# chenhuims/DistributedDeepLearningSpark

Hardware: AMD Instinct MI355X
Metric: images/sec (whole node) ResNet-50 ImageNet-shape at 1/2/4/8 MI355X (higher is better)
Workload: dtype bf16; 1 GPU; model=resnet50, global_batch=256, image=224, per_gpu_batch=256, parallelism=dp1, optimizer=sgd-momentum, buckets=4

## Files before the change

### distributeddeeplearningspark_amd/csrc/bindings.cpp

```cpp
#include <torch/extension.h>
#include <ATen/hip/impl/HIPStreamMasqueradingAsCUDA.h>
#include <ATen/DeviceGuard.h>

#include "ddl_gemm.h"
#include "ddl_ops.h"

namespace py = pybind11;
using namespace ddl;

namespace {

inline hipStream_t cur_stream() { return at::hip::getCurrentHIPStreamMasqueradingAsCUDA().stream(); }

#define CHECK_CUDA(x) TORCH_CHECK((x).is_cuda(), #x " must be a GPU tensor")
#define CHECK_BF16(x) TORCH_CHECK((x).scalar_type() == at::kBFloat16, #x " must be bf16")
#define CHECK_F32(x) TORCH_CHECK((x).scalar_type() == at::kFloat, #x " must be fp32")
#define CHECK_CONTIG(x) TORCH_CHECK((x).is_contiguous(), #x " must be contiguous")
#define HIP_OK(expr)                                                                   \
  do {                                                                                 \
    int _e = (expr);                                                                   \
    TORCH_CHECK(_e == 0, "HIP launch failed: ", hipGetErrorString((hipError_t)_e)); \
  } while (0)

void fill_geom(ConvGeom& g, const py::dict& d) {
  g.n = d["n"].cast<int>();
  g.hi = d["hi"].cast<int>();
  g.wi = d["wi"].cast<int>();
  g.c = d["c"].cast<int>();
  g.ho = d["ho"].cast<int>();
  g.wo = d["wo"].cast<int>();
  g.sh = d["sh"].cast<int>();
  g.sw = d["sw"].cast<int>();
  g.tap_c = d["tap_c"].cast<int>();
  g.tap_shift = (g.tap_c > 0 && (g.tap_c & (g.tap_c - 1)) == 0) ? __builtin_ctz((unsigned)g.tap_c) : -1;
  auto dh = d["dh"].cast<std::vector<int>>();
  auto dw = d["dw"].cast<std::vector<int>>();
  std::vector<int> wt = d.contains("wt") ? d["wt"].cast<std::vector<int>>() : std::vector<int>(dh.size(), 0);
  TORCH_CHECK(dh.size() == dw.size() && dh.size() <= (size_t)kMaxTaps && wt.size() == dh.size(), "bad tap table");
  g.ntaps = (int)dh.size();
  for (size_t i = 0; i < dh.size(); ++i) {
    TORCH_CHECK(dh[i] >= -128 && dh[i] < 128 && dw[i] >= -128 && dw[i] < 128, "tap offset out of int8 range");
    g.dh[i] = (int8_t)dh[i];
    g.dw[i] = (int8_t)dw[i];
    g.wt[i] = (int16_t)wt[i];
  }
}

void gemm(const at::Tensor& a, const at::Tensor& b, const at::Tensor& c, int64_t M, int64_t N, int64_t K,
          int64_t a_mode, int64_t b_mode, int64_t lda, int64_t ldb, int64_t ldc, int64_t epi, int64_t tile,
          int64_t k_split, double alpha, double beta, c10::optional<at::Tensor> bias,
          c10::optional<at::Tensor> resid, int64_t ldr, int64_t relu, c10::optional<py::dict> geom,
          c10::optional<py::dict> outmap, int64_t b_kdiv, int64_t b_tap_stride,
          c10::optional<at::Tensor> stats, c10::optional<at::Tensor> aux, double drop_p, int64_t drop_seed,
          c10::optional<at::Tensor> resid_mask, c10::optional<at::Tensor> bnr_x, c10::optional<at::Tensor> bnr_mask,
          c10::optional<at::Tensor> bnr_mean, int64_t rsub_h, int64_t rsub_w, c10::optional<at::Tensor> bnr_scale, c10::optional<at::Tensor> bnr_shift, int64_t split_stride,
          int64_t zcount, int64_t za, int64_t zb, int64_t zc, int64_t zbias, std::vector<int64_t> cls_tap0,
          std::vector<int64_t> cls_nt, std::vector<int64_t> cls_coff, bool bnr_premask,
          c10::optional<at::Tensor> colscale, c10::optional<at::Tensor> relu_mask_out) {
  CHECK_CUDA(a);
  CHECK_CUDA(b);
  CHECK_CUDA(c);
  CHECK_BF16(a);
  CHECK_BF16(b);
  if (epi == EPI_BF16) { CHECK_BF16(c); } else { CHECK_F32(c); }
  const bool k_vec = a_mode == OP_KC || a_mode == OP_KC_GATHER || a_mode == OP_KC_GATHER8 || b_mode == OP_KC;
  TORCH_CHECK(!k_vec || K % 8 == 0, "gemm: K-contiguous operands need K % 8 == 0 (16-B vectors), got ", K);
  if (a_mode == OP_KC) TORCH_CHECK(lda % 8 == 0, "gemm: lda must be a multiple of 8");
  if (b_mode == OP_KC) TORCH_CHECK(ldb % 8 == 0, "gemm: ldb must be a multiple of 8");
  if (a_mode == OP_RC) TORCH_CHECK(lda % 8 == 0, "gemm: lda must be a multiple of 8");
  if (b_mode == OP_RC || b_mode == OP_RC_TAPS) TORCH_CHECK(ldb % 8 == 0, "gemm: ldb must be a multiple of 8");
  TORCH_CHECK(((uintptr_t)a.data_ptr() % 16) == 0 && ((uintptr_t)b.data_ptr() % 16) == 0, "gemm: operands must be 16-B aligned");
  TORCH_CHECK(k_split > 0 && k_split % 64 == 0, "gemm: k_split must be a positive multiple of 64");
  TORCH_CHECK(tile >= 0 && tile <= kTileConv3, "gemm: bad tile id");
  if (tile == kTileStream) {
    TORCH_CHECK(a_mode == OP_KC && (b_mode == OP_KC || b_mode == OP_RC) && epi == EPI_BF16 && !outmap.has_value() &&
                    relu <= ACT_RELU && drop_p == 0.0 && beta == 0.0 && k_split >= K,
                "gemm stream: KC x (KC|RC) operands, bf16 epilogue without GELU/dropout/outmap/beta/split-K");
    TORCH_CHECK(gemm_stream_panel((int)N, (int)K) > 0, "gemm stream: unsupported (N, K) = (", N, ", ", K, ")");
    TORCH_CHECK(ldc % 8 == 0 && ((uintptr_t)c.data_ptr() % 16) == 0, "gemm stream: 16-B aligned output rows");
    TORCH_CHECK(!resid || (ldr % 4 == 0 && ((uintptr_t)resid->data_ptr() % 8) == 0), "gemm stream: resid alignment");
  }
  if (tile == kTile256) {
    TORCH_CHECK(a_mode <= OP_RC && b_mode <= OP_RC && !outmap.has_value(), "gemm256: plain KC/RC operands only");
    TORCH_CHECK(K % 64 == 0 && k_split % 64 == 0, "gemm256: K and k_split must be multiples of 64");
    TORCH_CHECK(M >= 8 && N >= 8, "gemm256: M, N >= 8");
  }
  const int bm = (tile == 0 || tile == 1) ? 128 : 64;
  const int bn = (tile == 0 || tile == 2) ? 128 : 64;
  if (a_mode == OP_RC || a_mode == OP_RC_GATHER) TORCH_CHECK(M % 8 == 0, "gemm: row-contiguous A needs M % 8 == 0");
  if (b_mode == OP_RC || b_mode == OP_RC_GATHER || b_mode == OP_RC_GATHER8 || b_mode == OP_RC_TAPS)
    TORCH_CHECK(N % 8 == 0, "gemm: row-contiguous B needs N % 8 == 0");
  GemmParams p{};
  p.a = a.data_ptr();
  p.b = b.data_ptr();
  p.c = c.data_ptr();
  p.lda = lda;
  p.ldb = ldb;
  p.ldc = ldc;
  p.M = (int)M;
  p.N = (int)N;
  p.K = (int)K;
  p.k_split = (int)k_split;
  p.a_mode = (int)a_mode;
  p.b_mode = (int)b_mode;
  p.b_kdiv = (int)b_kdiv;
  p.b_tap_stride = b_tap_stride;
  p.alpha = (float)alpha;
  p.beta = (float)beta;
  TORCH_CHECK(relu >= ACT_NONE && relu <= ACT_GELU_BWD, "gemm: bad activation code");
  TORCH_CHECK(epi == EPI_BF16 || (relu == 0 && drop_p == 0.0), "gemm: activation/dropout need the bf16 epilogue");
  p.relu = (int)relu;
  if (relu >= ACT_GELU) {
    TORCH_CHECK(aux.has_value(), "gemm: GELU epilogues need the aux (pre-activation) tensor");
    CHECK_CUDA(*aux);
    CHECK_BF16(*aux);
    TORCH_CHECK(aux->numel() >= (M - 1) * ldc + N && ((uintptr_t)aux->data_ptr() % 16) == 0, "gemm: aux size/alignment");
    p.aux = aux->data_ptr();
  }
  TORCH_CHECK(drop_p >= 0.0 && drop_p < 1.0, "gemm: dropout p in [0, 1)");
  if (drop_p > 0.0) {
    p.drop_thresh = drop_t8(drop_p);
    p.drop_scale = drop_scale8(p.drop_thresh);
    p.drop_seed = (unsigned long long)drop_seed;
  }
  p.ldr = ldr;
  if (bias) {
    CHECK_CUDA(*bias);
    CHECK_F32(*bias);
    TORCH_CHECK(bias->numel() >= N, "bias too short");
    TORCH_CHECK((uintptr_t)bias->data_ptr() % 16 == 0, "gemm: bias must be 16-B aligned (vector loads)");
    p.bias = bias->data_ptr<float>();
  }
  if (resid) {
    CHECK_CUDA(*resid);
    CHECK_BF16(*resid);
    p.resid = resid->data_ptr();
  }
  if (rsub_h > 0) {
    TORCH_CHECK(resid.has_value() && epi == EPI_BF16 && !outmap.has_value() && !resid_mask.has_value() && rsub_w > 0 &&
                    M % (rsub_h * rsub_w) == 0,
                "gemm: a stride-2 residual needs resid (bf16, no outmap / mask) and M = N * rsub_h * rsub_w");
    const int64_t hs = (rsub_h + 1) / 2, ws_ = (rsub_w + 1) / 2;
    TORCH_CHECK(resid->numel() >= ((M / (rsub_h * rsub_w)) * hs * ws_ - 1) * ldr + N, "gemm: stride-2 residual too small");
    p.rsub_h = (int)rsub_h;
    p.rsub_w = (int)rsub_w;
  }
  if (resid_mask) {
    TORCH_CHECK(resid.has_value() && epi == EPI_BF16 && !outmap.has_value(), "gemm: resid_mask needs a residual (bf16, no outmap)");
    TORCH_CHECK(resid_mask->scalar_type() == at::kByte && resid_mask->is_contiguous() && ldr % 8 == 0 &&
                    resid_mask->numel() >= ((M - 1) * ldr + N + 7) / 8,
                "gemm: resid_mask must be uint8 [M * ldr / 8] with ldr % 8 == 0");
    p.resid_mask = resid_mask->data_ptr<uint8_t>();
  }
  if (geom) {
    fill_geom(p.g, *geom);
    TORCH_CHECK((int64_t)p.g.n * p.g.hi * p.g.wi * p.g.c < (int64_t(1) << 31),
                "gemm: a gathered tensor must have fewer than 2^31 elements");
    if (a_mode == OP_KC_GATHER)
      TORCH_CHECK(p.g.tap_c % 64 == 0 && (cls_nt.empty() ? K == (int64_t)p.g.ntaps * p.g.tap_c : K <= (int64_t)p.g.ntaps * p.g.tap_c),
                  "conv A gather: tap_c % 64 and K = taps*C");
    if (b_mode == OP_RC_GATHER) TORCH_CHECK(p.g.tap_c % bn == 0 && N == (int64_t)p.g.ntaps * p.g.tap_c, "conv B gather: tap_c % BN and N = taps*C");
    if (b_mode == OP_RC_TAPS) TORCH_CHECK(b_kdiv % 64 == 0 && K == (int64_t)p.g.ntaps * b_kdiv, "conv B taps: kdiv % 64 and K = taps*kdiv");
    if (a_mode == OP_KC_GATHER8) TORCH_CHECK(p.g.tap_c % 8 == 0 && K == (int64_t)p.g.ntaps * p.g.tap_c, "conv A gather8: tap_c % 8 and K = taps*C");
    if (b_mode == OP_RC_GATHER8) TORCH_CHECK(p.g.tap_c % 8 == 0 && N == (int64_t)p.g.ntaps * p.g.tap_c, "conv B gather8: tap_c % 8 and N = taps*C");
    if (a_mode == OP_KC_GATHER || a_mode == OP_KC_GATHER8) TORCH_CHECK(p.g.c == p.g.tap_c, "gather: c == tap_c");
  } else {
    TORCH_CHECK(a_mode <= OP_RC && b_mode <= OP_RC, "gather modes need a geometry");
  }
  if (outmap) {
    const auto& d = *outmap;
    p.om.enabled = 1;
    p.om.gh = d["gh"].cast<int>();
    p.om.gw = d["gw"].cast<int>();
    p.om.hy = d["hy"].cast<int>();
    p.om.wy = d["wy"].cast<int>();
    p.om.so = d["so"].cast<int>();
    p.om.oh = d["oh"].cast<int>();
    p.om.ow = d["ow"].cast<int>();
    p.om.zero_siblings = d.contains("zero") ? d["zero"].cast<int>() : 0;
  }
  if (stats) {
    CHECK_CUDA(*stats);
    CHECK_F32(*stats);
    TORCH_CHECK(epi == EPI_BF16, "fused stats need the bf16 epilogue");
    TORCH_CHECK(stats->numel() >= (int64_t)kStatShards * 2 * N, "stats workspace too small");
    p.stats = stats->data_ptr<float>();
  }
  if (bnr_x) {
    TORCH_CHECK(stats.has_value() && bnr_mean.has_value() && epi == EPI_BF16 && tile != kTile256,
                "gemm: the fused BN-backward reduction needs a stats workspace, the mean and a bf16 epilogue");
    TORCH_CHECK(tile == kTileStream || (N % 4 == 0 && ldc % 8 == 0 && !bias && relu == 0 && !aux &&
                                        drop_p == 0.0 && (a_mode == OP_KC || (a_mode == OP_KC_GATHER && b_mode == OP_KC))),
                "gemm: BN-backward reduce outside the streaming kernel: plain or gathered-A data-gradient, N % 4 == 0, "
                "ldc % 8 == 0, no bias / activation (a residual and a parity-class output map are allowed)");
    CHECK_CUDA(*bnr_x);
    CHECK_BF16(*bnr_x);
    TORCH_CHECK(bnr_x->is_contiguous() && bnr_x->numel() >= (M - 1) * ldc + N && ((uintptr_t)bnr_x->data_ptr() % 16) == 0,
                "gemm: bnr_x must be a 16-B aligned bf16 [M][ldc]");
    CHECK_F32(*bnr_mean);
    TORCH_CHECK(bnr_mean->numel() >= N && ((uintptr_t)bnr_mean->data_ptr() % 16) == 0, "gemm: bnr_mean [N], 16-B aligned");
    p.bnr_x = bnr_x->data_ptr();
    p.bnr_mean = bnr_mean->data_ptr<float>();
    if (bnr_mask) {
      TORCH_CHECK(bnr_mask->scalar_type() == at::kByte && bnr_mask->is_contiguous() && ldc % 8 == 0 &&
                      bnr_mask->numel() >= ((M - 1) * ldc + N + 7) / 8,
                  "gemm: bnr_mask must be uint8 [M * ldc / 8]");
      p.bnr_mask = bnr_mask->data_ptr<uint8_t>();
    }
    if (bnr_scale || bnr_shift) {
      TORCH_CHECK(bnr_scale && bnr_shift && !bnr_mask, "gemm: bnr scale/shift (no mask bits)");
      CHECK_F32(*bnr_scale);
      CHECK_F32(*bnr_shift);
      TORCH_CHECK(bnr_scale->numel() >= N && bnr_shift->numel() >= N && ((uintptr_t)bnr_scale->data_ptr() % 16) == 0 &&
                      ((uintptr_t)bnr_shift->data_ptr() % 16) == 0,
                  "gemm: bnr scale / shift [N], 16-B aligned");
      p.bnr_scale = bnr_scale->data_ptr<float>();
      p.bnr_shift = bnr_shift->data_ptr<float>();
    }
    if (bnr_premask) {
      TORCH_CHECK(bnr_mask.has_value() && !outmap.has_value(), "gemm: bnr_premask needs the mask bits and no output map");
      p.bnr_premask = 1;
    }
  } else if (bnr_premask) {
    TORCH_CHECK(stats.has_value() && bnr_mask.has_value() && !bnr_scale && !bnr_shift && !outmap.has_value() &&
                    epi == EPI_BF16 && tile != kTile256,
                "gemm: bnr_premask needs a stats workspace, the mask bits, a bf16 epilogue and no output map");
    TORCH_CHECK(tile == kTileStream || (tile != kTileConv3 && N % 4 == 0 && ldc % 8 == 0 && !bias && relu == 0 && !aux &&
                                        drop_p == 0.0 && a_mode == OP_KC),
                "gemm: bnr_premask outside the streaming kernel: plain data-gradient (a pointwise conv), N % 4 == 0, "
                "ldc % 8 == 0, no bias / activation");
    TORCH_CHECK(bnr_mask->is_cuda() && bnr_mask->scalar_type() == at::kByte && bnr_mask->is_contiguous() && ldc % 8 == 0 &&
                    bnr_mask->numel() >= ((M - 1) * ldc + N + 7) / 8,
                "gemm: bnr_mask must be uint8 [M * ldc / 8]");
    p.bnr_mask = bnr_mask->data_ptr<uint8_t>();
    p.bnr_premask = 1;
  }
  if (colscale || relu_mask_out) {
    TORCH_CHECK(tile == kTileStream && colscale.has_value() && resid.has_value() && b_mode == OP_KC && !stats && !bnr_x &&
                    !bnr_premask && rsub_h == 0 && alpha == 1.0,
                "gemm: colscale / relu_mask_out run on the streaming kernel's forward form with a residual, without "
                "statistics or a BN-backward reduction; the column scale takes alpha's place (alpha == 1)");
    CHECK_CUDA(*colscale);
    CHECK_F32(*colscale);
    TORCH_CHECK(colscale->is_contiguous() && colscale->numel() >= N && ((uintptr_t)colscale->data_ptr() % 16) == 0,
                "gemm: colscale [N] fp32, 16-B aligned");
    p.colscale = colscale->data_ptr<float>();
    if (relu_mask_out) {
      TORCH_CHECK(relu_mask_out->is_cuda() && relu_mask_out->scalar_type() == at::kByte && relu_mask_out->is_contiguous() &&
                      relu_mask_out->numel() >= ((M - 1) * ldc + N + 7) / 8,
                  "gemm: relu_mask_out must be uint8 [M * ldc / 8]");
      p.relu_mask_out = relu_mask_out->data_ptr<uint8_t>();
    }
  }
  (void)bm;
  if (tile == kTileConv3)
    TORCH_CHECK(conv3x3_halo_ok(p) && epi == EPI_BF16, "gemm conv3x3: needs a 3x3 / stride-1 / pad-1 KC_GATHER x KC "
                "conv with C % 64 == 0, N % 64 == 0, no split-K and at most bias/ReLU/statistics in the epilogue");
  if (split_stride > 0) {
    const int64_t splits = (K + k_split - 1) / k_split;
    TORCH_CHECK(epi == EPI_F32 && beta == 0.0 && split_stride >= M * ldc && c.numel() >= splits * split_stride,
                "gemm: split-K slabs need EPI_F32, beta = 0 and a workspace of splits x split_stride floats");
    p.split_stride = split_stride;
  }
  if (zcount > 1 && cls_nt.empty()) {
    TORCH_CHECK(tile >= 0 && tile <= 3 && !stats && !bnr_x && !outmap && !resid && !aux && drop_p == 0.0 &&
                    split_stride == 0 && relu <= ACT_RELU && za >= 0 && zb >= 0 && zc >= 0 && zbias >= 0,
                "gemm: replica batching (zcount > 1) runs the 64/128 tiles with at most bias / ReLU / split-K atomics");
    TORCH_CHECK(za % 8 == 0 && zb % 8 == 0 && (epi == EPI_BF16 ? zc % 8 : zc % 4) == 0 && zbias % 4 == 0,
                "gemm: replica strides must keep 16-B alignment");
    TORCH_CHECK(c.numel() >= (zcount - 1) * zc + (M - 1) * ldc + N, "gemm: output too small for zcount replicas");
    TORCH_CHECK(!bias || bias->numel() >= (zcount - 1) * zbias + N, "gemm: bias too short for zcount replicas");
    p.zcount = (int)zcount;
    p.za = za;
    p.zb = zb;
    p.zc = zc;
    p.zbias = zbias;
  }
  if (!cls_nt.empty()) {
    const int64_t nc = (int64_t)cls_nt.size();
    TORCH_CHECK(nc <= kMaxZCls && (int64_t)cls_tap0.size() == nc && (int64_t)cls_coff.size() == nc && zcount == nc,
                "gemm: parity classes need cls_tap0 / cls_nt / cls_coff of zcount <= ", kMaxZCls, " entries");
    TORCH_CHECK(tile >= 0 && tile <= 3 && a_mode == OP_KC_GATHER && b_mode == OP_KC && epi == EPI_BF16 && outmap &&
                    p.om.oh == 0 && p.om.ow == 0 && !p.om.zero_siblings && !stats && !bnr_x && !resid && !aux && !bias &&
                    drop_p == 0.0 && relu == 0 && split_stride == 0 && za == 0 && zb == 0 && zc == 0 && zbias == 0,
                "gemm: parity classes run KC_GATHER x KC on the 64/128 tiles with a plain bf16 output map");
    TORCH_CHECK(p.om.gh > 0 && p.om.gw > 0 && M % ((int64_t)p.om.gh * p.om.gw) == 0, "gemm: classes need M = n * gh * gw");
    const int64_t nimg = M / ((int64_t)p.om.gh * p.om.gw);
    const int64_t last_row = ((nimg - 1) * p.om.hy + (int64_t)(p.om.gh - 1) * p.om.so) * p.om.wy + (int64_t)(p.om.gw - 1) * p.om.so;
    int64_t kmax = 0;
    for (int64_t z = 0; z < nc; ++z) {
      TORCH_CHECK(cls_nt[z] > 0 && cls_tap0[z] >= 0 && cls_tap0[z] + cls_nt[z] <= p.g.ntaps, "gemm: class taps out of range");
      TORCH_CHECK(cls_coff[z] >= 0 && cls_coff[z] % 8 == 0 && cls_coff[z] + last_row * ldc + N <= c.numel(),
                  "gemm: class output offset out of range");
      TORCH_CHECK((cls_tap0[z] + cls_nt[z]) * (int64_t)p.g.tap_c <= ldb, "gemm: class filter columns past ldb");
      kmax = std::max(kmax, cls_nt[z] * (int64_t)p.g.tap_c);
      p.cls_tap0[z] = (int)cls_tap0[z];
      p.cls_nt[z] = (int)cls_nt[z];
      p.cls_coff[z] = cls_coff[z];
    }
    TORCH_CHECK(K == kmax && k_split >= K, "gemm: classes need K = the largest class's K and no split-K");
    p.zcls = 1;
    p.zcount = (int)nc;
  }
  at::DeviceGuard guard(a.device());
  HIP_OK(launch_gemm_bf16(p, (int)epi, (int)tile, cur_stream()));
}

void conv3x3_wgrad(const at::Tensor& dy, const at::Tensor& x, const at::Tensor& gw, const c10::optional<at::Tensor>& ws,
                   int64_t splits, int64_t tpb, bool pp) {
  CHECK_CUDA(dy);
  CHECK_CUDA(x);
  CHECK_CUDA(gw);
  CHECK_BF16(dy);
  CHECK_BF16(x);
  CHECK_F32(gw);
  CHECK_CONTIG(dy);
  CHECK_CONTIG(x);
  CHECK_CONTIG(gw);
  TORCH_CHECK(x.dim() == 4 && gw.dim() == 4 && gw.size(1) == 3 && gw.size(2) == 3 && gw.size(3) == x.size(3),
              "conv3x3_wgrad: x [N, H, W, Ci], gw [Co, 3, 3, Ci]");
  const int n = (int)x.size(0), h = (int)x.size(1), w = (int)x.size(2), ci = (int)x.size(3), co = (int)gw.size(0);
  TORCH_CHECK(dy.numel() == (int64_t)n * h * w * co, "conv3x3_wgrad: dy must be [N, H, W, Co] (stride 1, pad 1)");
  TORCH_CHECK(conv3x3_wgrad_ok(n, h, w, ci, co), "conv3x3_wgrad: needs Ci, Co % 64 == 0 and a <= 256-pixel row tiling");
  int s_plan = 0, t_plan = 0, ntiles = 0;
  conv3x3_wgrad_plan(n, h, w, ci, co, 1, 1, s_plan, t_plan, ntiles);
  TORCH_CHECK(splits >= 1 && tpb >= 1 && (splits - 1) * tpb < ntiles && splits * tpb >= ntiles,
              "conv3x3_wgrad: splits x tiles-per-split must cover the pixel tiles exactly once");
  float* wsp = nullptr;
  if (ws) {
    CHECK_CUDA(*ws);
    CHECK_F32(*ws);
    TORCH_CHECK(ws->is_contiguous() && ws->numel() >= splits * co * 9 * (int64_t)ci, "conv3x3_wgrad: workspace too small");
    wsp = ws->data_ptr<float>();
  }
  at::DeviceGuard guard(x.device());
  HIP_OK(launch_conv3x3_wgrad(reinterpret_cast<const uint16_t*>(dy.data_ptr()), reinterpret_cast<const uint16_t*>(x.data_ptr()),
                              gw.data_ptr<float>(), wsp, n, h, w, ci, co, (int)splits, (int)tpb, pp, cur_stream()));
}

py::object conv3x3_wgrad_plan_py(int64_t n, int64_t h, int64_t w, int64_t ci, int64_t co, int64_t blocks_per_cu,
                                 int64_t cus) {
  if (!conv3x3_wgrad_ok((int)n, (int)h, (int)w, (int)ci, (int)co)) return py::none();
  int splits = 0, tpb = 0, ntiles = 0;
  conv3x3_wgrad_plan((int)n, (int)h, (int)w, (int)ci, (int)co, (int)blocks_per_cu, (int)cus, splits, tpb, ntiles);
  return py::make_tuple(splits, tpb);
}

}

void register_ops(py::module& m);
void register_runtime(py::module& m);
void register_transformer(py::module& m);
void register_rnn(py::module& m);
void register_layer_ops(py::module& m);

PYBIND11_MODULE(_C, m) {
  m.doc() = "MI355X-native kernels and runtime of distributeddeeplearningspark_amd";
  m.def("gemm", &gemm, "MFMA implicit-GEMM (bf16 in, fp32 accumulate)", py::arg("a"), py::arg("b"), py::arg("c"),
        py::arg("M"), py::arg("N"), py::arg("K"), py::arg("a_mode"), py::arg("b_mode"), py::arg("lda"),
        py::arg("ldb"), py::arg("ldc"), py::arg("epi"), py::arg("tile"), py::arg("k_split"), py::arg("alpha") = 1.0,
        py::arg("beta") = 0.0, py::arg("bias") = py::none(), py::arg("resid") = py::none(), py::arg("ldr") = 0,
        py::arg("relu") = false, py::arg("geom") = py::none(), py::arg("outmap") = py::none(),
        py::arg("b_kdiv") = 0, py::arg("b_tap_stride") = 0, py::arg("stats") = py::none(),
        py::arg("aux") = py::none(), py::arg("drop_p") = 0.0, py::arg("drop_seed") = 0,
        py::arg("resid_mask") = py::none(), py::arg("bnr_x") = py::none(), py::arg("bnr_mask") = py::none(),
        py::arg("bnr_mean") = py::none(), py::arg("rsub_h") = 0, py::arg("rsub_w") = 0,
        py::arg("bnr_scale") = py::none(), py::arg("bnr_shift") = py::none(),
        py::arg("split_stride") = 0, py::arg("zcount") = 1, py::arg("za") = 0, py::arg("zb") = 0, py::arg("zc") = 0,
        py::arg("zbias") = 0, py::arg("cls_tap0") = std::vector<int64_t>{}, py::arg("cls_nt") = std::vector<int64_t>{},
        py::arg("cls_coff") = std::vector<int64_t>{}, py::arg("bnr_premask") = false,
        py::arg("colscale") = py::none(), py::arg("relu_mask_out") = py::none());
  m.def("conv3x3_wgrad", &conv3x3_wgrad, "3x3 stride-1 weight gradient (halo kernel): gw += dW", py::arg("dy"),
        py::arg("x"), py::arg("gw"), py::arg("ws"), py::arg("splits"), py::arg("tpb"), py::arg("pp") = false);
  m.def("conv3x3_wgrad_plan", &conv3x3_wgrad_plan_py,
        "(splits, tiles per split) of the 3x3 weight-gradient halo kernel, or None when it does not apply",
        py::arg("n"), py::arg("h"), py::arg("w"), py::arg("ci"), py::arg("co"), py::arg("blocks_per_cu"),
        py::arg("cus"));
  m.attr("ACT_NONE") = (int)ACT_NONE;
  m.attr("ACT_RELU") = (int)ACT_RELU;
  m.attr("ACT_GELU") = (int)ACT_GELU;
  m.attr("ACT_GELU_BWD") = (int)ACT_GELU_BWD;
  m.attr("OP_KC") = (int)OP_KC;
  m.attr("OP_RC") = (int)OP_RC;
  m.attr("OP_KC_GATHER") = (int)OP_KC_GATHER;
  m.attr("OP_RC_GATHER") = (int)OP_RC_GATHER;
  m.attr("OP_RC_TAPS") = (int)OP_RC_TAPS;
  m.attr("OP_KC_GATHER8") = (int)OP_KC_GATHER8;
  m.attr("OP_RC_GATHER8") = (int)OP_RC_GATHER8;
  m.attr("EPI_BF16") = (int)EPI_BF16;
  m.attr("EPI_F32") = (int)EPI_F32;
  m.attr("EPI_F32_ATOMIC") = (int)EPI_F32_ATOMIC;
  register_ops(m);
  register_transformer(m);
  register_rnn(m);
  register_layer_ops(m);
  register_runtime(m);
}
```

### distributeddeeplearningspark_amd/csrc/include/ddl_gemm.h

```cpp
#pragma once
#include <stdint.h>

namespace ddl {

enum OperandMode : int {
  OP_KC = 0,
  OP_RC = 1,
  OP_KC_GATHER = 2,
  OP_RC_GATHER = 3,
  OP_RC_TAPS = 4,
  OP_KC_GATHER8 = 5,
  OP_RC_GATHER8 = 6,
};

enum EpilogueMode : int {
  EPI_BF16 = 0,
  EPI_F32 = 1,
  EPI_F32_ATOMIC = 2,
  EPI_BF16_LITE = 3,
  EPI_BF16_BNR = 4,
};

constexpr int kMaxTaps = 64;
constexpr int kMaxZCls = 4;

struct ConvGeom {
  int n, hi, wi, c;
  int ho, wo;
  int sh, sw;
  int ntaps;
  int tap_c;
  int tap_shift;
  int8_t dh[kMaxTaps];
  int8_t dw[kMaxTaps];
  int16_t wt[kMaxTaps];
};

struct OutMap {
  int enabled;
  int gh, gw;
  int hy, wy;
  int so;
  int oh, ow;
  int zero_siblings;
};

struct GemmParams {
  const void* a; long lda;
  const void* b; long ldb;
  void* c; long ldc;
  int M, N, K;
  int k_split;
  int a_mode, b_mode;
  int b_kdiv; long b_tap_stride;
  ConvGeom g;
  OutMap om;
  const float* bias;
  const void* resid; long ldr;
  const uint8_t* resid_mask;
  float alpha, beta;
  int relu;
  float* stats;
  void* aux;
  uint32_t drop_thresh;
  float drop_scale;
  unsigned long long drop_seed;
  const void* bnr_x;
  const uint8_t* bnr_mask;
  const float* bnr_mean;
  const float* bnr_scale;
  const float* bnr_shift;
  int bnr_premask;
  int rsub_h, rsub_w;
  int group_m;
  long split_stride;
  int zcount;
  long za, zb, zc, zbias;
  int zcls;
  int cls_tap0[kMaxZCls], cls_nt[kMaxZCls];
  long cls_coff[kMaxZCls];
  const float* colscale;
  uint8_t* relu_mask_out;
};

enum Activation : int { ACT_NONE = 0, ACT_RELU = 1, ACT_GELU = 2, ACT_GELU_BWD = 3 };

constexpr int kStatShards = 32;
constexpr int kTile256 = 4;
constexpr int kTileStream = 5;
constexpr int kTileConv3 = 6;

bool conv3x3_halo_ok(const GemmParams& p);

bool conv3x3_wgrad_ok(int n, int h, int w, int ci, int co);
void conv3x3_wgrad_plan(int n, int h, int w, int ci, int co, int blocks_per_cu, int cus, int& splits, int& tpb,
                        int& ntiles);
int launch_conv3x3_wgrad(const uint16_t* dy, const uint16_t* x, float* gw, float* ws, int n, int h, int w, int ci,
                         int co, int splits, int tpb, bool pp, void* stream);

int gemm_stream_panel(int N, int K);

int launch_gemm_bf16(const GemmParams& p, int epi, int tile, void* stream);

}
```

### distributeddeeplearningspark_amd/csrc/include/ddl_ops.h

```cpp
#pragma once
#include <hip/hip_runtime.h>
#include <stdint.h>

namespace ddl {

inline uint32_t drop_t8(double p) {
  if (!(p > 0.0)) return 0u;
  const double t = p * 256.0 + 0.5;
  return t < 1.0 ? 1u : (t >= 255.0 ? 255u : (uint32_t)t);
}
inline float drop_scale8(uint32_t t8) { return t8 ? (float)(256.0 / (256.0 - (double)t8)) : 1.f; }

constexpr int kBnShards = 32;
constexpr int kMaxPartials = 512;

int bn_partial_rows(long M, int C);
int splitk_finalize(float* ws, void* y, const float* bias, float* stats, long M, int C, int relu, int splits,
                    long slab_stride, hipStream_t s, long brows = 0,
                    long zbias = 0);
int bn_stats(const void* x, float* ws, long M, int C, hipStream_t s);
int bn_finalize(const float* ws, int S, long M, int C, const float* gamma, const float* beta, float eps,
                float momentum, float* running_mean, float* running_var, float* save_mean, float* save_invstd,
                float* scale, float* shift, hipStream_t s);
int bn_apply(const void* x, const float* scale, const float* shift, const void* resid, void* y, void* mask, long M,
             int C, int relu, hipStream_t s, const float* res_scale = nullptr, const float* res_shift = nullptr);
int bn_bwd_reduce(const void* dy, const void* x, const void* y, const float* scale, const float* shift,
                  const float* mean, float* ws, long M, int C, int mode, hipStream_t s);
int bn_bwd_finalize(const float* ws, int S, long M, int C, const float* gamma, const float* mean, const float* invstd,
                    float* dgamma, float* dbeta, float* coef, hipStream_t s);
int bn_bwd_dx(const void* dy, const void* x, const void* y, const float* scale, const float* shift,
              const float* coef, void* dx, void* dres, long M, int C, int mode, hipStream_t s,
              const void* x2 = nullptr, const float* mean2 = nullptr, float* ws2 = nullptr);

int bn_fold_sums(const void* w, long ldw, const float* P, const float* wsg, const float* mean, const float* wsy,
                 int rows, float* sums, float* s, int Co, int Ci, hipStream_t st);
int bn_fold_coef(const void* w, long ldw, const float* P, const float* S, const float* s, const float* coef, void* WA,
                 void* WAt, void* Gm, float* kv, float* dW, long lddw, int Co, int Ci, hipStream_t st);
int gram_colsum(const void* y2, long ld, long M, int Ci, float* S, float* s, int cus, hipStream_t st);
int bn_fold_fwd_stats(const void* w, long ldw, const float* S, const float* s, long M, float* ws, int Co, int Ci,
                      hipStream_t st);

bool pool3s2_bn_bwd_ok(int N, int H, int W, int C, int Ho, int Wo, int k = 3);
int pool3s2_bn_bwd(const void* dy, const uint8_t* am, const void* x, const float* scale, const float* shift,
                   const float* mean, const float* coef, float* ws, int S, void* dx, int N, int H, int W, int C, int Ho,
                   int Wo, hipStream_t s, int k = 3);

int maxpool_fwd(const void* x, void* y, uint8_t* argmax, int N, int H, int W, int C, int Ho, int Wo, int kh, int kw,
                int sh, int sw, int ph, int pw, hipStream_t s, const float* scale = nullptr, const float* shift = nullptr);
int maxpool_bwd(const void* dy, const uint8_t* argmax, void* dx, int N, int H, int W, int C, int Ho, int Wo, int kh,
                int kw, int sh, int sw, int ph, int pw, hipStream_t s);
int avgpool_global_fwd(const void* x, void* y, int N, int HW, int C, hipStream_t s);
int avgpool_global_bwd(const void* dy, void* dx, int N, int HW, int C, hipStream_t s);

int softmax_xent(const void* logits, int logits_bf16, const int64_t* labels, const float* target_probs,
                 float* loss_rows, void* dlogits, int B, int K, long ld, float grad_scale, float label_smoothing,
                 int ignore_index, hipStream_t s, const float* grad_scale_dev = nullptr, float* loss_out = nullptr,
                 float out_scale = 1.f, int zrows = 0);
int label_count_inv(const int64_t* labels, long n, int ignore_index, float* inv, hipStream_t s);
int rows_sum_scaled(const float* rows, long n, float scale, const float* dev, float* out, hipStream_t s);
int scale_bf16_dev(void* x, long n, const float* s_dev, hipStream_t s);
int mse_fwd_bwd(const float* pred, const float* target, long n, float* loss, float* grad, hipStream_t s);
int prob_xent(const float* p, const int64_t* labels, const float* target, float* loss_rows, float* dp, int B, int K,
              float eps, float scale, int ignore_index, hipStream_t s);

int cast_f32_bf16(const float* x, void* y, long n, hipStream_t s);
int cast_bf16_f32(const void* x, float* y, long n, hipStream_t s);
int sum_rows_bf16(const void* x, void* y, int R, long n, hipStream_t s);
int relu_bwd(const void* dy, const void* y, void* dx, long n, hipStream_t s);
int add_bf16(const void* a, const void* b, void* y, long n, hipStream_t s);
int bias_grad(const void* dy, float* db, long M, int N, int accumulate, hipStream_t s, float* det_ws = nullptr,
              const void* relu_y = nullptr, void* relu_dx = nullptr, int zcount = 1, long zdb = 0);
int pad_cols_bf16(const void* x, long ldx, void* out, long R, int K, int Kp, hipStream_t s);
constexpr int kMaxZeroRanges = 8;
struct ZeroRanges {
  void* p[kMaxZeroRanges];
  long pre[kMaxZeroRanges + 1];
  int tail_words[kMaxZeroRanges];
  int count;
};
int zero_ranges(const ZeroRanges& r, hipStream_t s);
int gather_bf16(const void* src, const int* idx, void* out, long n, hipStream_t s);
int scatter_add_f32(const float* src, const int* idx, float* dst, long n, hipStream_t s);
int bias_grad_rows(long M);
int slab_reduce(const float* ws, int splits, float* c, long M, int N, long ldc, float beta, hipStream_t s);
int transpose_bf16(const void* x, void* y, int R, int C, long ldx, hipStream_t s);
int im2col(const void* x, void* col, int n, int hi, int wi, int c, int ho, int wo, int sh, int sw, int ntaps,
           const int* dh, const int* dw, int kpad, hipStream_t s);
int s2d_pad(const void* x, void* y, int N, int H, int W, int C, int Ho, int Wo, int pad, hipStream_t s);
int normalize_u8(const uint8_t* x, void* y, long npix, int c, int cpad, const float* mean, const float* invstd,
                 hipStream_t s);

int sgd_step(float* w, const float* g, float* mom, void* w16, long n, float lr, float momentum, float dampening,
             float wd, int nesterov, float gscale, hipStream_t s);
int adam_step(float* w, const float* g, float* m, float* v, void* w16, long n, float lr, float b1, float b2,
              float eps, float wd, int adamw, float bc1, float bc2, float gscale, float* tstep,
              hipStream_t s, unsigned* tick_ctr = nullptr);
int step_tick(float* t, hipStream_t s);
int adagrad_step(float* w, const float* g, float* acc, void* w16, long n, float lr, float eps, float wd, float gscale,
                 hipStream_t s);
int rmsprop_step(float* w, const float* g, float* acc, void* w16, long n, float lr, float rho, float eps, float wd,
                 float gscale, hipStream_t s);
int sumsq_f32(const float* x, long n, float* out, hipStream_t s);

struct AttnParams {
  const uint16_t* qkv; long ld;
  int q_off, k_off, v_off;
  uint16_t* o; long ldo;
  float* lse;
  const int* lens;
  int B, H, S;
  float scale, scale_log2;
  uint32_t drop_t8;
  float drop_scale;
  unsigned long long drop_seed;
  const uint16_t* dout; long lddo;
  float* dvec;
  uint16_t* dqkv; long lddqkv;
  int xcd_remap;
};
int attn_fwd(const AttnParams& p, hipStream_t s);
int attn_bwd(const AttnParams& p, hipStream_t s);

int layernorm_fwd(const void* x, const float* gamma, const float* beta, void* y, float* mean, float* rstd, long M,
                  int H, float eps, float drop_p, unsigned long long seed, hipStream_t s);
int ln_partial_rows(long M);
int ln_bwd_rows(long M, int H);
int layernorm_bwd(const void* dy, const void* x, const float* mean, const float* rstd, const float* gamma, void* dx,
                  void* dx_drop, float drop_p, unsigned long long seed, float* ws, int P, long M, int H,
                  float in_drop_p, unsigned long long in_seed, int parts, hipStream_t s);
int embed_word_grad(const int64_t* sorted_ids, const int64_t* perm, const void* ds, float* gword, long T, int H,
                    hipStream_t s);
int embed_word_grad_atomic(const int64_t* ids, const void* ds, float* gword, long T, int H, long V, hipStream_t s);
int embed_pos_grad(const void* ds, float* gpos, int B, int S, int H, hipStream_t s);
int colsum_partials(const float* ws, int P, int N, float* out, int accumulate, hipStream_t s, long ld = 0);
int mlm_gather(const void* h, const int64_t* pos, void* out, int B, int S, int P, int H, hipStream_t s);
int mlm_scatter(const void* dout, const int64_t* pos, void* dh, int B, int S, int P, int H, hipStream_t s);
int embed_fwd(const int64_t* ids, const int64_t* types, const void* word, const void* pos, const void* type,
              void* out, long T, int S, int H, hipStream_t s);
int embed_bwd(const int64_t* ids, const int64_t* types, const void* ds, float* gword, float* gpos, float* wsT, int P,
              int ntypes, long T, int S, int H, hipStream_t s);

constexpr int kMaxRnnRep = 16;
struct RnnRep {
  const float* x[kMaxRnnRep];
  const float* y[kMaxRnnRep];
  const float* W[kMaxRnnRep];
  const float* U[kMaxRnnRep];
  const float* b[kMaxRnnRep];
  const float* Wd[kMaxRnnRep];
  const float* bd[kMaxRnnRep];
  float* gW[kMaxRnnRep];
  float* gU[kMaxRnnRep];
  float* gb[kMaxRnnRep];
  float* gWd[kMaxRnnRep];
  float* gbd[kMaxRnnRep];
  float* hist[kMaxRnnRep];
  int nbr[kMaxRnnRep];
  int steps[kMaxRnnRep];
  int* ctr;
  int* live;
  int B, K;
};
struct OptRep {
  float* w[kMaxRnnRep];
  const float* g[kMaxRnnRep];
  float* s1[kMaxRnnRep];
  float* s2[kMaxRnnRep];
  float* t[kMaxRnnRep];
};
int rnn_replica_step(int cell, const RnnRep& rp, int R, int T, int H, int I, float* hs, float* cs, float* gates,
                     float* hlast, float* dh, float* dgates, const OptRep& op, long n, int opt, float lr, float p1,
                     float p2, float eps, float wd, int amode, hipStream_t s);
bool rnn_replica_ok(int cell, int H, int I, int K, int B);

bool rnn_fast_path(int H);
bool rnn_fuses_input(int H, int I);
bool rnn_reg_path(int cell, int H, int act, int ract);
int rnn_fwd(int cell, const float* xw, const float* x, const float* W, const float* b, int I, const float* U,
            float* hs, float* cs, float* gates, float* y, int B, int T, int H, int rs, int act, int ract,
            hipStream_t s);
int rnn_param_grad(int cell, const float* dg, const float* hs, const float* gates, const float* x, float* gU,
                   float* gW, float* gb, int B, int T, int H, int I, hipStream_t s, int rev = 0);
bool rnn_bwd_uses_ut(int H);
int rnn_bwd(int cell, const float* dy, const float* U, const float* UT, const float* hs, const float* cs,
            const float* gates, float* dgates, int B, int T, int H, int rs, int act, int ract, hipStream_t s);

struct RnnDir {
  const float* xw[2];
  const float* W[2];
  const float* b[2];
// ... 91 lines not shown
```

### distributeddeeplearningspark_amd/csrc/kernels/bn_fold.hip

```cpp
#include "ddl_common.h"
#include "ddl_ops.h"

namespace ddl {
namespace {

constexpr int FT = 32;
constexpr int BKG = 128;
constexpr int BKW = 64;

__device__ __forceinline__ double wave_sum(double v) {
#pragma unroll
  for (int o = 32; o > 0; o >>= 1) v += __shfl_xor(v, o, 64);
  return v;
}

constexpr int kSumSplit = 8;
__global__ __launch_bounds__(256) void bn_fold_sums_kernel(const bf16_t* __restrict__ w, long ldw,
                                                            const float* __restrict__ P,
                                                            const float* __restrict__ wsg,
                                                            const float* __restrict__ mean,
                                                            const float* __restrict__ wsy, int rows,
                                                            float* __restrict__ sums, float* __restrict__ s, int Co,
                                                            int Ci, int cb) {
  const int lane = threadIdx.x & 63, wv = threadIdx.x >> 6;
// ... 148 lines not shown
#pragma unroll
    for (int v = 0; v < G::V; ++v) {
      const int row = t0 + pr + v * G::PPP;
      reg[v] = row < r1 ? *reinterpret_cast<const uint4*>(y2 + (long)row * ld + ch * 8) : make_uint4(0u, 0u, 0u, 0u);
    }
  };
  load(r0);
  for (int t0 = r0; t0 < r1; t0 += G::TP) {
    __syncthreads();
#pragma unroll
    for (int v = 0; v < G::V; ++v)
      *reinterpret_cast<uint4*>(tile + (pr + v * G::PPP) * G::ROWB + ch * 16) = reg[v];
    if (panel == 0) {
#pragma unroll
      for (int v = 0; v < G::V; ++v) {
        const uint32_t wv[4] = {reg[v].x, reg[v].y, reg[v].z, reg[v].w};
#pragma unroll
        for (int q = 0; q < 4; ++q) {
          cs[2 * q] += __uint_as_float(wv[q] << 16);
          cs[2 * q + 1] += __uint_as_float(wv[q] & 0xffff0000u);
        }
      }
    }
    __syncthreads();
    if (t0 + G::TP < r1) load(t0 + G::TP);
    f32x4 acc[G::RB];
#pragma unroll
    for (int i = 0; i < G::RB; ++i) acc[i] = f32x4{0.f, 0.f, 0.f, 0.f};
#pragma unroll 2
    for (int kk = 0; kk < G::TP / 32; ++kk) {
      const bf16x8 b = gram_frag<G::ROWB>(tile, kk, cb, lane);
#pragma unroll
      for (int i = 0; i < G::RB; ++i) acc[i] = mfma16x16x32(gram_frag<G::ROWB>(tile, kk, 16 * i, lane), b, acc[i]);
    }
#pragma unroll
    for (int i = 0; i < G::RB; ++i) tot[i] += acc[i];
  }
#pragma unroll
  for (int i = 0; i < G::RB; ++i)
#pragma unroll
    for (int e = 0; e < 4; ++e)
      atomicAdd(S + (long)(16 * i + 4 * (lane >> 4) + e) * CI + cb + (lane & 15), tot[i][e]);
  if (panel == 0) {
    __syncthreads();
    float* red = reinterpret_cast<float*>(tile);
#pragma unroll
    for (int e = 0; e < 8; ++e) red[pr * CI + ch * 8 + e] = cs[e];
    __syncthreads();
    if ((int)threadIdx.x < CI) {
      double a = 0.0;
      for (int j = 0; j < G::PPP; ++j) a += (double)red[j * CI + threadIdx.x];
      atomicAdd(s + threadIdx.x, (float)a);
    }
  }
}

constexpr int FST = 32;
__global__ __launch_bounds__(256) void bn_fold_fwd_stats_kernel(const bf16_t* __restrict__ w, long ldw,
                                                                 const float* __restrict__ S,
                                                                 const float* __restrict__ s, long M,
                                                                 float* __restrict__ ws, int Co, int Ci) {
  __shared__ float Ssh[FST][256];
  __shared__ double wsh[4][256];
  __shared__ double sb[256];
  const int lane = threadIdx.x & 63, wv = threadIdx.x >> 6;
  const int co = (int)blockIdx.x * 4 + wv;
  const int cor = min(co, Co - 1);
  const double invM = 1.0 / (double)M;
  for (int ci = lane; ci < Ci; ci += 64) wsh[wv][ci] = (double)bf2f(w[(long)cor * ldw + ci]);
  for (int ci = threadIdx.x; ci < Ci; ci += 256) sb[ci] = (double)s[ci] * invM;
  double q[4] = {0.0, 0.0, 0.0, 0.0};
  for (int ci0 = 0; ci0 < Ci; ci0 += FST) {
    __syncthreads();
    for (int idx = threadIdx.x * 4; idx < FST * Ci; idx += 1024) {
      const float4 v = *reinterpret_cast<const float4*>(S + (long)ci0 * Ci + idx);
      *reinterpret_cast<float4*>(&Ssh[idx / Ci][idx % Ci]) = v;
    }
    __syncthreads();
#pragma unroll
    for (int t = 0; t < 4; ++t) {
      const int cj = lane + 64 * t;
      if (cj < Ci) {
        const double sj = sb[cj];
        double inner = 0.0;
#pragma unroll 8
        for (int r = 0; r < FST; ++r) inner += wsh[wv][ci0 + r] * ((double)Ssh[r][cj] * invM - sb[ci0 + r] * sj);
        q[t] += inner;
      }
    }
  }
  double mean = 0.0, var = 0.0;
#pragma unroll
  for (int t = 0; t < 4; ++t) {
    const int cj = lane + 64 * t;
    if (cj < Ci) {
      mean += wsh[wv][cj] * sb[cj];
      var += wsh[wv][cj] * q[t];
    }
  }
  mean = wave_sum(mean);
  var = wave_sum(var);
  if (var < 0.0) var = 0.0;
  if (lane == 0 && co < Co) {
    ws[co] = (float)((double)M * mean);
    ws[Co + co] = (float)((double)M * (var + mean * mean));
  }
}

}

int gram_colsum(const void* y2, long ld, long M, int Ci, float* S, float* s, int cus, hipStream_t st) {
  if ((Ci != 64 && Ci != 128 && Ci != 256) || M <= 0 || M >= (1L << 30) || ld % 8) return (int)hipErrorInvalidValue;
  const int P = Ci / 64, tp = Ci == 64 ? 256 : (Ci == 128 ? 128 : 64);
  long rows = std::max<long>(std::max(1024, 8 * Ci), (M + 2 * cus / P - 1) / std::max(1, 2 * cus / P));
  rows = (rows + tp - 1) / tp * tp;
  const int chunks = (int)((M + rows - 1) / rows);
  const dim3 grid((unsigned)(chunks * P));
  const bf16_t* y = (const bf16_t*)y2;
  switch (Ci) {
    case 64: hipLaunchKernelGGL(gram_colsum_kernel<64>, grid, dim3(256), 0, st, y, ld, (int)M, (int)rows, S, s); break;
    case 128: hipLaunchKernelGGL(gram_colsum_kernel<128>, grid, dim3(256), 0, st, y, ld, (int)M, (int)rows, S, s); break;
    default: hipLaunchKernelGGL(gram_colsum_kernel<256>, grid, dim3(256), 0, st, y, ld, (int)M, (int)rows, S, s); break;
  }
  return (int)hipGetLastError();
}

int bn_fold_fwd_stats(const void* w, long ldw, const float* S, const float* s, long M, float* ws, int Co, int Ci,
                      hipStream_t st) {
  if (Ci % FST || Ci > 256 || Ci % 4 || Co <= 0 || M <= 0) return (int)hipErrorInvalidValue;
  hipLaunchKernelGGL(bn_fold_fwd_stats_kernel, dim3((Co + 3) / 4), dim3(256), 0, st, (const bf16_t*)w, ldw, S, s, M, ws,
                     Co, Ci);
  return (int)hipGetLastError();
}

int bn_fold_sums(const void* w, long ldw, const float* P, const float* wsg, const float* mean, const float* wsy,
                 int rows, float* sums, float* s, int Co, int Ci, hipStream_t st) {
  const int cb = (Co + 3) / 4;
  const int sblocks = rows > 0 ? kSumSplit * ((Ci + 63) / 64) : 0;
  hipLaunchKernelGGL(bn_fold_sums_kernel, dim3(cb + sblocks), dim3(256), 0, st, (const bf16_t*)w, ldw, P, wsg,
                     mean, wsy, rows, sums, s, Co, Ci, cb);
  return (int)hipGetLastError();
}

int bn_fold_coef(const void* w, long ldw, const float* P, const float* S, const float* s, const float* coef, void* WA,
                 void* WAt, void* Gm, float* kv, float* dW, long lddw, int Co, int Ci, hipStream_t st) {
  if (Co % BKG || Ci % BKW) return (int)hipErrorInvalidValue;
  const int tc = Ci / FT;
  const int blocks = tc * tc + (Co / FT) * tc;
  hipLaunchKernelGGL(bn_fold_coef_kernel, dim3(blocks), dim3(256), 0, st, (const bf16_t*)w, ldw, P, S, s, coef,
                     (bf16_t*)WA, (bf16_t*)WAt, (bf16_t*)Gm, kv, dW, lddw, Co, Ci);
  return (int)hipGetLastError();
}

}
```

### distributeddeeplearningspark_amd/csrc/kernels/gemm_dispatch.hip

```cpp
#include "ddl_gemm.h"
#include <hip/hip_runtime.h>
#include <stdlib.h>
namespace ddl {
int launch_gemm_plain_akc(const GemmParams& p, int epi, int tile, hipStream_t s);
int launch_gemm_plain_arc(const GemmParams& p, int epi, int tile, hipStream_t s);
int launch_gemm_conv(const GemmParams& p, int epi, int tile, hipStream_t s);
int launch_gemm256(const GemmParams& p, int epi, hipStream_t s);
int launch_gemm_stream(const GemmParams& p, int epi, hipStream_t s);
int launch_conv3x3(const GemmParams& p, int epi, hipStream_t s);

int launch_gemm_bf16(const GemmParams& p_in, int epi, int tile, void* stream) {
  hipStream_t s = reinterpret_cast<hipStream_t>(stream);
  if (p_in.M <= 0 || p_in.N <= 0) return 0;
  GemmParams p = p_in;
  p.group_m = 8;
  if ((p.colscale || p.relu_mask_out) && tile != kTileStream) return (int)hipErrorInvalidValue;
  if (p.bnr_premask && (!p.bnr_mask || !p.stats || p.bnr_scale)) return (int)hipErrorInvalidValue;
  if (p.bnr_premask && !p.bnr_x && tile != kTileStream && p.a_mode != OP_KC) return (int)hipErrorInvalidValue;
  if ((p.bnr_x || p.bnr_premask) && tile != kTileStream &&
      (tile == kTile256 || epi != EPI_BF16 || p.om.zero_siblings ||
       (p.resid && (p.ldr % 4 || (uintptr_t)p.resid % 8)) || p.aux || p.drop_thresh || p.bias || p.relu || p.N % 4 || p.ldc % 8 ||
       !(p.a_mode == OP_KC || p.a_mode == OP_KC_GATHER) || (p.a_mode == OP_KC_GATHER && p.b_mode != OP_KC)))
    return (int)hipErrorInvalidValue;
  const bool plain = (p.a_mode == OP_KC || p.a_mode == OP_RC) && (p.b_mode == OP_KC || p.b_mode == OP_RC);
  if (tile == kTile256) {
    if (!plain || p.K % 64 || p.k_split % 64 || p.om.enabled) return (int)hipErrorInvalidValue;
    return launch_gemm256(p, epi, s);
  }
  if (tile == kTileStream) return launch_gemm_stream(p, epi, s);
  if (tile == kTileConv3) return launch_conv3x3(p, epi, s);
  if (plain) return p.a_mode == OP_KC ? launch_gemm_plain_akc(p, epi, tile, s) : launch_gemm_plain_arc(p, epi, tile, s);
  return launch_gemm_conv(p, epi, tile, s);
}
}
```

### distributeddeeplearningspark_amd/csrc/kernels/gemm_stream.hip

```cpp
#include "ddl_gemm_kernel.h"

namespace ddl {
namespace gst {

constexpr int THREADS = 256;
constexpr int BM = 64;
constexpr int LDS_BUDGET = 80 * 1024;
typedef __attribute__((address_space(3))) void lds_t;

template <int WN, int K, bool CSM = false>
struct Cfg {
  static constexpr int NB = 4 * WN;
  static constexpr int RN = WN / 16;
  static constexpr int KS = K / 32;
  static constexpr int CPR = K / 8;
  static constexpr int TILE = BM * K * 2;
  static constexpr int D = TILE / 1024 / 4;
  static constexpr int OCPR = NB / 8;
  static constexpr int STAGE = BM * NB * 2;
  static constexpr int RPP = THREADS / OCPR;
  static constexpr int S = BM / RPP;
  static constexpr int SV = CSM ? 2 * S : S;
  static constexpr int NBUF_FIT = (LDS_BUDGET - STAGE) / TILE;
  static constexpr int NBUF = NBUF_FIT > 4 ? 4 : NBUF_FIT;
  static constexpr int LDS = NBUF * TILE + STAGE;
  static_assert(NBUF >= 2, "A ring needs two buffers");
  static_assert(D >= 1 && OCPR >= 8 && RPP >= 1 && BM % RPP == 0, "shape");
  static_assert((NBUF - 1) * (D + SV) <= 63, "vmcnt range");
  static_assert(4 * 2 * OCPR * 8 * 4 <= STAGE, "stats reduction fits in the staging buffer");
};

template <int CPR>
__device__ __forceinline__ int sw(int r) {
  if constexpr (CPR == 8) return (r >> 1) & 7;
  else return r & 15;
}

template <int N>
__device__ __forceinline__ void wait_vm() {
  __builtin_amdgcn_s_waitcnt((N & 15) | ((N >> 4) << 14) | 0x0F70);
}

template <class CF, int SV = CF::S>
__device__ __forceinline__ void wait_tile(int younger_store_tiles) {
  constexpr int base = (CF::NBUF - 1) * CF::D;
  switch (younger_store_tiles) {
    case 0: wait_vm<base>(); break;
    case 1: wait_vm<base + SV>(); break;
    case 2: wait_vm<base + 2 * SV>(); break;
    default: wait_vm<base + 3 * SV>(); break;
  }
}

template <class CF>
__device__ __forceinline__ void stage_a(const bf16_t* __restrict__ A, long lda, int M, int m0, char* slot, int w,
                                        int lane) {
#pragma unroll
  for (int i = 0; i < CF::D; ++i) {
    const int blk = i * 4 + w;
    const int u = blk * 64 + lane;
    const int r = u / CF::CPR, cp = u % CF::CPR;
    const int c = cp ^ sw<CF::CPR>(r);
    const int gr = min(m0 + r, M - 1);
    const bf16_t* src = A + (long)gr * lda + c * 8;
    const uint32_t dst = __builtin_amdgcn_readfirstlane((uint32_t) reinterpret_cast<uintptr_t>((lds_t*)(slot + blk * 1024)));
    asm volatile("s_mov_b32 m0, %1\n\tglobal_load_lds_dwordx4 %0, off" ::"v"(src), "s"(dst) : "memory", "m0");
  }
}

}

typedef __attribute__((ext_vector_type(2))) unsigned u32x2_t;
typedef __attribute__((ext_vector_type(4))) unsigned u32x4_t;
__device__ __forceinline__ u32x4_t ald128(const void* p) {
  u32x4_t v;
  asm volatile("global_load_dwordx4 %0, %1, off" : "=v"(v) : "v"(p) : "memory");
  return v;
}
__device__ __forceinline__ u32x2_t ald64(const void* p) {
  u32x2_t v;
  asm volatile("global_load_dwordx2 %0, %1, off" : "=v"(v) : "v"(p) : "memory");
  return v;
}
__device__ __forceinline__ unsigned ald32(const void* p) {
  unsigned v;
  asm volatile("global_load_dword %0, %1, off" : "=v"(v) : "v"(p) : "memory");
  return v;
}
__device__ __forceinline__ unsigned ald16(const void* p) {
  unsigned v;
  asm volatile("global_load_ushort %0, %1, off" : "=v"(v) : "v"(p) : "memory");
  return v;
}
__device__ __forceinline__ unsigned ald8(const void* p) {
  unsigned v;
  asm volatile("global_load_ubyte %0, %1, off" : "=v"(v) : "v"(p) : "memory");
  return v;
}
template <bool ASM> __device__ __forceinline__ u32x4_t sld128(const void* p) {
  if constexpr (ASM) return ald128(p);
  return *reinterpret_cast<const u32x4_t*>(p);
}
template <bool ASM> __device__ __forceinline__ u32x2_t sld64(const void* p) {
  if constexpr (ASM) return ald64(p);
  return *reinterpret_cast<const u32x2_t*>(p);
}
template <bool ASM> __device__ __forceinline__ unsigned sld32(const void* p) {
  if constexpr (ASM) return ald32(p);
  return *reinterpret_cast<const uint32_t*>(p);
}
template <bool ASM> __device__ __forceinline__ unsigned sld16(const void* p) {
  if constexpr (ASM) return ald16(p);
  return *reinterpret_cast<const uint16_t*>(p);
}
template <bool ASM> __device__ __forceinline__ unsigned sld8(const void* p) {
  if constexpr (ASM) return ald8(p);
  return *reinterpret_cast<const uint8_t*>(p);
}


template <int WN, int K, int BMODE, bool RES, int BNR = 0, bool CSM = false>
__global__ __launch_bounds__(gst::THREADS, 2) void gemm_stream_kernel(const GemmParams p) {
  using namespace gst;
  using CF = Cfg<WN, K, CSM>;
  constexpr bool kAsmSide = true;
  __shared__ __attribute__((aligned(16))) char smem[CF::LDS];
  char* const stg = smem + CF::NBUF * CF::TILE;
  const int lane = threadIdx.x & 63, w = threadIdx.x >> 6;
  const int n0 = blockIdx.y * CF::NB;
  const int mt = (p.M + BM - 1) / BM;
  const int nloc = ((int)blockIdx.x < mt) ? (mt - 1 - (int)blockIdx.x) / (int)gridDim.x + 1 : 0;
  const bf16_t* __restrict__ A = reinterpret_cast<const bf16_t*>(p.a);

  bf16x8 bfr[CF::RN][CF::KS];
  {
    const bf16_t* __restrict__ B = reinterpret_cast<const bf16_t*>(p.b);
#pragma unroll
    for (int rn = 0; rn < CF::RN; ++rn)
#pragma unroll
      for (int ks = 0; ks < CF::KS; ++ks) {
        const int n = n0 + WN * w + 16 * rn + (lane & 15);
        const int k = 32 * ks + 8 * (lane >> 4);
        if constexpr (BMODE == OP_KC) {
          bfr[rn][ks] = *reinterpret_cast<const bf16x8*>(B + (long)n * p.ldb + k);
        } else {
          s16x8 v;
#pragma unroll
          for (int j = 0; j < 8; ++j) v[j] = (short)B[(long)(k + j) * p.ldb + n];
          bfr[rn][ks] = __builtin_bit_cast(bf16x8, v);
        }
      }
  }
  float bias_r[CF::RN][4];
#pragma unroll
  for (int rn = 0; rn < CF::RN; ++rn) {
    const float4 bv = p.bias ? *reinterpret_cast<const float4*>(p.bias + n0 + WN * w + 16 * rn + 4 * (lane >> 4))
                             : make_float4(0.f, 0.f, 0.f, 0.f);
    bias_r[rn][0] = bv.x;
    bias_r[rn][1] = bv.y;
    bias_r[rn][2] = bv.z;
    bias_r[rn][3] = bv.w;
  }
  float csc_r[CSM ? CF::RN : 1][4];
  if constexpr (CSM) {
#pragma unroll
    for (int rn = 0; rn < CF::RN; ++rn) {
      const float4 cv = *reinterpret_cast<const float4*>(p.colscale + n0 + WN * w + 16 * rn + 4 * (lane >> 4));
      csc_r[rn][0] = cv.x;
      csc_r[rn][1] = cv.y;
      csc_r[rn][2] = cv.z;
      csc_r[rn][3] = cv.w;
    }
  }
  wait_vm<0>();
  auto tile_m0 = [&](int i) { return min((int)blockIdx.x + i * (int)gridDim.x, mt - 1) * BM; };

#pragma unroll
  for (int s = 0; s < CF::NBUF - 1; ++s) stage_a<CF>(A, p.lda, p.M, tile_m0(s), smem + s * CF::TILE, w, lane);

  float s1[8], s2[8];
#pragma unroll
  for (int e = 0; e < 8; ++e) s1[e] = s2[e] = 0.f;
  const int oc = threadIdx.x % CF::OCPR, orow = threadIdx.x / CF::OCPR;
  float bmu[8];
  float bsc[BNR == 2 ? 8 : 1], bsh[BNR == 2 ? 8 : 1];
  if constexpr (BNR == 1 || BNR == 2) {
    const float4 a = *reinterpret_cast<const float4*>(p.bnr_mean + n0 + oc * 8);
    const float4 b = *reinterpret_cast<const float4*>(p.bnr_mean + n0 + oc * 8 + 4);
    bmu[0] = a.x; bmu[1] = a.y; bmu[2] = a.z; bmu[3] = a.w;
    bmu[4] = b.x; bmu[5] = b.y; bmu[6] = b.z; bmu[7] = b.w;
  }
  if constexpr (BNR == 2) {
    const float4 a0 = *reinterpret_cast<const float4*>(p.bnr_scale + n0 + oc * 8);
    const float4 a1 = *reinterpret_cast<const float4*>(p.bnr_scale + n0 + oc * 8 + 4);
    const float4 b0 = *reinterpret_cast<const float4*>(p.bnr_shift + n0 + oc * 8);
    const float4 b1 = *reinterpret_cast<const float4*>(p.bnr_shift + n0 + oc * 8 + 4);
    bsc[0] = a0.x; bsc[1] = a0.y; bsc[2] = a0.z; bsc[3] = a0.w; bsc[4] = a1.x; bsc[5] = a1.y; bsc[6] = a1.z; bsc[7] = a1.w;
    bsh[0] = b0.x; bsh[1] = b0.y; bsh[2] = b0.z; bsh[3] = b0.w; bsh[4] = b1.x; bsh[5] = b1.y; bsh[6] = b1.z; bsh[7] = b1.w;
  }
  bf16_t* __restrict__ Cout = reinterpret_cast<bf16_t*>(p.c);

  for (int i = 0; i < nloc; ++i) {
    const int m0 = tile_m0(i);
    u32x2_t rres[BM / 16][CF::RN];
    unsigned rmk32[BM / 16];
    u32x2_t rmk64[CF::RN == 4 ? BM / 16 : 1];
    unsigned rodd_bits = 0u;
    const bool has_mask = p.resid_mask != nullptr;
    if constexpr (RES) {
#pragma unroll
      for (int mb = 0; mb < BM / 16; ++mb) {
        const int m = min(m0 + 16 * mb + (lane & 15), p.M - 1);
        long rrow = m;
        if (p.rsub_h) {
          int rn_, ri_, rj_;
          pix_decompose((uint32_t)m, p.rsub_h, p.rsub_w, rn_, ri_, rj_);
          const bool rodd = (ri_ | rj_) & 1;
          rodd_bits |= (rodd ? 1u : 0u) << mb;
          rrow = rodd ? 0L : ((long)rn_ * ((p.rsub_h + 1) >> 1) + (ri_ >> 1)) * ((p.rsub_w + 1) >> 1) + (rj_ >> 1);
        }
        const long row = rrow * p.ldr + n0 + WN * w;
#pragma unroll
        for (int rn = 0; rn < CF::RN; ++rn)
          rres[mb][rn] = sld64<kAsmSide>(reinterpret_cast<const bf16_t*>(p.resid) + row + 16 * rn + 4 * (lane >> 4));
        const void* mp = has_mask ? (const void*)(p.resid_mask + (row >> 3)) : p.resid;
        if constexpr (CF::RN == 1) rmk32[mb] = sld16<kAsmSide>(mp);
        else if constexpr (CF::RN == 2) rmk32[mb] = sld32<kAsmSide>(mp);
        else rmk64[mb] = sld64<kAsmSide>(mp);
      }
    }
    u32x4_t bx[(BNR == 1 || BNR == 2) ? CF::S : 1];
    unsigned bm8[(BNR == 1 || BNR == 3) ? CF::S : 1];
    if constexpr (BNR) {
#pragma unroll
      for (int ps = 0; ps < CF::S; ++ps) {
        const int m = min(m0 + orow + ps * CF::RPP, p.M - 1);
        const long idx = (long)m * p.ldc + n0 + oc * 8;
        if constexpr (BNR != 3) bx[ps] = sld128<kAsmSide>(reinterpret_cast<const bf16_t*>(p.bnr_x) + idx);
        if constexpr (BNR == 1)
          bm8[ps] = sld8<kAsmSide>(p.bnr_mask ? (const void*)(p.bnr_mask + (idx >> 3)) : (const void*)p.bnr_x);
        if constexpr (BNR == 3) bm8[ps] = sld8<kAsmSide>(p.bnr_mask + (idx >> 3));
      }
    }
    const int ahead = i + CF::NBUF - 1;
    stage_a<CF>(A, p.lda, p.M, tile_m0(ahead), smem + (ahead % CF::NBUF) * CF::TILE, w, lane);
    if constexpr (CSM) {
      if (p.relu_mask_out) wait_tile<CF, CF::SV>(min(i, CF::NBUF - 1));
      else wait_tile<CF>(min(i, CF::NBUF - 1));
    } else {
      wait_tile<CF>(min(i, CF::NBUF - 1));
    }
    __builtin_amdgcn_s_barrier();

    const char* abuf = smem + (i % CF::NBUF) * CF::TILE;
    f32x4 acc[BM / 16][CF::RN];
#pragma unroll
    for (int mb = 0; mb < BM / 16; ++mb)
#pragma unroll
      for (int rn = 0; rn < CF::RN; ++rn) acc[mb][rn] = f32x4{0.f, 0.f, 0.f, 0.f};
#pragma unroll
    for (int ks = 0; ks < CF::KS; ++ks)
#pragma unroll
      for (int mb = 0; mb < BM / 16; ++mb) {
        const int r = 16 * mb + (lane & 15);
        const int c = 4 * ks + (lane >> 4);
        const bf16x8 a = *reinterpret_cast<const bf16x8*>(abuf + r * (K * 2) + ((c ^ sw<CF::CPR>(r)) << 4));
#pragma unroll
        for (int rn = 0; rn < CF::RN; ++rn) acc[mb][rn] = mfma16x16x32(bfr[rn][ks], a, acc[mb][rn]);
      }

    constexpr int kBnrLoads = BNR == 1 ? 2 * CF::S : (BNR != 0 ? CF::S : 0);
    if constexpr (kAsmSide && RES) {
      wait_vm<CF::D + kBnrLoads>();
      __builtin_amdgcn_sched_barrier(0);
#pragma unroll
      for (int mb = 0; mb < BM / 16; ++mb) {
#pragma unroll
        for (int rn = 0; rn < CF::RN; ++rn) asm volatile("" : "+v"(rres[mb][rn]));
        if constexpr (CF::RN == 4) asm volatile("" : "+v"(rmk64[mb]));
        else asm volatile("" : "+v"(rmk32[mb]));
      }
    }
#pragma unroll
    for (int mb = 0; mb < BM / 16; ++mb) {
      const int r = 16 * mb + (lane & 15);
#pragma unroll
      for (int rn = 0; rn < CF::RN; ++rn) {
        const int nl = WN * w + 16 * rn + 4 * (lane >> 4);
        float v[4];
#pragma unroll
        for (int e = 0; e < 4; ++e) {
          if constexpr (CSM) v[e] = fmaf(acc[mb][rn][e], csc_r[rn][e], bias_r[rn][e]);
          else v[e] = fmaf(acc[mb][rn][e], p.alpha, bias_r[rn][e]);
        }
        if constexpr (RES) {
          const u32x2_t rv = rres[mb][rn];
          uint64_t mraw;
          if constexpr (CF::RN == 4) mraw = ((uint64_t)rmk64[mb].y << 32) | rmk64[mb].x;
          else mraw = rmk32[mb];
          const uint64_t rm = ((rodd_bits >> mb) & 1u) ? 0ull : (has_mask ? mraw : ~0ull);
          const uint32_t mk = (uint32_t)(rm >> (16 * rn + 4 * (lane >> 4)));
          v[0] += (mk & 1u) ? __uint_as_float(rv.x << 16) : 0.f;
          v[1] += (mk & 2u) ? __uint_as_float(rv.x & 0xffff0000u) : 0.f;
          v[2] += (mk & 4u) ? __uint_as_float(rv.y << 16) : 0.f;
          v[3] += (mk & 8u) ? __uint_as_float(rv.y & 0xffff0000u) : 0.f;
        }
        if (p.relu == ACT_RELU) {
#pragma unroll
          for (int e = 0; e < 4; ++e) v[e] = fmaxf(v[e], 0.f);
        }
        *reinterpret_cast<uint2*>(stg + r * (CF::NB * 2) + (((nl >> 3) ^ sw<CF::OCPR>(r)) << 4) + (nl & 7) * 2) =
            make_uint2(pack_bf16x2(v[0], v[1]), pack_bf16x2(v[2], v[3]));
      }
    }
    __builtin_amdgcn_s_waitcnt(0xC07F);
    __builtin_amdgcn_s_barrier();

    if constexpr (kAsmSide && BNR) {
      wait_vm<CF::D>();
      __builtin_amdgcn_sched_barrier(0);
#pragma unroll
      for (int ps = 0; ps < CF::S; ++ps) {
        if constexpr (BNR != 3) asm volatile("" : "+v"(bx[ps]));
        if constexpr (BNR == 1 || BNR == 3) asm volatile("" : "+v"(bm8[ps]));
      }
    }
#pragma unroll
    for (int ps = 0; ps < CF::S; ++ps) {
      const int r = orow + ps * CF::RPP;
      const int m = m0 + r;
      uint4 v = *reinterpret_cast<const uint4*>(stg + r * (CF::NB * 2) + ((oc ^ sw<CF::OCPR>(r)) << 4));
      if constexpr (BNR == 3) {
        const uint32_t b = bm8[ps];
        v.x &= ((b & 1u) ? 0xffffu : 0u) | ((b & 2u) ? 0xffff0000u : 0u);
        v.y &= ((b & 4u) ? 0xffffu : 0u) | ((b & 8u) ? 0xffff0000u : 0u);
        v.z &= ((b & 16u) ? 0xffffu : 0u) | ((b & 32u) ? 0xffff0000u : 0u);
        v.w &= ((b & 64u) ? 0xffffu : 0u) | ((b & 128u) ? 0xffff0000u : 0u);
      }
      if (m < p.M) {
        *reinterpret_cast<uint4*>(Cout + (long)m * p.ldc + n0 + oc * 8) = v;
        if constexpr (CSM) {
          if (p.relu_mask_out) {
            const uint32_t wv[4] = {v.x, v.y, v.z, v.w};
            uint32_t bits = 0u;
#pragma unroll
            for (int q = 0; q < 4; ++q) {
              bits |= (((wv[q] & 0xffffu) - 1u) < 0x7f80u ? 1u : 0u) << (2 * q);
              bits |= (((wv[q] >> 16) - 1u) < 0x7f80u ? 1u : 0u) << (2 * q + 1);
            }
            p.relu_mask_out[((long)m * p.ldc + n0 + oc * 8) >> 3] = (uint8_t)bits;
          }
        }
        if constexpr (BNR == 3) {
          const uint32_t wv[4] = {v.x, v.y, v.z, v.w};
#pragma unroll
          for (int q = 0; q < 4; ++q) {
            s1[2 * q] += __uint_as_float(wv[q] << 16);
            s1[2 * q + 1] += __uint_as_float(wv[q] & 0xffff0000u);
          }
        } else if constexpr (BNR) {
          const uint32_t wv[4] = {v.x, v.y, v.z, v.w};
          const uint32_t xv[4] = {bx[ps].x, bx[ps].y, bx[ps].z, bx[ps].w};
          uint32_t bmk = 0xffu;
          if constexpr (BNR == 1) bmk = p.bnr_mask ? bm8[ps] : 0xffu;
#pragma unroll
          for (int q = 0; q < 4; ++q) {
#pragma unroll
            for (int h = 0; h < 2; ++h) {
              const int e = 2 * q + h;
              const float xe = __uint_as_float(h ? (xv[q] & 0xffff0000u) : (xv[q] << 16));
              bool keep;
              if constexpr (BNR == 2) keep = xe * bsc[e] + bsh[e] > 0.f;
              else keep = (bmk >> e) & 1u;
              const float d = keep ? __uint_as_float(h ? (wv[q] & 0xffff0000u) : (wv[q] << 16)) : 0.f;
              s1[e] += d;
              s2[e] += d * (xe - bmu[e]);
            }
          }
        } else if (!CSM && p.stats) {
          const uint32_t wv[4] = {v.x, v.y, v.z, v.w};
#pragma unroll
          for (int q = 0; q < 4; ++q) {
            const float lo = __uint_as_float(wv[q] << 16), hi = __uint_as_float(wv[q] & 0xffff0000u);
            s1[2 * q] += lo;
            s2[2 * q] += lo * lo;
            s1[2 * q + 1] += hi;
            s2[2 * q + 1] += hi * hi;
          }
        }
      }
    }
  }
  wait_vm<0>();

  if (!CSM && p.stats) {
#pragma unroll
    for (int o = CF::OCPR; o < 64; o <<= 1)
#pragma unroll
      for (int e = 0; e < 8; ++e) {
        s1[e] += __shfl_xor(s1[e], o, 64);
        s2[e] += __shfl_xor(s2[e], o, 64);
      }
    __syncthreads();
    float* red = reinterpret_cast<float*>(stg);
    if (lane < CF::OCPR) {
#pragma unroll
      for (int e = 0; e < 8; ++e) {
        red[(w * CF::OCPR + lane) * 16 + e] = s1[e];
        red[(w * CF::OCPR + lane) * 16 + 8 + e] = s2[e];
      }
    }
    __syncthreads();
    float* st = p.stats + (long)(blockIdx.x % kStatShards) * 2 * p.N;
    for (int t = threadIdx.x; t < CF::NB; t += THREADS) {
      const int ch = t >> 3, e = t & 7;
      float a = 0.f, b = 0.f;
#pragma unroll
      for (int ww = 0; ww < 4; ++ww) {
        a += red[(ww * CF::OCPR + ch) * 16 + e];
        b += red[(ww * CF::OCPR + ch) * 16 + 8 + e];
      }
      atomicAdd(st + n0 + t, a);
      atomicAdd(st + p.N + n0 + t, b);
    }
  }
}

namespace {

int num_cus() {
  static int cus = 0;
  if (!cus) {
    int dev = 0;
    (void)hipGetDevice(&dev);
    if (hipDeviceGetAttribute(&cus, hipDeviceAttributeMultiprocessorCount, dev) != hipSuccess || cus <= 0) cus = 256;
  }
  return cus;
}

template <int WN, int K, int BMODE>
int launch_ws(const GemmParams& p, hipStream_t s) {
  using CF = gst::Cfg<WN, K>;
  constexpr bool kRes = !(WN == 64 && K == 128);
  constexpr bool kBnr = CF::NB <= (K >= 256 ? 64 : 128);
  const int panels = p.N / CF::NB;
  const int mt = (p.M + gst::BM - 1) / gst::BM;
  const int gx = std::max(1, std::min(mt, 2 * num_cus() / std::max(1, panels)));
  if (p.colscale || p.relu_mask_out) {
    constexpr bool kCsm = BMODE == OP_KC && ((WN == 64 && K == 64) || (WN == 32 && K == 128) || (WN == 32 && K == 256));
    if constexpr (kCsm) {
      if (!p.colscale || !p.resid || p.bnr_x || p.bnr_premask || p.stats || p.rsub_h) return (int)hipErrorInvalidValue;
      hipLaunchKernelGGL((gemm_stream_kernel<WN, K, BMODE, true, 0, true>), dim3(gx, panels), dim3(gst::THREADS), 0, s, p);
    } else {
      return (int)hipErrorInvalidValue;
    }
  } else if (p.bnr_premask) {
    if constexpr (kBnr && kRes && BMODE == OP_RC) {
      if (!p.bnr_mask || p.bnr_scale) return (int)hipErrorInvalidValue;
      if (p.resid)
        hipLaunchKernelGGL((gemm_stream_kernel<WN, K, BMODE, true, 3>), dim3(gx, panels), dim3(gst::THREADS), 0, s, p);
      else
        hipLaunchKernelGGL((gemm_stream_kernel<WN, K, BMODE, false, 3>), dim3(gx, panels), dim3(gst::THREADS), 0, s, p);
    } else {
      return (int)hipErrorInvalidValue;
    }
  } else if (p.bnr_x && p.bnr_scale) {
    constexpr bool kRes2 = WN == 16 && K == 256 && BMODE == OP_RC;
    if constexpr (kBnr) {
      if (p.resid) {
        if constexpr (kRes2)
          hipLaunchKernelGGL((gemm_stream_kernel<WN, K, BMODE, true, 2>), dim3(gx, panels), dim3(gst::THREADS), 0, s, p);
        else
          return (int)hipErrorInvalidValue;
      } else {
        hipLaunchKernelGGL((gemm_stream_kernel<WN, K, BMODE, false, 2>), dim3(gx, panels), dim3(gst::THREADS), 0, s, p);
      }
    } else {
      return (int)hipErrorInvalidValue;
    }
  } else if (p.bnr_x) {
    if constexpr (kBnr && kRes) {
      if (p.resid)
        hipLaunchKernelGGL((gemm_stream_kernel<WN, K, BMODE, true, 1>), dim3(gx, panels), dim3(gst::THREADS), 0, s, p);
      else
        hipLaunchKernelGGL((gemm_stream_kernel<WN, K, BMODE, false, 1>), dim3(gx, panels), dim3(gst::THREADS), 0, s, p);
    } else if constexpr (kBnr) {
      if (p.resid) return (int)hipErrorInvalidValue;
      hipLaunchKernelGGL((gemm_stream_kernel<WN, K, BMODE, false, 1>), dim3(gx, panels), dim3(gst::THREADS), 0, s, p);
    } else {
      return (int)hipErrorInvalidValue;
    }
  } else if (p.resid) {
    if constexpr (kRes)
      hipLaunchKernelGGL((gemm_stream_kernel<WN, K, BMODE, true>), dim3(gx, panels), dim3(gst::THREADS), 0, s, p);
    else
      return (int)hipErrorInvalidValue;
  } else {
    hipLaunchKernelGGL((gemm_stream_kernel<WN, K, BMODE, false>), dim3(gx, panels), dim3(gst::THREADS), 0, s, p);
  }
  return (int)hipGetLastError();
}

template <int WN, int BMODE>
int launch_k(const GemmParams& p, hipStream_t s) {
  switch (p.K) {
    case 64: return launch_ws<WN, 64, BMODE>(p, s);
    case 128: return launch_ws<WN, 128, BMODE>(p, s);
    default:
      if constexpr (WN <= 32) return launch_ws<WN, 256, BMODE>(p, s);
      return (int)hipErrorInvalidValue;
  }
}

template <int BMODE>
int launch_panel(const GemmParams& p, int nb, hipStream_t s) {
  switch (nb) {
    case 64: return launch_k<16, BMODE>(p, s);
    case 128: return launch_k<32, BMODE>(p, s);
    default: return launch_k<64, BMODE>(p, s);
  }
}

}

int gemm_stream_panel(int N, int K) {
  if (K != 64 && K != 128 && K != 256) return 0;
  const int max_nb = K == 256 ? 128 : 256;
  for (int nb = max_nb; nb >= 64; nb >>= 1)
    if (N % nb == 0 && (N == nb || nb == max_nb)) return nb;
  return 0;
}

int launch_gemm_stream(const GemmParams& p, int epi, hipStream_t s) {
  int nb = gemm_stream_panel(p.N, p.K);
  if (p.resid && p.K == 128 && nb == 256) nb = 128;
  if ((p.bnr_x || p.bnr_premask) && nb > (p.K >= 256 ? 64 : 128)) nb = p.K >= 256 ? 64 : 128;
  const bool ok = nb && epi == EPI_BF16 && p.a_mode == OP_KC && (p.b_mode == OP_KC || p.b_mode == OP_RC) &&
                  !p.om.enabled && !p.aux && !p.drop_thresh && (p.relu == ACT_NONE || p.relu == ACT_RELU) &&
                  p.beta == 0.f && p.k_split >= p.K && p.lda % 8 == 0 && p.ldc % 8 == 0 &&
                  (p.b_mode == OP_RC || p.ldb % 8 == 0) && (!p.resid || p.ldr % 4 == 0) &&
                  ((uintptr_t)p.a % 16 == 0) && ((uintptr_t)p.c % 16 == 0) &&
                  (p.b_mode == OP_RC || (uintptr_t)p.b % 16 == 0) && (!p.resid || (uintptr_t)p.resid % 8 == 0) &&
                  (!p.bnr_x || (p.stats && (uintptr_t)p.bnr_x % 16 == 0 && (uintptr_t)p.bnr_mean % 16 == 0)) &&
                  (!p.bnr_scale || (p.bnr_shift && (uintptr_t)p.bnr_scale % 16 == 0 &&
                                    (uintptr_t)p.bnr_shift % 16 == 0)) &&
                  (!p.bnr_premask || (p.stats && p.bnr_mask)) &&
                  (!p.colscale || (uintptr_t)p.colscale % 16 == 0);
  if (!ok) return (int)hipErrorInvalidValue;
  return p.b_mode == OP_KC ? launch_panel<OP_KC>(p, nb, s) : launch_panel<OP_RC>(p, nb, s);
}

}
```

### distributeddeeplearningspark_amd/csrc/ops_bindings.cpp

```cpp
#include <torch/extension.h>
#include <ATen/hip/impl/HIPStreamMasqueradingAsCUDA.h>
#include <ATen/DeviceGuard.h>

#include "ddl_ops.h"

namespace py = pybind11;
using namespace ddl;

namespace {

inline hipStream_t cur_stream() { return at::hip::getCurrentHIPStreamMasqueradingAsCUDA().stream(); }

#define CK(cond, ...) TORCH_CHECK(cond, __VA_ARGS__)
#define GPU(x) CK((x).is_cuda(), #x " must be a GPU tensor")
#define BF16(x) CK((x).scalar_type() == at::kBFloat16 && (x).is_contiguous(), #x " must be contiguous bf16")
#define F32(x) CK((x).scalar_type() == at::kFloat && (x).is_contiguous(), #x " must be contiguous fp32")
#define HIP_OK(expr)                                                                  \
  do {                                                                                \
    int _e = (expr);                                                                  \
    CK(_e == 0, "HIP launch failed: ", hipGetErrorString((hipError_t)_e)); \
  } while (0)

template <class T>
T* optr(const c10::optional<at::Tensor>& t) {
// ... 8 lines not shown
  HIP_OK(bn_stats(x.data_ptr(), ws.data_ptr<float>(), x.numel() / C, (int)C, cur_stream()));
}

void splitk_finalize_(const at::Tensor& ws, const at::Tensor& y, int64_t C, c10::optional<at::Tensor> bias, bool relu,
                      c10::optional<at::Tensor> stats, int64_t splits, int64_t brows, int64_t zbias) {
  GPU(ws); F32(ws); BF16(y);
  CK(C % 8 == 0 && y.numel() % C == 0 && y.is_contiguous() && ws.is_contiguous(), "splitk_finalize: shapes");
  CK(splits >= 0 && ws.numel() >= std::max<int64_t>(splits, 1) * y.numel() && (splits > 0 || ws.numel() == y.numel()),
     "splitk_finalize: workspace size");
  if (bias) {
    F32(*bias);
    CK(brows > 0 ? (zbias % 4 == 0 && bias->numel() >= ((y.numel() / C - 1) / brows) * zbias + C) : bias->numel() == C,
       "splitk_finalize: bias [C] (or per-replica biases every zbias elements)");
  }
  if (stats) { F32(*stats); CK(stats->numel() == (int64_t)kBnShards * 2 * C, "splitk_finalize: stats [32, 2, C]"); }
  at::DeviceGuard g(ws.device());
  HIP_OK(splitk_finalize(ws.data_ptr<float>(), y.data_ptr(), optr<const float>(bias), optr<float>(stats), y.numel() / C,
                         (int)C, relu ? 1 : 0, (int)splits, (long)y.numel(), cur_stream(), (long)brows, (long)zbias));
}

int64_t bn_partial_rows_(int64_t M, int64_t C) { return bn_partial_rows(M, (int)C); }

void bn_finalize_(const at::Tensor& ws, int64_t M, int64_t C, c10::optional<at::Tensor> gamma,
                  c10::optional<at::Tensor> beta, double eps, double momentum, c10::optional<at::Tensor> rmean,
                  c10::optional<at::Tensor> rvar, const at::Tensor& smean, const at::Tensor& sinv,
                  const at::Tensor& scale, const at::Tensor& shift) {
  GPU(ws); F32(ws); F32(smean); F32(sinv); F32(scale); F32(shift);
  CK(smean.numel() >= C && sinv.numel() >= C && scale.numel() >= C && shift.numel() >= C, "bn_finalize: sizes");
  CK(ws.numel() % (2 * C) == 0, "bn_finalize: ws must be [S][2][C]");
  at::DeviceGuard g(ws.device());
  HIP_OK(bn_finalize(ws.data_ptr<float>(), (int)(ws.numel() / (2 * C)), M, (int)C, optr<const float>(gamma),
                     optr<const float>(beta), (float)eps, (float)momentum, optr<float>(rmean), optr<float>(rvar),
                     smean.data_ptr<float>(), sinv.data_ptr<float>(), scale.data_ptr<float>(),
                     shift.data_ptr<float>(), cur_stream()));
}

void bn_apply_(const at::Tensor& x, const at::Tensor& scale, const at::Tensor& shift, c10::optional<at::Tensor> resid,
               const at::Tensor& y, int64_t C, bool relu, c10::optional<at::Tensor> mask,
               c10::optional<at::Tensor> res_scale, c10::optional<at::Tensor> res_shift) {
  GPU(x); BF16(x); BF16(y); F32(scale); F32(shift);
  CK(C % 8 == 0 && x.numel() % C == 0 && y.numel() == x.numel(), "bn_apply: shapes");
  if (resid) { BF16(*resid); CK(resid->numel() == x.numel(), "bn_apply: resid shape"); }
  CK(res_scale.has_value() == res_shift.has_value() && (!res_scale || resid), "bn_apply: res_scale/res_shift pair needs resid");
  if (res_scale) {
    F32(*res_scale); F32(*res_shift);
    CK(res_scale->numel() == C && res_shift->numel() == C && res_scale->is_contiguous() && res_shift->is_contiguous(),
       "bn_apply: res_scale/res_shift [C]");
  }
  if (mask) {
    CK(mask->scalar_type() == at::kByte && mask->is_contiguous() && mask->numel() >= (x.numel() / 8 + 3) / 4 * 4,
       "bn_apply: mask must be uint8 [numel / 8 rounded up to 4] (one byte per 8 channels)");
  }
  at::DeviceGuard g(x.device());
  HIP_OK(bn_apply(x.data_ptr(), scale.data_ptr<float>(), shift.data_ptr<float>(), optr<const void>(resid), y.data_ptr(),
                  optr<void>(mask), x.numel() / C, (int)C, relu ? 1 : 0, cur_stream(), optr<const float>(res_scale),
                  optr<const float>(res_shift)));
}

void bn_bwd_reduce_(const at::Tensor& dy, const at::Tensor& x, c10::optional<at::Tensor> y,
                    c10::optional<at::Tensor> scale, c10::optional<at::Tensor> shift, const at::Tensor& mean,
                    const at::Tensor& ws, int64_t C, int64_t mode) {
  GPU(dy); BF16(dy); BF16(x); F32(mean); F32(ws);
  CK(dy.numel() == x.numel() && x.numel() % C == 0 && C % 8 == 0, "bn_bwd_reduce: shapes");
  if (mode == 1) { CK(y.has_value(), "mode 1 needs y"); BF16(*y); CK(y->numel() == x.numel(), "bn_bwd_reduce: y shape"); }
  if (mode == 3) CK(y.has_value() && y->scalar_type() == at::kByte && y->numel() >= x.numel() / 8,
                    "mode 3 needs the uint8 bit mask of bn_apply");
  CK(mode >= 0 && mode <= 3, "bn_bwd_reduce: mode");
  if (mode == 2) { CK(scale.has_value() && shift.has_value(), "mode 2 needs scale/shift"); F32(*scale); F32(*shift); }
  CK(ws.numel() >= (int64_t)bn_partial_rows(x.numel() / C, (int)C) * 2 * C, "bn_bwd_reduce: workspace too small");
  at::DeviceGuard g(x.device());
  HIP_OK(bn_bwd_reduce(dy.data_ptr(), x.data_ptr(), optr<const void>(y), optr<const float>(scale),
                       optr<const float>(shift), mean.data_ptr<float>(), ws.data_ptr<float>(), x.numel() / C, (int)C,
                       (int)mode, cur_stream()));
}

void bn_bwd_finalize_(const at::Tensor& ws, int64_t M, int64_t C, c10::optional<at::Tensor> gamma,
                      const at::Tensor& mean, const at::Tensor& invstd, c10::optional<at::Tensor> dgamma,
                      c10::optional<at::Tensor> dbeta, const at::Tensor& coef) {
  GPU(ws); F32(ws); F32(mean); F32(invstd); F32(coef);
  CK(coef.numel() >= 3 * C, "bn_bwd_finalize: coef size");
  CK(ws.numel() % (2 * C) == 0, "bn_bwd_finalize: ws must be [S][2][C]");
  at::DeviceGuard g(ws.device());
  HIP_OK(bn_bwd_finalize(ws.data_ptr<float>(), (int)(ws.numel() / (2 * C)), M, (int)C, optr<const float>(gamma), mean.data_ptr<float>(),
                         invstd.data_ptr<float>(), optr<float>(dgamma), optr<float>(dbeta), coef.data_ptr<float>(),
                         cur_stream()));
}

void bn_fold_sums_(const at::Tensor& w, const at::Tensor& P, const at::Tensor& wsg, const at::Tensor& mean,
                   c10::optional<at::Tensor> wsy, const at::Tensor& sums, const at::Tensor& s) {
  GPU(w); F32(P); F32(wsg); F32(mean); F32(sums); F32(s);
  CK(w.scalar_type() == at::kBFloat16 && w.dim() == 2 && w.stride(1) == 1, "bn_fold_sums: w [Co, Ci] bf16");
  const int64_t Co = w.size(0), Ci = w.size(1);
  CK(P.numel() == Co * Ci && wsg.numel() == (int64_t)kBnShards * 2 * Co && mean.numel() >= Co && sums.numel() == 2 * Co &&
         s.numel() == Ci,
     "bn_fold_sums: shapes");
  if (wsy) { F32(*wsy); CK(wsy->numel() % (2 * Ci) == 0 && wsy->numel() > 0, "bn_fold_sums: wsy [rows, 2, Ci]"); }
  at::DeviceGuard g(w.device());
  HIP_OK(bn_fold_sums(w.data_ptr(), w.stride(0), P.data_ptr<float>(), wsg.data_ptr<float>(), mean.data_ptr<float>(),
                      optr<const float>(wsy), wsy ? (int)(wsy->numel() / (2 * Ci)) : 0, sums.data_ptr<float>(),
                      s.data_ptr<float>(), (int)Co, (int)Ci, cur_stream()));
}

void gram_colsum_(const at::Tensor& y2, const at::Tensor& S, const at::Tensor& s) {
  GPU(y2); GPU(S); GPU(s); F32(S); F32(s);
  CK(y2.scalar_type() == at::kBFloat16 && y2.dim() == 2 && y2.stride(1) == 1 && y2.stride(0) % 8 == 0 &&
         ((uintptr_t)y2.data_ptr() % 16) == 0,
     "gram_colsum: y2 [M, Ci] bf16, 16-B aligned rows");
  const int64_t M = y2.size(0), Ci = y2.size(1);
  CK((Ci == 64 || Ci == 128 || Ci == 256) && M > 0 && y2.stride(0) >= Ci, "gram_colsum: Ci in {64, 128, 256}");
  CK(S.numel() == Ci * Ci && s.numel() == Ci && ((uintptr_t)S.data_ptr() % 16) == 0, "gram_colsum: S [Ci, Ci], s [Ci]");
  CK(S.device() == y2.device() && s.device() == y2.device(), "gram_colsum: y2, S and s on one device");
  at::DeviceGuard g(y2.device());
  static int cus_of[64] = {};
  const int dev = y2.device().index();
  int cus = dev >= 0 && dev < 64 ? cus_of[dev] : 0;
  if (!cus) {
    if (hipDeviceGetAttribute(&cus, hipDeviceAttributeMultiprocessorCount, dev) != hipSuccess || cus <= 0) cus = 256;
    if (dev >= 0 && dev < 64) cus_of[dev] = cus;
  }
  HIP_OK(gram_colsum(y2.data_ptr(), y2.stride(0), M, (int)Ci, S.data_ptr<float>(), s.data_ptr<float>(), cus, cur_stream()));
}

void bn_fold_fwd_stats_(const at::Tensor& w, const at::Tensor& S, const at::Tensor& s, int64_t M, const at::Tensor& ws) {
  GPU(w); GPU(S); GPU(s); GPU(ws); F32(S); F32(s); F32(ws);
  CK(S.device() == w.device() && s.device() == w.device() && ws.device() == w.device(),
     "bn_fold_fwd_stats: w, S, s and ws on one device");
  CK(w.scalar_type() == at::kBFloat16 && w.dim() == 2 && w.stride(1) == 1, "bn_fold_fwd_stats: w [Co, Ci] bf16");
  const int64_t Co = w.size(0), Ci = w.size(1);
  CK(Ci % 32 == 0 && Ci <= 256 && M > 0 && S.numel() == Ci * Ci && s.numel() == Ci && ws.numel() >= 2 * Co &&
         ((uintptr_t)S.data_ptr() % 16) == 0,
     "bn_fold_fwd_stats: Ci % 32 == 0, Ci <= 256, S [Ci, Ci], s [Ci], ws [>= 1, 2, Co]");
  at::DeviceGuard g(w.device());
  HIP_OK(bn_fold_fwd_stats(w.data_ptr(), w.stride(0), S.data_ptr<float>(), s.data_ptr<float>(), M, ws.data_ptr<float>(),
                           (int)Co, (int)Ci, cur_stream()));
}

void bn_fold_coef_(const at::Tensor& w, const at::Tensor& P, const at::Tensor& S, const at::Tensor& s,
                   const at::Tensor& coef, const at::Tensor& WA, const at::Tensor& WAt, const at::Tensor& Gm,
                   const at::Tensor& kv, const at::Tensor& dW) {
  GPU(w); F32(P); F32(S); F32(s); F32(coef); BF16(WA); BF16(WAt); BF16(Gm); F32(kv);
  CK(w.scalar_type() == at::kBFloat16 && w.dim() == 2 && w.stride(1) == 1, "bn_fold_coef: w [Co, Ci] bf16");
  const int64_t Co = w.size(0), Ci = w.size(1);
  CK(Co % 128 == 0 && Ci % 64 == 0, "bn_fold_coef: Co % 128, Ci % 64");
  CK(P.numel() == Co * Ci && S.numel() == Ci * Ci && s.numel() == Ci && coef.numel() >= 3 * Co && WA.numel() == Co * Ci &&
         WAt.numel() == Co * Ci && Gm.numel() == Ci * Ci && kv.numel() == Ci,
     "bn_fold_coef: shapes");
  CK(dW.is_cuda() && dW.scalar_type() == at::kFloat && dW.dim() == 2 && dW.size(0) == Co && dW.size(1) == Ci &&
         dW.stride(1) == 1 && dW.stride(0) >= Ci,
     "bn_fold_coef: dW [Co, Ci] fp32");
  at::DeviceGuard g(w.device());
  HIP_OK(bn_fold_coef(w.data_ptr(), w.stride(0), P.data_ptr<float>(), S.data_ptr<float>(), s.data_ptr<float>(),
                      coef.data_ptr<float>(), WA.data_ptr(), WAt.data_ptr(), Gm.data_ptr(), kv.data_ptr<float>(),
                      dW.data_ptr<float>(), dW.stride(0), (int)Co, (int)Ci, cur_stream()));
}

void bn_bwd_dx_(const at::Tensor& dy, const at::Tensor& x, c10::optional<at::Tensor> y,
                c10::optional<at::Tensor> scale, c10::optional<at::Tensor> shift, const at::Tensor& coef,
                const at::Tensor& dx, c10::optional<at::Tensor> dres, int64_t C, int64_t mode) {
  GPU(dy); BF16(dy); BF16(x); BF16(dx); F32(coef);
  CK(dy.numel() == x.numel() && dx.numel() == x.numel() && x.numel() % C == 0 && C % 8 == 0, "bn_bwd_dx: shapes");
  CK(coef.numel() >= 3 * C, "bn_bwd_dx: coef size");
  if (mode == 1) { CK(y.has_value(), "mode 1 needs y"); BF16(*y); CK(y->numel() == x.numel(), "bn_bwd_dx: y shape"); }
  if (mode == 3) CK(y.has_value() && y->scalar_type() == at::kByte && y->numel() >= x.numel() / 8,
                    "mode 3 needs the uint8 bit mask of bn_apply");
  CK(mode >= 0 && mode <= 3, "bn_bwd_dx: mode");
  if (mode == 2) { CK(scale.has_value() && shift.has_value(), "mode 2 needs scale/shift"); F32(*scale); F32(*shift); }
  if (dres) { BF16(*dres); CK(dres->numel() == x.numel(), "bn_bwd_dx: dres shape"); }
  at::DeviceGuard g(x.device());
  HIP_OK(bn_bwd_dx(dy.data_ptr(), x.data_ptr(), optr<const void>(y), optr<const float>(scale),
                   optr<const float>(shift), coef.data_ptr<float>(), dx.data_ptr(), optr<void>(dres), x.numel() / C,
                   (int)C, (int)mode, cur_stream()));
}

void bn_bwd_dx_red_(const at::Tensor& dy, const at::Tensor& x, c10::optional<at::Tensor> y,
                    c10::optional<at::Tensor> scale, c10::optional<at::Tensor> shift, const at::Tensor& coef,
                    const at::Tensor& dx, int64_t C, int64_t mode, const at::Tensor& x2, const at::Tensor& mean2,
                    const at::Tensor& ws2) {
  GPU(dy); BF16(dy); BF16(x); BF16(dx); F32(coef); BF16(x2); F32(mean2); F32(ws2);
  CK(dy.numel() == x.numel() && dx.numel() == x.numel() && x2.numel() == x.numel() && x.numel() % C == 0 && C % 8 == 0,
     "bn_bwd_dx_red: shapes");
  CK(coef.numel() >= 3 * C && mean2.numel() >= C, "bn_bwd_dx_red: coef / mean2 size");
  CK(ws2.numel() >= (int64_t)bn_partial_rows(x.numel() / C, (int)C) * 2 * C, "bn_bwd_dx_red: workspace too small");
  if (mode == 1) { CK(y.has_value(), "mode 1 needs y"); BF16(*y); CK(y->numel() == x.numel(), "bn_bwd_dx_red: y shape"); }
  if (mode == 3) CK(y.has_value() && y->scalar_type() == at::kByte && y->numel() >= x.numel() / 8,
                    "mode 3 needs the uint8 bit mask of bn_apply");
  CK(mode >= 0 && mode <= 3, "bn_bwd_dx_red: mode");
  if (mode == 2) { CK(scale.has_value() && shift.has_value(), "mode 2 needs scale/shift"); F32(*scale); F32(*shift); }
  at::DeviceGuard g(x.device());
  HIP_OK(bn_bwd_dx(dy.data_ptr(), x.data_ptr(), optr<const void>(y), optr<const float>(scale),
                   optr<const float>(shift), coef.data_ptr<float>(), dx.data_ptr(), nullptr, x.numel() / C, (int)C,
                   (int)mode, cur_stream(), x2.data_ptr(), mean2.data_ptr<float>(), ws2.data_ptr<float>()));
}

void pool3s2_bn_bwd_(const at::Tensor& dy, const at::Tensor& am, const at::Tensor& x, const at::Tensor& scale,
                     const at::Tensor& shift, const at::Tensor& mean, const at::Tensor& coef_or_ws,
                     c10::optional<at::Tensor> dx, int64_t k) {
  GPU(dy); BF16(dy); BF16(x); F32(scale); F32(shift); F32(mean); F32(coef_or_ws);
  CK(dy.dim() == 4 && x.dim() == 4 && dy.size(0) == x.size(0) && dy.size(3) == x.size(3) && dy.is_contiguous() &&
     x.is_contiguous(), "pool3s2_bn_bwd: NHWC dy / x");
  CK(am.scalar_type() == at::kByte && am.numel() == dy.numel() && am.is_contiguous(), "pool3s2_bn_bwd: argmax bytes");
  const int N = (int)x.size(0), H = (int)x.size(1), W = (int)x.size(2), C = (int)x.size(3);
  const int Ho = (int)dy.size(1), Wo = (int)dy.size(2);
  CK(pool3s2_bn_bwd_ok(N, H, W, C, Ho, Wo, (int)k), "pool3s2_bn_bwd: 3x3 / 2 / pad-1 (k = 3) or 2x2 / 2 (k = 2) pool, ",
     "C % 8 == 0, C <= 2048");
  CK(scale.numel() >= C && shift.numel() >= C && mean.numel() >= C, "pool3s2_bn_bwd: per-channel vectors");
  if (dx) {
    BF16(*dx);
    CK(dx->numel() == x.numel() && dx->is_contiguous() && coef_or_ws.numel() >= 3 * C, "pool3s2_bn_bwd: dx / coef");
  } else {
    CK(coef_or_ws.numel() % (2 * C) == 0 && coef_or_ws.numel() / (2 * C) <= 16384, "pool3s2_bn_bwd: ws [S][2][C]");
  }
  at::DeviceGuard g(x.device());
  HIP_OK(pool3s2_bn_bwd(dy.data_ptr(), am.data_ptr<uint8_t>(), x.data_ptr(), scale.data_ptr<float>(),
                        shift.data_ptr<float>(), mean.data_ptr<float>(), dx ? coef_or_ws.data_ptr<float>() : nullptr,
                        dx ? nullptr : coef_or_ws.data_ptr<float>(), (int)(coef_or_ws.numel() / (2 * C)),
                        dx ? dx->data_ptr() : nullptr, N, H, W, C, Ho, Wo,
                        cur_stream(), (int)k));
}

void maxpool_fwd_(const at::Tensor& x, const at::Tensor& y, const at::Tensor& am, int64_t kh, int64_t kw, int64_t sh,
                  int64_t sw, int64_t ph, int64_t pw, c10::optional<at::Tensor> scale, c10::optional<at::Tensor> shift) {
  GPU(x); BF16(x); BF16(y);
  CK(am.scalar_type() == at::kByte && am.is_contiguous(), "argmax must be uint8");
  CK(x.dim() == 4 && y.dim() == 4, "maxpool: NHWC tensors");
  const int N = x.size(0), H = x.size(1), W = x.size(2), C = x.size(3), Ho = y.size(1), Wo = y.size(2);
  CK(C % 8 == 0 && y.size(0) == N && y.size(3) == C && am.numel() == y.numel(), "maxpool: shapes");
  CK(kh * kw <= 256, "maxpool: window too large for byte argmax");
  at::DeviceGuard g(x.device());
  CK(scale.has_value() == shift.has_value(), "maxpool: scale and shift together");
  if (scale) {
    F32(*scale); F32(*shift);
    CK(scale->numel() == C && shift->numel() == C && scale->is_contiguous() && shift->is_contiguous() &&
           ((uintptr_t)scale->data_ptr() % 16) == 0 && ((uintptr_t)shift->data_ptr() % 16) == 0,
       "maxpool: per-channel scale / shift [C], 16-B aligned");
  }
  HIP_OK(maxpool_fwd(x.data_ptr(), y.data_ptr(), am.data_ptr<uint8_t>(), N, H, W, C, Ho, Wo, kh, kw, sh, sw, ph, pw,
                     cur_stream(), optr<const float>(scale), optr<const float>(shift)));
}

void maxpool_bwd_(const at::Tensor& dy, const at::Tensor& am, const at::Tensor& dx, int64_t kh, int64_t kw, int64_t sh,
                  int64_t sw, int64_t ph, int64_t pw) {
  GPU(dy); BF16(dy); BF16(dx);
  const int N = dx.size(0), H = dx.size(1), W = dx.size(2), C = dx.size(3), Ho = dy.size(1), Wo = dy.size(2);
  CK(C % 8 == 0 && dy.size(3) == C && am.numel() == dy.numel(), "maxpool_bwd: shapes");
  at::DeviceGuard g(dy.device());
  HIP_OK(maxpool_bwd(dy.data_ptr(), am.data_ptr<uint8_t>(), dx.data_ptr(), N, H, W, C, Ho, Wo, kh, kw, sh, sw, ph, pw,
                     cur_stream()));
}

void avgpool_fwd_(const at::Tensor& x, const at::Tensor& y) {
  GPU(x); BF16(x); BF16(y);
  CK(x.dim() == 4, "avgpool: NHWC");
  const int N = x.size(0), HW = x.size(1) * x.size(2), C = x.size(3);
  CK(C % 8 == 0 && y.numel() == (int64_t)N * C, "avgpool: shapes");
  at::DeviceGuard g(x.device());
  HIP_OK(avgpool_global_fwd(x.data_ptr(), y.data_ptr(), N, HW, C, cur_stream()));
}

void avgpool_bwd_(const at::Tensor& dy, const at::Tensor& dx) {
  GPU(dy); BF16(dy); BF16(dx);
  const int N = dx.size(0), HW = dx.size(1) * dx.size(2), C = dx.size(3);
  CK(C % 8 == 0 && dy.numel() == (int64_t)N * C, "avgpool_bwd: shapes");
  at::DeviceGuard g(dy.device());
  HIP_OK(avgpool_global_bwd(dy.data_ptr(), dx.data_ptr(), N, HW, C, cur_stream()));
}

void softmax_xent_(const at::Tensor& logits, c10::optional<at::Tensor> labels, c10::optional<at::Tensor> probs,
                   c10::optional<at::Tensor> loss_rows, c10::optional<at::Tensor> dlogits, double grad_scale, double smoothing,
                   int64_t ignore_index, c10::optional<at::Tensor> grad_scale_dev, c10::optional<at::Tensor> loss_out,
                   double out_scale, int64_t zrows) {
  GPU(logits);
  CK(logits.dim() == 2 && logits.stride(1) == 1 && logits.stride(0) >= logits.size(1),
     "softmax_xent: logits [B,K] with unit column stride");
  const bool bf = logits.scalar_type() == at::kBFloat16;
  CK(bf || logits.scalar_type() == at::kFloat, "softmax_xent: logits bf16/fp32");
  const int B = logits.size(0), K = logits.size(1);
  CK(loss_rows.has_value() || loss_out.has_value(), "softmax_xent: loss_rows and/or loss_out");
  if (loss_rows) { F32(*loss_rows); CK(loss_rows->numel() == B, "loss_rows size"); }
  const int64_t nz = zrows > 0 ? (B + zrows - 1) / zrows : 1;
  if (loss_out) { F32(*loss_out); CK(loss_out->numel() == nz && nz <= 64 && B <= 4096, "softmax_xent: loss_out [B / zrows <= 64], B <= 4096 (one workgroup)"); }
  CK(zrows == 0 || loss_out.has_value(), "softmax_xent: zrows needs loss_out");
  CK((labels.has_value()) != (probs.has_value()), "exactly one of labels/probs");
  if (labels) CK(labels->scalar_type() == at::kLong && labels->numel() == B, "labels int64 [B]");
  if (probs) { F32(*probs); CK(probs->numel() == (int64_t)B * K, "probs [B,K]"); }
  const long ld = logits.stride(0);
  if (dlogits)
    CK(dlogits->scalar_type() == logits.scalar_type() && dlogits->dim() == 2 && dlogits->size(0) == B &&
           dlogits->stride(0) == ld && dlogits->stride(1) == 1,
       "dlogits: same layout as logits");
  if (grad_scale_dev) { F32(*grad_scale_dev); CK(grad_scale_dev->numel() == 1 && grad_scale_dev->is_cuda(), "grad_scale_dev: one fp32 on the GPU"); }
  at::DeviceGuard g(logits.device());
  HIP_OK(softmax_xent(logits.data_ptr(), bf ? 1 : 0, optr<const int64_t>(labels), optr<const float>(probs),
                      optr<float>(loss_rows), optr<void>(dlogits), B, K, ld, (float)grad_scale, (float)smoothing,
                      (int)ignore_index, cur_stream(), optr<const float>(grad_scale_dev), optr<float>(loss_out),
                      (float)out_scale, (int)zrows));
}

void label_count_inv_(const at::Tensor& labels, int64_t ignore_index, const at::Tensor& inv) {
  GPU(labels); F32(inv);
  CK(labels.scalar_type() == at::kLong && labels.is_contiguous() && inv.numel() == 1, "label_count_inv: int64 labels, inv [1]");
  at::DeviceGuard g(labels.device());
  HIP_OK(label_count_inv(labels.data_ptr<int64_t>(), labels.numel(), (int)ignore_index, inv.data_ptr<float>(), cur_stream()));
}

void rows_sum_scaled_(const at::Tensor& rows, double scale, c10::optional<at::Tensor> dev, const at::Tensor& out) {
  GPU(rows); F32(rows); F32(out);
// ... 260 lines not shown
    const long bytes = (long)d.numel() * (long)d.element_size();
    CK((long)s.numel() * (long)s.element_size() >= bytes * nbs[q], "batch_fetch: shard smaller than nbatch batches");
    bc.src[q] = s.data_ptr();
    bc.dst[q] = d.data_ptr();
    bc.bytes[q] = bytes;
    bc.nbatch[q] = nbs[q];
  }
  at::DeviceGuard g(ctr.device());
  HIP_OK(batch_fetch(bc, (int)srcs.size(), ctr.data_ptr<int>(), cur_stream()));
}
void step_record_(const at::Tensor& loss, c10::optional<at::Tensor> hist, const at::Tensor& ctr,
                  c10::optional<at::Tensor> steps, c10::optional<at::Tensor> ts) {
  F32(loss);
  const int64_t R = loss.numel();
  CK(loss.is_cuda() && loss.is_contiguous() && R >= 1 && R <= 64, "step_record: 1..64 fp32 losses on the GPU");
  CK(ctr.is_cuda() && ctr.scalar_type() == at::kInt && ctr.numel() == 1 && ctr.device() == loss.device(),
     "step_record: int32 step counter on the loss device");
  if (hist) {
    F32(*hist);
    CK(hist->device() == loss.device() && hist->is_contiguous() && (R == 1 || (hist->dim() == 2 && hist->size(0) == R)),
       "step_record: history [cap] (or [R, cap] for R losses) on the loss device");
  }
  if (steps) CK(steps->is_cuda() && steps->scalar_type() == at::kInt && steps->numel() == R &&
                    steps->device() == loss.device(), "step_record: int32 steps [R] on the loss device");
  if (ts) { F32(*ts); CK(ts->is_cuda() && ts->numel() == R && ts->device() == loss.device(), "step_record: ts [R]"); }
  at::DeviceGuard g(loss.device());
  HIP_OK(step_record(loss.data_ptr<float>(), optr<float>(hist), hist ? (int)(hist->numel() / R) : 0, ctr.data_ptr<int>(),
                     cur_stream(), (int)R, steps ? steps->data_ptr<int>() : nullptr, optr<float>(ts)));
}
void opt_stack_step_(int64_t opt, const at::Tensor& w, const at::Tensor& g, c10::optional<at::Tensor> s1,
                     c10::optional<at::Tensor> s2, c10::optional<at::Tensor> w16, const at::Tensor& ctr,
                     const at::Tensor& steps, c10::optional<at::Tensor> ts, double lr, double mu, double b1, double b2,
                     double eps, double wd, int64_t amode) {
  F32(w); F32(g);
  CK(w.is_cuda() && w.dim() == 2 && w.is_contiguous() && g.sizes() == w.sizes() && g.is_contiguous() &&
         g.device() == w.device(), "opt_stack_step: w, g [R, n] contiguous on one GPU");
  const int64_t R = w.size(0), n = w.size(1);
  for (auto* t : {&s1, &s2}) if (*t) { F32(**t); CK((*t)->sizes() == w.sizes() && (*t)->is_contiguous() &&
                                                       (*t)->device() == w.device(), "opt_stack_step: state [R, n]"); }
  if (w16) CK(w16->scalar_type() == at::kBFloat16 && w16->sizes() == w.sizes() && w16->is_contiguous() &&
                  w16->device() == w.device(), "opt_stack_step: bf16 copy [R, n]");
  CK(ctr.is_cuda() && ctr.scalar_type() == at::kInt && ctr.numel() == 1 && ctr.device() == w.device(),
     "opt_stack_step: int32 step counter");
  CK(steps.is_cuda() && steps.scalar_type() == at::kInt && steps.numel() == R && steps.device() == w.device(),
     "opt_stack_step: int32 steps [R]");
  if (ts) { F32(*ts); CK(ts->numel() == R && ts->device() == w.device(), "opt_stack_step: ts [R]"); }
  at::DeviceGuard dg(w.device());
  HIP_OK(opt_stack_step((int)opt, w.data_ptr<float>(), g.data_ptr<float>(), optr<float>(s1), optr<float>(s2),
                        w16 ? w16->data_ptr() : nullptr, n, (int)R, ctr.data_ptr<int>(), steps.data_ptr<int>(),
                        optr<float>(ts), (float)lr, (float)mu, (float)b1, (float)b2, (float)eps, (float)wd, (int)amode,
                        cur_stream()));
}
void prob_xent_(const at::Tensor& p, c10::optional<at::Tensor> labels, c10::optional<at::Tensor> target,
                const at::Tensor& loss_rows, const at::Tensor& dp, double eps, double scale, int64_t ignore_index) {
  GPU(p); F32(p); F32(loss_rows); F32(dp);
  CK(p.dim() == 2 && dp.sizes() == p.sizes() && loss_rows.numel() == p.size(0), "prob_xent: p [B, K], dp, loss_rows [B]");
  CK((labels.has_value()) != (target.has_value()), "prob_xent: labels OR target");
  if (labels) CK(labels->scalar_type() == at::kLong && labels->is_contiguous() && labels->numel() == p.size(0),
                 "prob_xent: int64 labels [B]");
  if (target) { F32(*target); CK(target->sizes() == p.sizes(), "prob_xent: target [B, K]"); }
  at::DeviceGuard g(p.device());
  HIP_OK(prob_xent(p.data_ptr<float>(), labels ? labels->data_ptr<int64_t>() : nullptr, optr<const float>(target),
                   loss_rows.data_ptr<float>(), dp.data_ptr<float>(), (int)p.size(0), (int)p.size(1), (float)eps,
                   (float)scale, (int)ignore_index, cur_stream()));
}
void slab_reduce_(const at::Tensor& ws, int64_t splits, const at::Tensor& c, int64_t M, int64_t N, int64_t ldc,
                  double beta) {
  GPU(ws); F32(ws); GPU(c);
  CK(c.scalar_type() == at::kFloat, "slab_reduce: fp32 c");
  CK(splits >= 1 && ws.numel() >= splits * M * N && ldc >= N && c.numel() >= (M - 1) * ldc + N,
     "slab_reduce: ws [splits, M, N], c [M, ldc]");
  at::DeviceGuard g(ws.device());
  HIP_OK(slab_reduce(ws.data_ptr<float>(), (int)splits, c.data_ptr<float>(), M, (int)N, ldc, (float)beta, cur_stream()));
}
void mse_fwd_bwd_(const at::Tensor& pred, const at::Tensor& target, const at::Tensor& loss, const at::Tensor& grad) {
  F32(pred); F32(target); F32(loss); F32(grad);
  CK(pred.is_cuda() && pred.numel() == target.numel() && grad.numel() == pred.numel() && loss.numel() == 1,
     "mse: pred / target / grad sizes");
  at::DeviceGuard gd(pred.device());
  HIP_OK(mse_fwd_bwd(pred.data_ptr<float>(), target.data_ptr<float>(), pred.numel(), loss.data_ptr<float>(),
                     grad.data_ptr<float>(), cur_stream()));
}
void etl_minmax_(const at::Tensor& x, const at::Tensor& y, double o_min, double scale, double n_min) {
  CK(x.is_cuda() && x.scalar_type() == at::kDouble && y.scalar_type() == at::kDouble && x.is_contiguous() &&
         y.is_contiguous() && x.numel() == y.numel(), "etl_minmax: contiguous fp64 x / y of equal size");
  at::DeviceGuard gd(x.device());
  HIP_OK(etl_minmax(x.data_ptr<double>(), y.data_ptr<double>(), x.numel(), o_min, scale, n_min, cur_stream()));
}
void etl_one_hot_(const at::Tensor& labels, const at::Tensor& y, const at::Tensor& bad) {
  CK(labels.is_cuda() && labels.scalar_type() == at::kLong && labels.is_contiguous(), "etl_one_hot: int64 labels");
  CK(y.scalar_type() == at::kDouble && y.dim() == 2 && y.size(0) == labels.numel() && y.is_contiguous(),
     "etl_one_hot: y [n, K] fp64");
  CK(bad.scalar_type() == at::kInt && bad.numel() == 1, "etl_one_hot: int32 flag");
  at::DeviceGuard gd(y.device());
  HIP_OK(etl_one_hot(labels.data_ptr<int64_t>(), y.data_ptr<double>(), labels.numel(), (int)y.size(1),
                     bad.data_ptr<int>(), cur_stream()));
}
void etl_argmax_(const at::Tensor& x, const at::Tensor& out) {
  CK(x.is_cuda() && x.scalar_type() == at::kDouble && x.dim() == 2 && x.stride(1) == 1, "etl_argmax: x [rows, K] fp64");
  CK(out.scalar_type() == at::kLong && out.numel() == x.size(0), "etl_argmax: out int64 [rows]");
  at::DeviceGuard gd(x.device());
  HIP_OK(etl_argmax(x.data_ptr<double>(), x.size(0), (int)x.size(1), x.stride(0), out.data_ptr<int64_t>(),
                    cur_stream()));
}
void step_tick_(const at::Tensor& t) {
  F32(t);
  CK(t.is_cuda() && t.numel() == 1, "step counter: one fp32 element on the GPU");
  at::DeviceGuard gd(t.device());
  HIP_OK(step_tick(t.data_ptr<float>(), cur_stream()));
}
void adagrad_step_(const at::Tensor& w, const at::Tensor& g, const at::Tensor& acc, c10::optional<at::Tensor> w16,
                   double lr, double eps, double wd, double gscale) {
  OPT_CHECK(w, g);
  F32(acc);
  CK(acc.numel() == w.numel(), "adagrad: state size");
  if (w16) BF16(*w16);
  at::DeviceGuard gd(w.device());
  HIP_OK(adagrad_step(w.data_ptr<float>(), g.data_ptr<float>(), acc.data_ptr<float>(), optr<void>(w16), w.numel(),
                      (float)lr, (float)eps, (float)wd, (float)gscale, cur_stream()));
}
void rmsprop_step_(const at::Tensor& w, const at::Tensor& g, const at::Tensor& acc, c10::optional<at::Tensor> w16,
                   double lr, double rho, double eps, double wd, double gscale) {
  OPT_CHECK(w, g);
  F32(acc);
  CK(acc.numel() == w.numel(), "rmsprop: state size");
  if (w16) BF16(*w16);
  at::DeviceGuard gd(w.device());
  HIP_OK(rmsprop_step(w.data_ptr<float>(), g.data_ptr<float>(), acc.data_ptr<float>(), optr<void>(w16), w.numel(),
                      (float)lr, (float)rho, (float)eps, (float)wd, (float)gscale, cur_stream()));
}
void sumsq_(const at::Tensor& x, const at::Tensor& out) {
  GPU(x); F32(x); F32(out);
  CK(x.numel() % 4 == 0, "sumsq: multiple of 4");
  at::DeviceGuard gd(x.device());
  HIP_OK(sumsq_f32(x.data_ptr<float>(), x.numel(), out.data_ptr<float>(), cur_stream()));
}

}

void register_ops(py::module& m) {
  m.attr("BN_SHARDS") = (int)kBnShards;
  m.def("bn_stats", &bn_stats_);
  m.def("splitk_finalize", &splitk_finalize_, py::arg("ws"), py::arg("y"), py::arg("C"), py::arg("bias"), py::arg("relu"),
        py::arg("stats"), py::arg("splits") = 0, py::arg("brows") = 0, py::arg("zbias") = 0);
  m.def("bn_partial_rows", &bn_partial_rows_);
  m.def("bn_finalize", &bn_finalize_);
  m.def("bn_apply", &bn_apply_, py::arg("x"), py::arg("scale"), py::arg("shift"), py::arg("resid"), py::arg("y"),
        py::arg("C"), py::arg("relu"), py::arg("mask") = py::none(), py::arg("res_scale") = py::none(),
        py::arg("res_shift") = py::none());
  m.def("bn_bwd_reduce", &bn_bwd_reduce_);
  m.def("bn_bwd_finalize", &bn_bwd_finalize_);
  m.def("bn_fold_sums", &bn_fold_sums_);
  m.def("bn_fold_coef", &bn_fold_coef_);
  m.def("gram_colsum", &gram_colsum_);
  m.def("bn_fold_fwd_stats", &bn_fold_fwd_stats_);
  m.def("bn_bwd_dx", &bn_bwd_dx_);
  m.def("bn_bwd_dx_red", &bn_bwd_dx_red_);
  m.def("pool3s2_bn_bwd", &pool3s2_bn_bwd_, py::arg("dy"), py::arg("am"), py::arg("x"), py::arg("scale"),
        py::arg("shift"), py::arg("mean"), py::arg("coef_or_ws"), py::arg("dx"), py::arg("k") = 3);
  m.def("pool3s2_bn_bwd_ok", [](int64_t N, int64_t H, int64_t W, int64_t C, int64_t Ho, int64_t Wo, int64_t k) {
    return pool3s2_bn_bwd_ok((int)N, (int)H, (int)W, (int)C, (int)Ho, (int)Wo, (int)k);
  });
  m.def("maxpool_fwd", &maxpool_fwd_, "NHWC max pool (byte argmax); optional fused BN affine + ReLU on load",
        py::arg("x"), py::arg("y"), py::arg("am"), py::arg("kh"), py::arg("kw"), py::arg("sh"), py::arg("sw"),
        py::arg("ph"), py::arg("pw"), py::arg("scale") = py::none(), py::arg("shift") = py::none());
  m.def("maxpool_bwd", &maxpool_bwd_);
  m.def("avgpool_fwd", &avgpool_fwd_);
  m.def("avgpool_bwd", &avgpool_bwd_);
  m.def("softmax_xent", &softmax_xent_, "fused softmax cross-entropy", py::arg("logits"), py::arg("labels"),
        py::arg("probs"), py::arg("loss_rows"), py::arg("dlogits"), py::arg("grad_scale"), py::arg("smoothing"),
        py::arg("ignore_index"), py::arg("grad_scale_dev") = py::none(), py::arg("loss_out") = py::none(),
        py::arg("out_scale") = 1.0, py::arg("zrows") = 0);
  m.def("label_count_inv", &label_count_inv_);
  m.def("rows_sum_scaled", &rows_sum_scaled_);
  m.def("pad_cols_bf16", &pad_cols_bf16_, "zero-padded copy of a row-strided bf16 view");
  m.def("zero_ranges", &zero_ranges_, "zero up to 8 contiguous device buffers in one launch", py::arg("buffers"));
  m.def("gather_bf16", &gather_bf16_, "out[i] = src[idx[i]] (0 where idx < 0)", py::arg("src"), py::arg("idx"),
        py::arg("out"), py::arg("src_extent"));
  m.def("scatter_add_f32", &scatter_add_f32_, "dst[idx[i]] += src[i] (idx injective, < 0 skipped)", py::arg("src"),
        py::arg("idx"), py::arg("dst"), py::arg("dst_extent"));
  m.def("scale_bf16_dev", &scale_bf16_dev_);
  m.def("cast_f32_bf16", &cast_f32_bf16_);
  m.def("sum_rows_bf16", &sum_rows_bf16_);
  m.def("cast_bf16_f32", &cast_bf16_f32_);
  m.def("relu_bwd", &relu_bwd_);
  m.def("add_bf16", &add_bf16_);
  m.def("bias_grad", &bias_grad_, py::arg("dy"), py::arg("db"), py::arg("N"), py::arg("accumulate"),
        py::arg("relu_y") = py::none(), py::arg("relu_dx") = py::none(), py::arg("zcount") = 1, py::arg("zdb") = 0);
  m.def("transpose_bf16", &transpose_bf16_);
  m.def("im2col", &im2col_);
  m.def("normalize_u8", &normalize_u8_);
  m.def("s2d_pad", &s2d_pad_);
  m.def("sgd_step", &sgd_step_);
  m.def("adam_step", &adam_step_, "fused Adam/AdamW", py::arg("w"), py::arg("g"), py::arg("m"), py::arg("v"),
        py::arg("w16"), py::arg("lr"), py::arg("b1"), py::arg("b2"), py::arg("eps"), py::arg("wd"), py::arg("mode"),
        py::arg("bc1"), py::arg("bc2"), py::arg("gscale"), py::arg("tstep") = py::none(),
        py::arg("tick_ctr") = py::none());
  m.def("step_tick", &step_tick_);
  m.def("mse_fwd_bwd", &mse_fwd_bwd_);
  m.def("prob_xent", &prob_xent_);
  m.def("slab_reduce", &slab_reduce_);
  m.def("commit_delta", &commit_delta_);
  m.def("commit_apply", &commit_apply_);
  m.def("commit_replicas", &commit_replicas_, "one commit round over R co-located replicas", py::arg("ws"),
        py::arg("w16s"), py::arg("scales"), py::arg("center"), py::arg("sum") = py::none(), py::arg("elastic") = false,
        py::arg("mode") = 0);
  m.def("batch_fetch", &batch_fetch_);
  m.def("step_record", &step_record_, py::arg("loss"), py::arg("hist"), py::arg("ctr"), py::arg("steps") = py::none(),
        py::arg("ts") = py::none());
  m.def("opt_stack_step", &opt_stack_step_);
  m.def("etl_minmax", &etl_minmax_);
  m.def("etl_one_hot", &etl_one_hot_);
  m.def("etl_argmax", &etl_argmax_);
  m.def("adagrad_step", &adagrad_step_);
  m.def("rmsprop_step", &rmsprop_step_);
  m.def("sumsq", &sumsq_);
}
```

### distributeddeeplearningspark_amd/ops/fused_blocks.py

```python
from __future__ import annotations

import weakref

import torch

from . import conv as CV
from . import determinism as _det
from . import gemm as G
from . import zpad as ZP
from ._native import C
from .norm import new_stats_workspace, partials_workspace, pool_epoch
from .streams import on_grad_stream


class _ConvBNState:

    __slots__ = ("g", "yc", "y", "mean", "invstd", "scale", "shift", "mode", "mask", "pre_reduced", "fold", "gram",
                 "__weakref__")

    def __init__(self):
        self.pre_reduced = None
        self.fold = False
        self.gram = None


_PRODUCERS: dict = {}


def _register_output(y, unit, st):
    _PRODUCERS[y.data_ptr()] = (weakref.ref(y), unit, weakref.ref(st))
    if len(_PRODUCERS) > 4096:
        for k in [k for k, v in _PRODUCERS.items() if v[0]() is None]:
            del _PRODUCERS[k]


def _producer_of(x):
    e = _PRODUCERS.get(x.data_ptr())
    if e is None or e[0]() is not x:
        return None
    st = e[2]()
    return None if st is None else (e[1], st)


def _bn_forward(layer_bn, yc, stats, resid, relu, training, mask=None, apply=True, res_affine=None):
    Cc = yc.shape[-1]
    M = yc.numel() // Cc
    dev = yc.device
    bn = layer_bn
    gamma = None if bn.gamma is None else bn.gamma.master
    beta = None if bn.beta is None else bn.beta.master
    rm, rv = bn._states["moving_mean"], bn._states["moving_variance"]
    scale, shift, mean, invstd = torch.empty(4, Cc, dtype=torch.float32, device=dev).unbind(0)
    if stats is None:
        stats = partials_workspace(M, Cc, dev)
        C().bn_stats(yc, stats, Cc)
    C().bn_finalize(stats, M, Cc, gamma, beta, bn.epsilon, 1.0 - bn.momentum, rm, rv, mean, invstd, scale, shift)
    if not apply:
        return None, mean, invstd, scale, shift
    y = torch.empty_like(yc)
    rs, rt = res_affine if res_affine is not None else (None, None)
    C().bn_apply(yc, scale, shift, resid, y, Cc, relu, mask, rs, rt)
    return y, mean, invstd, scale, shift


def convbn_forward(unit, x, resid=None, relu=True, apply=True, res_affine=None):
    conv, bn = unit.conv, unit.bn
    N, H, W, Ci = x.shape
    kh, kw = conv.kernel_size
    p = conv.padding if isinstance(conv.padding, tuple) else (kh // 2, kw // 2)
    g = CV.geometry(N, H, W, Ci, conv.filters, kh, kw, conv.strides, p, conv.dilation_rate)
    stats = new_stats_workspace(conv.filters, x.device)
    yc = CV.conv_fwd_native(x, conv.kernel.data, g, stats=stats)
    st = _ConvBNState()
    st.g, st.yc = g, yc
    bits = relu and resid is not None
    st.mask = torch.empty(-(-yc.numel() // 32) * 4, dtype=torch.uint8, device=yc.device) if bits else None
    st.y, st.mean, st.invstd, st.scale, st.shift = _bn_forward(bn, yc, stats, resid, relu, True, st.mask, apply,
                                                               res_affine)
    st.mode = 0 if not relu else (2 if resid is None else (3 if bits else 1))
    return st


def bn_backward(unit, st, dy, want_dres, red2=None, dy_mask=None, reduced=None):
    bn = unit.bn
    Cc = st.yc.shape[-1]
    M = st.yc.numel() // Cc
    mode = st.mode
    y = st.y if st.mode == 1 else (st.mask if st.mode == 3 else None)
    if dy_mask is not None:
        if st.mode != 0:
            raise ValueError("bn_backward: dy_mask applies to a BN without its own ReLU")
        mode, y = 3, dy_mask
    pre, st.pre_reduced = st.pre_reduced, None
    if reduced is not None:
        ws = reduced
    elif pre is not None and not pre[2] and _same_tensor(pre[1], dy):
        ws = pre[0]
    else:
        ws = partials_workspace(M, Cc, dy.device)
        C().bn_bwd_reduce(dy, st.yc, y, st.scale, st.shift, st.mean, ws, Cc, mode)
    coef = torch.empty(3 * Cc, dtype=torch.float32, device=dy.device)
    C().bn_bwd_finalize(ws, M, Cc, None if bn.gamma is None else bn.gamma.master, st.mean, st.invstd,
                        None if bn.gamma is None else bn.gamma.grad, None if bn.beta is None else bn.beta.grad, coef)
    dyc = torch.empty_like(dy)
    dres = torch.empty_like(dy) if want_dres else None
    if red2 is not None:
        if dres is not None:
            raise ValueError("bn_backward: red2 replaces dres")
        C().bn_bwd_dx_red(dy, st.yc, y, st.scale, st.shift, coef, dyc, Cc, mode, red2[0], red2[1], red2[2])
    else:
        C().bn_bwd_dx(dy, st.yc, y, st.scale, st.shift, coef, dyc, dres, Cc, mode)
    if bn.grad_hook is not None:
        bn.grad_hook()
    return dyc, dres


def conv_backward(unit, st, dyc, x, need_dx, resid=None, resid_mask=None, bnr=None, rsub=None):
    conv = unit.conv
    with on_grad_stream(dyc.device, dyc, x, default=False):
        CV.conv_wgrad_native(dyc, x, st.g, conv.kernel.grad)
    dx = None
    if need_dx:
        dx = CV.conv_dgrad_native(dyc, conv.kernel.data, st.g, resid=resid, resid_mask=resid_mask, bnr=bnr, rsub=rsub)
    if conv.grad_hook is not None:
        conv.grad_hook()
    return dx


class _BottleneckFn(torch.autograd.Function):
    @staticmethod
    def forward(ctx, x, anchor, block):
        ctx.prev = _producer_of(x) if _FUSE_BNR else None
        x = x.contiguous()
        s_down = convbn_forward(block.down, x, relu=False, apply=False) if block.down is not None else None
        sc = s_down.yc if s_down is not None else x
        s1 = convbn_forward(block.c1, x, relu=True)
        s2 = convbn_forward(block.c2, s1.y, relu=True)
        g3 = _fold_fwd_geometry(block.c3, s2.y) if s_down is None else None
        if g3 is not None:
            s3 = _convbn3_fold_forward(block.c3, s2.y, sc, g3)
        else:
            s3 = convbn_forward(block.c3, s2.y, resid=sc, relu=True,
                                res_affine=None if s_down is None else (s_down.scale, s_down.shift))
        s3.fold = s_down is None and s3.mode == 3 and _fold_gate(s3.g)
        ctx.block, ctx.states = block, (s_down, s1, s2, s3)
        ctx.save_for_backward(x)
        ctx.needs_dx = ctx.needs_input_grad[0]
        _register_output(s3.y, block.c3, s3)
        return s3.y

    @staticmethod
    def backward(ctx, dout):
        (x,) = ctx.saved_tensors
        b = ctx.block
        s_down, s1, s2, s3 = ctx.states
        dout = dout.contiguous()
        masked_sc = s_down is None and s3.mode == 3 and s1.g.is_pointwise
        fuse_down = _FUSE_DOWN and s_down is not None and s3.mode == 3 and s_down.mode == 0
        ws_d = None
        pre3 = s3.pre_reduced
        fold = (_FOLD_BN3 and s3.fold and not _det.enabled() and pre3 is not None and pre3[2]
                and _same_tensor(pre3[1], dout) and b.c3.bn.gamma is not None)
        if fold:
            s3.pre_reduced = None
            bnr2 = _bnr_mode2(s2, dout.device)
            d2 = _fold_bn3_backward(b.c3, s3, s2, dout, pre3[0], bnr2)
            dsc = dout
        elif s3.yc is None:
            _recompute_yc(b.c3, s3, s2)
            d3c, dsc = bn_backward(b.c3, s3, dout, want_dres=not masked_sc)
        elif fuse_down:
            Cd = s_down.yc.shape[-1]
            ws_d = partials_workspace(s_down.yc.numel() // Cd, Cd, dout.device)
            d3c, dsc = bn_backward(b.c3, s3, dout, False, red2=(s_down.yc, s_down.mean, ws_d))
        else:
            d3c, dsc = bn_backward(b.c3, s3, dout, want_dres=not masked_sc)
        if not fold:
            bnr2 = _bnr_mode2(s2, dout.device)
            d2 = conv_backward(b.c3, s3, d3c, s2.y, True, bnr=bnr2)
        _take_reduced(s2, bnr2, d2)
        d2c, _ = bn_backward(b.c2, s2, d2, False)
        bnr1 = _bnr_mode2(s1, dout.device)
        d1 = conv_backward(b.c2, s2, d2c, s1.y, True, bnr=bnr1)
        _take_reduced(s1, bnr1, d1)
        d1c, _ = bn_backward(b.c1, s1, d1, False)
        rsub = None
        if s_down is not None:
            if fuse_down:
                ddc, _ = bn_backward(b.down, s_down, dout, False, dy_mask=s3.mask, reduced=ws_d)
            else:
                ddc, _ = bn_backward(b.down, s_down, dsc, False)
            gd = s_down.g
            if (_HALF_RES_SC and ctx.needs_dx and s1.g.is_pointwise and gd.KH == 1 and gd.KW == 1
                    and (gd.sh, gd.sw) == (2, 2) and (gd.ph, gd.pw) == (0, 0)):
                wd = b.down.conv.kernel.data
                dsc = G.linear_dgrad(ddc.view(gd.M, gd.Co), wd.view(gd.Co, gd.Ci))
                rsub = (gd.H, gd.W)
                conv_backward(b.down, s_down, ddc, x, False)
            else:
                dsc = conv_backward(b.down, s_down, ddc, x, ctx.needs_dx)
        bnr = None
        if ctx.needs_dx and ctx.prev is not None and ctx.prev[1].mode == 3 and not _det.enabled():
            pst = ctx.prev[1]
            premask = bool(_FOLD_BN3 and pst.fold and s1.g.is_pointwise)
            if premask or pst.yc is not None:
                bnr = {"x": pst.yc, "mask": pst.mask, "mean": pst.mean,
                       "ws": new_stats_workspace(pst.g.Co, dout.device), "premask": premask}
        if _TEST_MUTATION is not None and _TEST_MUTATION[0] == "drop_shortcut" and _TEST_MUTATION[1] in (None, b.name):
            masked_sc, dsc, rsub = False, None, None
        if masked_sc:
            dx = conv_backward(b.c1, s1, d1c, x, ctx.needs_dx, resid=dout, resid_mask=s3.mask, bnr=bnr)
        else:
            dx = conv_backward(b.c1, s1, d1c, x, ctx.needs_dx, resid=dsc, bnr=bnr, rsub=rsub)
        if bnr is not None and bnr.get("done"):
            ctx.prev[1].pre_reduced = (bnr["ws"], dx, bool(bnr["premask"]))
        ctx.states = ctx.prev = None
        return dx, None, None



_FUSE_BNR = True
_TEST_MUTATION = None
_FUSE_BNR_INNER = True
_HALF_RES_SC = True
_FUSE_DOWN = True
_FUSE_STEM_BWD = True
_STEM_PARTIALS = 2048


def _bnr_mode2(st, device):
    if not _FUSE_BNR_INNER or st.mode != 2 or _det.enabled():
        return None
    return {"x": st.yc, "scale": st.scale, "shift": st.shift, "mean": st.mean,
            "ws": new_stats_workspace(st.yc.shape[-1], device)}


def _take_reduced(st, bnr, d):
    if bnr is not None and bnr.get("done"):
        st.pre_reduced = (bnr["ws"], d, False)


_FOLD_BN3 = True
_FOLD_MIN_ELEMS = 1 << 26


def _fold_gate(g) -> bool:
    return g.is_pointwise and g.Ci % 64 == 0 and g.Co % 128 == 0 and g.M * g.Co >= _FOLD_MIN_ELEMS


_FOLD_BN3_FWD = True


def _fold_fwd_geometry(unit, x2):
    if not (_FOLD_BN3 and _FOLD_BN3_FWD) or _det.enabled() or x2.device.type != "cuda":
        return None
    if unit.bn.gamma is None:
        return None
    conv = unit.conv
    N, H, W, Ci = x2.shape
    kh, kw = conv.kernel_size
    if (kh, kw) != (1, 1):
        return None
    p = conv.padding if isinstance(conv.padding, tuple) else (0, 0)
    g = CV.geometry(N, H, W, Ci, conv.filters, kh, kw, conv.strides, p, conv.dilation_rate)
    if not (_fold_gate(g) and G.stream_colscale_ok(g.Co, g.Ci) and x2.is_contiguous()):
        return None
    return g


def _convbn3_fold_forward(unit, x2, resid, g):
    conv, bn = unit.conv, unit.bn
    M, Co, Ci = g.M, g.Co, g.Ci
    dev = x2.device
    x2m = x2.view(M, Ci)
    ps = new_stats_workspace(-(-(Ci * Ci + Ci) // 64), dev).view(-1)
    S, s = ps[: Ci * Ci].view(Ci, Ci), ps[Ci * Ci : Ci * Ci + Ci]
    C().gram_colsum(x2m, S, s)
    stats = new_stats_workspace(Co, dev)
    w = conv.kernel.data.view(Co, Ci)
    C().bn_fold_fwd_stats(w, S, s, M, stats)
    gamma = None if bn.gamma is None else bn.gamma.master
    beta = None if bn.beta is None else bn.beta.master
    rm, rv = bn._states["moving_mean"], bn._states["moving_variance"]
    scale, shift, mean, invstd = torch.empty(4, Co, dtype=torch.float32, device=dev).unbind(0)
    C().bn_finalize(stats, M, Co, gamma, beta, bn.epsilon, 1.0 - bn.momentum, rm, rv, mean, invstd, scale, shift)
    st = _ConvBNState()
    st.g, st.yc = g, None
    st.mask = torch.empty(-(-M * Co // 32) * 4, dtype=torch.uint8, device=dev)
    y = torch.empty((g.N, g.H, g.W, Co), dtype=torch.bfloat16, device=dev)
    G.linear_fwd(x2m, w, bias=shift, relu=True, out=y.view(M, Co), resid=resid.view(M, Co), colscale=scale,
                 relu_mask_out=st.mask)
    st.y, st.mean, st.invstd, st.scale, st.shift, st.mode = y, mean, invstd, scale, shift, 3
    st.gram = (S, s, pool_epoch(dev))
    return st


def _recompute_yc(unit, s3, s2):
    geo = s3.g
    w = unit.conv.kernel.data.view(geo.Co, geo.Ci)
    yc = torch.empty((geo.N, geo.H, geo.W, geo.Co), dtype=torch.bfloat16, device=s2.y.device)
    G.linear_fwd(s2.y.view(geo.M, geo.Ci), w, out=yc.view(geo.M, geo.Co))
    s3.yc = yc


def fold_conv_bn_backward(w, gw, g2, y2, ws_g, mean, invstd, gamma, dgamma, dbeta, bnr2=None, out=None, gram=None):
    M, Co = g2.shape
    Ci = y2.shape[1]
    dev = g2.device
    if gram is not None:
        S, s = gram
        P = new_stats_workspace(-(-(Co * Ci) // 64), dev).view(-1)[: Co * Ci].view(Co, Ci)
        G.linear_wgrad(g2, y2, P)
        wsy = None
    else:
        ps = new_stats_workspace(-(-(Co * Ci + Ci * Ci + Ci) // 64), dev).view(-1)
        P, S = ps[: Co * Ci].view(Co, Ci), ps[Co * Ci : Co * Ci + Ci * Ci].view(Ci, Ci)
        s = ps[Co * Ci + Ci * Ci : Co * Ci + Ci * Ci + Ci]
        G.linear_wgrad(g2, y2, P)
        G.linear_wgrad(y2, y2, S)
        wsy = partials_workspace(M, Ci, dev)
        C().bn_stats(y2, wsy, Ci)
    f32 = torch.empty(5 * Co + Ci, dtype=torch.float32, device=dev)
    sums, coef, kv = f32[: 2 * Co], f32[2 * Co : 5 * Co], f32[5 * Co :]
    C().bn_fold_sums(w, P, ws_g, mean, wsy, sums, s)
    C().bn_bwd_finalize(sums, M, Co, gamma, mean, invstd, dgamma, dbeta, coef)
    b16 = torch.empty(2 * Co * Ci + Ci * Ci, dtype=torch.bfloat16, device=dev)
    WA, WAt, Gm = b16[: Co * Ci].view(Co, Ci), b16[Co * Ci : 2 * Co * Ci].view(Ci, Co), b16[2 * Co * Ci :].view(Ci, Ci)
    C().bn_fold_coef(w, P, S, s, coef, WA, WAt, Gm, kv, gw)
    r = G.linear_fwd(y2, Gm, bias=kv)
    if out is None:
        out = torch.empty((M, Ci), dtype=torch.bfloat16, device=dev)
    G.linear_dgrad(g2, WA, out=out, resid=r, bnr=bnr2, wt=WAt)
    return out, sums.view(2, Co)


def _fold_bn3_backward(unit, s3, s2, g, ws_g, bnr2):
    conv, bn = unit.conv, unit.bn
    geo = s3.g
    M, Co, Ci = geo.M, geo.Co, geo.Ci
    d2 = torch.empty((geo.N, geo.H, geo.W, Ci), dtype=torch.bfloat16, device=g.device)
    gram = None
    if s3.gram is not None and s3.gram[2] == pool_epoch(g.device):
        gram = s3.gram[:2]
    fold_conv_bn_backward(conv.kernel.data.view(Co, Ci), conv.kernel.grad.view(Co, Ci), g.view(M, Co), s2.y.view(M, Ci),
                          ws_g, s3.mean, s3.invstd, bn.gamma.master, bn.gamma.grad,
                          None if bn.beta is None else bn.beta.grad, bnr2=bnr2, out=d2.view(M, Ci), gram=gram)
    if bn.grad_hook is not None:
        bn.grad_hook()
    if conv.grad_hook is not None:
        conv.grad_hook()
    return d2


def _same_tensor(a, b) -> bool:
    return (a.data_ptr() == b.data_ptr() and a.shape == b.shape and a.stride() == b.stride()
            and a._version == b._version)


def bottleneck(block, x, anchor):
    return _BottleneckFn.apply(x, anchor, block)


def convbn_relu(unit, x, anchor, relu=True):
    if not x.requires_grad and _stem_s2d_ok(unit.conv, x.shape[-1]):
        return _StemS2DFn.apply(x, anchor, unit, relu)
    return _ConvBNFn.apply(x, anchor, unit, relu)


_STEM_S2D = True
_STEM_POOL = True


def _stem_s2d_ok(conv, Ci) -> bool:
    return (_STEM_S2D and Ci <= 4 and tuple(conv.kernel_size) == (7, 7)
            and tuple(conv.strides) == (2, 2) and tuple(conv.dilation_rate) == (1, 1)
            and (conv.padding == (3, 3) or conv.padding == 3 or conv.padding == "same"))


def _s2d_weight(w):
    Co, _, _, Cc = w.shape
    w8 = torch.nn.functional.pad(w, (0, 0, 0, 1, 0, 1))
    w4 = w8.view(Co, 4, 2, 4, 2, Cc).permute(0, 1, 3, 2, 4, 5).reshape(Co, 4, 4, 4 * Cc)
    return torch.nn.functional.pad(w4, (0, 16 - 4 * Cc)).contiguous()


def _s2d_weight_grad(g4, Cc):
    Co = g4.shape[0]
    g = g4[..., : 4 * Cc].reshape(Co, 4, 4, 2, 2, Cc).permute(0, 1, 3, 2, 4, 5).reshape(Co, 8, 8, Cc)
    return g[:, :7, :7, :]


_S2D_TABLES: dict = {}


def _s2d_table(t):
    key = (tuple(t.shape), tuple(t.stride()), str(t.device))
    hit = _S2D_TABLES.get(key)
    if hit is None:
        offs = torch.zeros((), dtype=torch.int64)
        for d, (n, st) in enumerate(zip(t.shape, t.stride())):
            offs = offs.unsqueeze(-1) + torch.arange(n, dtype=torch.int64) * st
        Co, _, _, Cc = t.shape
        o8 = torch.nn.functional.pad(offs, (0, 0, 0, 1, 0, 1), value=-1)
        o4 = o8.view(Co, 4, 2, 4, 2, Cc).permute(0, 1, 3, 2, 4, 5).reshape(Co, 4, 4, 4 * Cc)
        tab = torch.nn.functional.pad(o4, (0, 16 - 4 * Cc), value=-1).contiguous()
        hit = _S2D_TABLES[key] = (tab.to(torch.int32).to(t.device), int(offs.max()) + 1)
    return hit


def _s2d_weight_dev(w):
    if not (w.is_cuda and w.dtype == torch.bfloat16):
        return _s2d_weight(w)
    tab, ext = _s2d_table(w)
    out = torch.empty(tab.shape, dtype=w.dtype, device=w.device)
    C().gather_bf16(w, tab, out, ext)
    return out


def _s2d_weight_grad_into(conv, g, dyc, xs, Cc):
    gw = conv.kernel.grad
    tmp = torch.empty((g.Co, 4, 4, 16), dtype=torch.float32, device=dyc.device)
    if not gw.is_cuda:
        tmp.zero_()
        CV.conv_wgrad_native(dyc, xs, g, tmp)
        gw.add_(_s2d_weight_grad(tmp, Cc))
        return
    C().zero_ranges([tmp])
    CV.conv_wgrad_native(dyc, xs, g, tmp)
    tab, ext = _s2d_table(gw)
    C().scatter_add_f32(tmp, tab, gw, ext)


class _StemPoolFn(torch.autograd.Function):

    @staticmethod
    def forward(ctx, x, anchor, unit, k, s, p):
        x = x.contiguous()
        N, H, W, Cc = x.shape
        conv = unit.conv
        Ho, Wo = (H + 6 + 1) // 2, (W + 6 + 1) // 2
        xs = torch.empty((N, Ho, Wo, 16), dtype=x.dtype, device=x.device)
        C().s2d_pad(x, xs, 3)
        w4 = _s2d_weight_dev(conv.kernel.data.detach())
        g = CV.geometry(N, Ho, Wo, 16, conv.filters, 4, 4, (1, 1), (0, 0), (1, 1))
        stats = new_stats_workspace(conv.filters, x.device)
        yc = CV.conv_fwd_native(xs, w4, g, stats=stats)
        st = _ConvBNState()
        st.g, st.yc = g, yc
        st.y, st.mean, st.invstd, st.scale, st.shift = _bn_forward(unit.bn, yc, stats, None, True, True, apply=False)
        st.mode = 2
        _, Hc, Wc, Co = yc.shape
        Hp, Wp = (Hc + 2 * p - k) // s + 1, (Wc + 2 * p - k) // s + 1
        y = torch.empty((N, Hp, Wp, Co), dtype=yc.dtype, device=yc.device)
        am = torch.empty((N, Hp, Wp, Co), dtype=torch.uint8, device=yc.device)
        C().maxpool_fwd(yc, y, am, k, k, s, s, p, p, st.scale, st.shift)
        ctx.unit, ctx.st, ctx.cc, ctx.pool = unit, st, Cc, (k, s, p)
        ctx.save_for_backward(xs, am)
        return y

    @staticmethod
    def backward(ctx, dy):
        xs, am = ctx.saved_tensors
        unit, st = ctx.unit, ctx.st
        k, s, p = ctx.pool
        dy = dy.contiguous()
        N, H, W, Co = st.yc.shape
        if _FUSE_STEM_BWD and (k, s, p) == (3, 2, 1) and C().pool3s2_bn_bwd_ok(N, H, W, Co, dy.shape[1], dy.shape[2], 3):
            bn = unit.bn
            M = N * H * W
            ws = torch.empty((_STEM_PARTIALS, 2, Co), dtype=torch.float32, device=dy.device)
            C().pool3s2_bn_bwd(dy, am, st.yc, st.scale, st.shift, st.mean, ws, None)
            coef = torch.empty(3 * Co, dtype=torch.float32, device=dy.device)
            C().bn_bwd_finalize(ws, M, Co, None if bn.gamma is None else bn.gamma.master, st.mean, st.invstd,
                                None if bn.gamma is None else bn.gamma.grad, None if bn.beta is None else bn.beta.grad,
                                coef)
            dyc = torch.empty_like(st.yc)
            C().pool3s2_bn_bwd(dy, am, st.yc, st.scale, st.shift, st.mean, coef, dyc)
            if bn.grad_hook is not None:
                bn.grad_hook()
        else:
            d = torch.empty_like(st.yc)
            C().maxpool_bwd(dy, am, d, k, k, s, s, p, p)
            dyc, _ = bn_backward(unit, st, d, False)
        conv = unit.conv
        g = st.g
        with on_grad_stream(dy.device, dyc, xs, default=False):
            _s2d_weight_grad_into(conv, g, dyc, xs, ctx.cc)
        if conv.grad_hook is not None:
            conv.grad_hook()
        ctx.st = None
        return None, None, None, None, None, None


def stem_pool(unit, x, anchor, k=3, s=2, p=1):
    if (not _STEM_POOL or x.requires_grad or not _stem_s2d_ok(unit.conv, x.shape[-1])
            or unit.conv.filters % 8):
        return None
    return _StemPoolFn.apply(x, anchor, unit, k, s, p)


class _StemS2DFn(torch.autograd.Function):

    @staticmethod
    def forward(ctx, x, anchor, unit, relu):
# ... 146 lines not shown
```

### distributeddeeplearningspark_amd/ops/gemm.py

```python
from __future__ import annotations

import math

import torch

from . import determinism as _det
from ._native import C

KC, RC, KC_GATHER, RC_GATHER, RC_TAPS, KC_GATHER8, RC_GATHER8 = 0, 1, 2, 3, 4, 5, 6
EPI_BF16, EPI_F32, EPI_F32_ATOMIC = 0, 1, 2
TILE256 = 4
TILE_STREAM = 5
TILE_CONV3 = 6
_TILES = {0: (128, 128), 1: (128, 64), 2: (64, 128), 3: (64, 64), TILE256: (256, 256), TILE_STREAM: (64, 256),
          TILE_CONV3: (224, 128)}
_ONE_PER_CU = (TILE256,)
_CU = 256
import os as _os

_USE256 = "auto"


_USE_STREAM = "1"
_TILE_FILL = 2.0
# ... 28 lines not shown
    if outmap is not None or aux is not None or drop_p or int(relu) > ACT_RELU or beta:
        return False
    if M < 16384 or not stream_panel(N, K) or lda % 8 or ldc % 8 or (resid is not None and ldr % 4):
        return False
    return True


def use_tile256(M: int, N: int, K: int, a_mode: int, b_mode: int, epi: int) -> bool:
    if _USE256 == "0" or a_mode > RC or b_mode > RC or K % 64 or M < 128 or N < 128:
        return False
    tiles = math.ceil(M / 256) * math.ceil(N / 256)
    if _USE256 == "1":
        return tiles >= _CU // 2
    return epi == EPI_BF16 and tiles >= 4 * _CU and K >= 4096


def choose_tile(M: int, N: int, bn_cap: int = 128) -> int:
    bn = 128 if (N > 64 and bn_cap >= 128) else 64
    bm = 128 if M > 64 else 64
    if bm == 128 and bn == 128 and math.ceil(M / 128) * math.ceil(N / 128) < _TILE_FILL * _CU:
        bm = 64 if M <= N else 128
        bn = 64 if M > N else 128
    for tid, (tm, tn) in _TILES.items():
        if (tm, tn) == (bm, bn):
            return tid
    return 3


def choose_split(M: int, N: int, K: int, tile: int, allow: bool, rounds: float | None = None) -> int:
    kfull = max(64, math.ceil(K / 64) * 64)
    if not allow:
        return kfull
    bm, bn = _TILES[tile]
    tiles = math.ceil(M / bm) * math.ceil(N / bn)
    per_cu = 1 if tile in _ONE_PER_CU else 2
    if tiles >= per_cu * _CU or K < 1024:
        return kfull
    splits = min(math.ceil((rounds or _SPLIT_ROUNDS) * per_cu * _CU / tiles), max(1, K // 512))
    ks = math.ceil(K / splits / 64) * 64
    return max(64, ks)


def gemm(a, b, c, M, N, K, a_mode, b_mode, lda, ldb, ldc, epi, *, alpha=1.0, beta=0.0, bias=None, resid=None,
         ldr=0, relu=False, geom=None, outmap=None, b_kdiv=0, b_tap_stride=0, stats=None, tile=None, k_split=None,
         bn_cap=128, aux=None, drop_p=0.0, drop_seed=0, split_rounds=None, resid_mask=None, bnr=None, rsub=None,
         slabs=None, defer_slabs=False, colscale=None, relu_mask_out=None):
    if colscale is not None or relu_mask_out is not None:
        if (tile not in (None, TILE_STREAM) or colscale is None or resid is None or alpha != 1.0
                or not stream_colscale_ok(N, K)):
            raise ValueError("gemm: colscale / relu_mask_out need the streaming kernel's forward form with a residual "
                             "(the column scale takes alpha's place: alpha == 1)")
        tile = TILE_STREAM
    if tile is None:
        if use_stream(M, N, K, a_mode, b_mode, epi, lda, ldc, outmap=outmap, aux=aux, drop_p=drop_p, relu=relu,
                      beta=beta, resid=resid, ldr=ldr):
            tile = TILE_STREAM
        elif outmap is None and bnr is None and use_tile256(M, N, K, a_mode, b_mode, epi):
            tile = TILE256
        elif epi == EPI_F32 and a_mode <= RC and b_mode <= RC and big_wgrad(M, N, K) and _SPLITK_SLABS_MODE != "0":
            tile = 0
        else:
            tile = choose_tile(M, N, bn_cap)
    if (k_split is None and tile == 0 and epi == EPI_F32 and a_mode == RC and b_mode == RC and big_wgrad(M, N, K)
            and _SPLITK_SLABS_MODE == "auto" and slabs is not False):
        k_split = slab_split(M, N, K)
    if k_split is None:
        k_split = choose_split(M, N, K, tile, allow=(epi != EPI_BF16), rounds=split_rounds)
    split_stride = 0
    if k_split < K and epi != EPI_F32 and _det.enabled():
        k_split = max(64, math.ceil(K / 64) * 64)
    out, slab_beta = c, None
    if epi == EPI_F32 and k_split < K:
        if beta not in (0.0, 1.0):
            raise ValueError("split-K fp32 gemm supports beta in {0,1} (beta=0 needs a zeroed C)")
        auto = _SPLITK_SLABS_MODE == "auto" and tile == 0 and big_wgrad(M, N, K) and math.ceil(K / k_split) <= 32
        use_slabs = (_det.enabled() or _SPLITK_SLABS or auto) if slabs is None else (slabs or _det.enabled())
        if tile in (0, 1, 2, 3) + _ONE_PER_CU and use_slabs:
            splits = math.ceil(K / k_split)
            out, split_stride, slab_beta, ldc_c = _slab_workspace(splits * M * N, c.device), M * N, beta, ldc
            ldc, beta = N, 0.0
        else:
            epi = EPI_F32_ATOMIC
    if bnr is not None:
        if tile in _ONE_PER_CU:
            raise ValueError("bnr: not on the 256-row kernels")
        stats = bnr["ws"]
    C().gemm(a, b, out, M, N, K, a_mode, b_mode, lda, ldb, ldc, epi, tile, k_split, alpha, beta, bias, resid, ldr,
             int(relu), geom, outmap, b_kdiv, b_tap_stride, stats, aux, float(drop_p), int(drop_seed), resid_mask,
             None if bnr is None else bnr.get("x"), None if bnr is None else bnr.get("mask"),
             None if bnr is None else bnr.get("mean"), *(rsub or (0, 0)), None if bnr is None else bnr.get("scale"),
             None if bnr is None else bnr.get("shift"), split_stride,
             bnr_premask=bool(bnr is not None and bnr.get("premask")), colscale=colscale, relu_mask_out=relu_mask_out)
    if split_stride:
        if defer_slabs:
            return out, math.ceil(K / k_split)
        C().slab_reduce(out, math.ceil(K / k_split), c, M, N, ldc_c, float(slab_beta))
    return c


_SPLITK_SLABS_MODE = _os.environ.get("DDL_SPLITK_SLABS", "auto")
_SPLITK_SLABS = _SPLITK_SLABS_MODE == "1"


def big_wgrad(M: int, N: int, K: int) -> bool:
    return M * N >= (1 << 19) and K >= 8192 and M >= 512 and N >= 512


def slab_split(M: int, N: int, K: int) -> int:
    tiles = math.ceil(M / 128) * math.ceil(N / 128)
    splits = max(1, min((3 * _CU) // tiles, K // 1152))
    return max(64, math.ceil(K / splits / 64) * 64)
_SLAB_WS: dict = {}


def _slab_workspace(n, device):
    from . import scope as _scope

    key = (str(device), torch.cuda.current_stream(device).cuda_stream if device.type == "cuda" else 0, _scope.tag())
    ws = _SLAB_WS.get(key)
    if ws is None or ws.numel() < n:
        ws = _SLAB_WS[key] = torch.empty(max(n, 1 << 20), dtype=torch.float32, device=device)
    return ws[:n]


ACT_NONE, ACT_RELU, ACT_GELU, ACT_GELU_BWD = 0, 1, 2, 3


def linear_fwd(x2, w, bias=None, relu=False, out=None, resid=None, stats=None, act=None, aux=None, drop_p=0.0,
               drop_seed=0, colscale=None, relu_mask_out=None):
    M, K = x2.shape
    N = w.shape[0]
    if out is None:
        out = torch.empty((M, N), dtype=torch.bfloat16, device=x2.device)
    act = (ACT_RELU if relu else ACT_NONE) if act is None else act
    tiles = math.ceil(M / 64) * math.ceil(N / 64)
    if colscale is not None or relu_mask_out is not None:
        return gemm(x2, w, out, M, N, K, KC, KC, x2.stride(0), w.stride(0), out.stride(0), EPI_BF16, bias=bias, relu=act,
                    resid=resid, ldr=(resid.stride(0) if resid is not None else 0), stats=stats, aux=aux, drop_p=drop_p,
                    drop_seed=drop_seed, colscale=colscale, relu_mask_out=relu_mask_out)
    if (K >= 1024 and tiles <= _SKINNY_FWD_TILES and act <= ACT_RELU and resid is None and stats is None and aux is None
            and not drop_p and N % 8 == 0 and out.is_contiguous() and x2.device.type == "cuda" and not _det.enabled()):
        ws = splitk_workspace(M, N, x2.device)
        splits = max(2, min(math.ceil(256 / tiles), K // 256))
        r = gemm(x2, w, ws, M, N, K, KC, KC, x2.stride(0), w.stride(0), N, EPI_F32, tile=3,
                 k_split=math.ceil(K / splits / 64) * 64, defer_slabs=True)
        if isinstance(r, tuple):
            C().splitk_finalize(r[0], out, N, bias, act == ACT_RELU, None, r[1])
        else:
            C().splitk_finalize(ws, out, N, bias, act == ACT_RELU, None)
        return out
    return gemm(x2, w, out, M, N, K, KC, KC, x2.stride(0), w.stride(0), out.stride(0), EPI_BF16, bias=bias, relu=act,
                resid=resid, ldr=(resid.stride(0) if resid is not None else 0), stats=stats, aux=aux, drop_p=drop_p,
                drop_seed=drop_seed)


_SPLITK_WS = {}
_SKINNY_FWD_TILES = 16


def splitk_workspace(M, N, device):
    from . import scope as _scope

    key = (M, N, str(device) + _scope.tag())
    ws = _SPLITK_WS.get(key)
    if ws is None:
        ws = _SPLITK_WS[key] = torch.zeros((M, N), dtype=torch.float32, device=device)
    return ws


_SPLITK_DGRAD = True


def linear_dgrad(dy, w, out=None, resid=None, gelu_pre=None, stats=None, resid_mask=None, bnr=None, rsub=None,
                 wt=None):
    M, N = dy.shape
    K = w.shape[1]
    if out is None:
        out = torch.empty((M, K), dtype=torch.bfloat16, device=dy.device)
    act = ACT_GELU_BWD if gelu_pre is not None else ACT_NONE
    ldr = resid.stride(0) if resid is not None else 0
    tiles = math.ceil(M / 64) * math.ceil(K / 64)
    if (_SPLITK_DGRAD and not _det.enabled() and gelu_pre is None and resid is None and rsub is None and N >= 4096 and tiles <= 1024 and K % 8 == 0
            and out.is_contiguous() and out.dtype == torch.bfloat16 and dy.device.type == "cuda"):
        ws = splitk_workspace(M, K, dy.device)
        t128 = math.ceil(M / 128) * math.ceil(K / 128)
        if 2 * t128 <= 3 * _CU:
            splits = max(2, min((3 * _CU) // t128, N // 1152))
            r = gemm(dy, w, ws, M, K, N, KC, RC, dy.stride(0), w.stride(0), K, EPI_F32, tile=0,
                     k_split=math.ceil(N / splits / 64) * 64, defer_slabs=True, slabs=True)
        else:
            splits = max(2, min(math.ceil(2048 / tiles), N // 512))
            r = gemm(dy, w, ws, M, K, N, KC, RC, dy.stride(0), w.stride(0), K, EPI_F32, tile=3,
                     k_split=math.ceil(N / splits / 64) * 64, defer_slabs=True)
        if isinstance(r, tuple):
            C().splitk_finalize(r[0], out, K, None, False, stats, r[1])
        else:
            C().splitk_finalize(ws, out, K, None, False, stats)
        return out
    if M >= _WT_MIN_M and not use_stream(M, K, N, KC, RC, EPI_BF16, dy.stride(0), out.stride(0), aux=gelu_pre,
                                         relu=act, resid=resid, ldr=ldr):
        wt = transpose(w) if wt is None else wt
        fb = _bnr_plain_ok(bnr, stats, resid, gelu_pre, K)
        gemm(dy, wt, out, M, K, N, KC, KC, dy.stride(0), wt.stride(0), out.stride(0), EPI_BF16, resid=resid,
             ldr=ldr, relu=act, aux=gelu_pre, stats=stats, resid_mask=resid_mask, rsub=rsub, bnr=bnr if fb else None)
        if fb:
            bnr["done"] = True
        return out
    if (bnr is not None and stats is None
            and ("scale" not in bnr or (resid is None and rsub is None) or (rsub is None and (K, N) == (64, 256)))
            and use_stream(M, K, N, KC, RC, EPI_BF16, dy.stride(0), out.stride(0), aux=gelu_pre, relu=act,
                           resid=resid, ldr=ldr)):
        gemm(dy, w, out, M, K, N, KC, RC, dy.stride(0), w.stride(0), out.stride(0), EPI_BF16, resid=resid, ldr=ldr,
             relu=act, aux=gelu_pre, resid_mask=resid_mask, tile=TILE_STREAM, bnr=bnr, rsub=rsub)
        bnr["done"] = True
        return out
    fb = _bnr_plain_ok(bnr, stats, resid, gelu_pre, K) and not use_stream(
        M, K, N, KC, RC, EPI_BF16, dy.stride(0), out.stride(0), aux=gelu_pre, relu=act, resid=resid, ldr=ldr)
    gemm(dy, w, out, M, K, N, KC, RC, dy.stride(0), w.stride(0), out.stride(0), EPI_BF16, resid=resid,
         ldr=ldr, relu=act, aux=gelu_pre, stats=stats, resid_mask=resid_mask, rsub=rsub, bnr=bnr if fb else None)
    if fb:
        bnr["done"] = True
    return out


def _bnr_plain_ok(bnr, stats, resid, gelu_pre, ncols) -> bool:
    return (bnr is not None and stats is None and gelu_pre is None and ncols % 8 == 0
            and (bnr["x"].is_contiguous() if bnr.get("x") is not None else bool(bnr.get("premask")))
            and (resid is None or (resid.stride(0) % 4 == 0 and resid.data_ptr() % 8 == 0)))


def transpose(w):
    R, Cc = w.shape
    if w.stride(1) != 1 or R % 8 or Cc % 8 or w.stride(0) % 8:
        return w.t().contiguous()
    if w.is_contiguous():
        from . import derived

        return derived.taps_transpose(w, (0,), (Cc, R))
    out = torch.empty((Cc, R), dtype=w.dtype, device=w.device)
    C().transpose_bf16(w, out)
    return out


def linear_wgrad(dy, x2, gw):
    M, N = dy.shape
    K = x2.shape[1]
    rounds = None if (big_wgrad(N, K, M) and _SPLITK_SLABS_MODE == "auto") else _LINEAR_WGRAD_ROUNDS
    return gemm(dy, x2, gw, N, K, M, RC, RC, dy.stride(0), x2.stride(0), gw.stride(0), EPI_F32, beta=1.0,
                split_rounds=rounds)


def matmul(a, b, trans_a=False, trans_b=False, out=None, alpha=1.0):
    M = a.shape[1] if trans_a else a.shape[0]
    K = a.shape[0] if trans_a else a.shape[1]
    N = b.shape[0] if trans_b else b.shape[1]
    if out is None:
        out = torch.empty((M, N), dtype=torch.bfloat16, device=a.device)
    a_mode = RC if trans_a else KC
    b_mode = KC if trans_b else RC
    return gemm(a, b, out, M, N, K, a_mode, b_mode, a.stride(0), b.stride(0), out.stride(0), EPI_BF16, alpha=alpha)
```

Measured before the change: 13260 images/sec.

## Fuse projection shortcut conv+BN into conv3 with a dual-product streaming GEMM

Adds a dual form of the streaming GEMM kernel that computes two K=64 products (conv3 and the downsample conv), applies each one's folded BN column scale and shift, adds them, and applies ReLU in one pass. This removes the separate downsample conv output and the residual read and write in the projection block's forward pass. The backward pass gets a path that skips the downsample conv's dx computation and a new kernel for exact column sums. The fused path only applies to the stage-1 projection block, where the input has 64 channels and the tensors are large. It relies on BN folding via Gram statistics, which adds extra stats passes over the input.

```diff
diff --git a/distributeddeeplearningspark_amd/csrc/bindings.cpp b/distributeddeeplearningspark_amd/csrc/bindings.cpp
--- a/distributeddeeplearningspark_amd/csrc/bindings.cpp
+++ b/distributeddeeplearningspark_amd/csrc/bindings.cpp
@@ -56,7 +56,9 @@
           c10::optional<at::Tensor> bnr_mean, int64_t rsub_h, int64_t rsub_w, c10::optional<at::Tensor> bnr_scale, c10::optional<at::Tensor> bnr_shift, int64_t split_stride,
           int64_t zcount, int64_t za, int64_t zb, int64_t zc, int64_t zbias, std::vector<int64_t> cls_tap0,
           std::vector<int64_t> cls_nt, std::vector<int64_t> cls_coff, bool bnr_premask,
-          c10::optional<at::Tensor> colscale, c10::optional<at::Tensor> relu_mask_out) {
+          c10::optional<at::Tensor> colscale, c10::optional<at::Tensor> relu_mask_out,
+          c10::optional<at::Tensor> a2, c10::optional<at::Tensor> b2, int64_t lda2, int64_t ldb2,
+          c10::optional<at::Tensor> colscale2, c10::optional<at::Tensor> bias2) {
   CHECK_CUDA(a);
   CHECK_CUDA(b);
   CHECK_CUDA(c);
@@ -235,7 +237,50 @@
     p.bnr_mask = bnr_mask->data_ptr<uint8_t>();
     p.bnr_premask = 1;
   }
-  if (colscale || relu_mask_out) {
+  const bool dual = a2 || b2 || colscale2 || bias2;
+  if (dual) {
+    TORCH_CHECK(tile == kTileStream && a2.has_value() && b2.has_value() && colscale.has_value() && colscale2.has_value() &&
+                    a_mode == OP_KC && b_mode == OP_KC && K == 64 && N % 128 == 0 && !resid && !resid_mask && !stats &&
+                    !bnr_x && !bnr_mask && !bnr_premask && rsub_h == 0 && alpha == 1.0 && !geom && !outmap && zcount <= 1 &&
+                    cls_nt.empty() && split_stride == 0,
+                "gemm: a second product (a2 / b2 / colscale2 / bias2) runs on the streaming kernel with K = 64 per "
+                "product, N % 128 == 0, K-contiguous operands and both column scales, without a residual, statistics, "
+                "a BN-backward reduction or alpha");
+    CHECK_CUDA(*a2);
+    CHECK_CUDA(*b2);
+    CHECK_BF16(*a2);
+    CHECK_BF16(*b2);
+    TORCH_CHECK(lda >= K && lda2 >= K && ldb >= K && ldb2 >= K && lda2 % 8 == 0 && ldb2 % 8 == 0 && ldc >= N &&
+                    ((uintptr_t)a2->data_ptr() % 16) == 0 && ((uintptr_t)b2->data_ptr() % 16) == 0,
+                "gemm: a2 / b2 leading dimensions (>= K, % 8) and 16-B alignment");
+    TORCH_CHECK(a.numel() >= (M - 1) * lda + K && a2->numel() >= (M - 1) * lda2 + K && b.numel() >= (N - 1) * ldb + K &&
+                    b2->numel() >= (N - 1) * ldb2 + K && c.numel() >= (M - 1) * ldc + N,
+                "gemm: an operand of the dual product is too small");
+    for (const auto* t : {&colscale, &colscale2}) {
+      CHECK_CUDA(**t);
+      CHECK_F32(**t);
+      TORCH_CHECK((*t)->is_contiguous() && (*t)->numel() >= N && ((uintptr_t)(*t)->data_ptr() % 16) == 0,
+                  "gemm: colscale / colscale2 [N] fp32, 16-B aligned");
+    }
+    p.colscale = colscale->data_ptr<float>();
+    p.colscale2 = colscale2->data_ptr<float>();
+    if (bias2) {
+      CHECK_CUDA(*bias2);
+      CHECK_F32(*bias2);
+      TORCH_CHECK(bias2->numel() >= N && (uintptr_t)bias2->data_ptr() % 16 == 0, "gemm: bias2 [N] fp32, 16-B aligned");
+      p.bias2 = bias2->data_ptr<float>();
+    }
+    p.a2 = a2->data_ptr();
+    p.b2 = b2->data_ptr();
+    p.lda2 = lda2;
+    p.ldb2 = ldb2;
+    if (relu_mask_out) {
+      TORCH_CHECK(relu_mask_out->is_cuda() && relu_mask_out->scalar_type() == at::kByte && relu_mask_out->is_contiguous() &&
+                      relu_mask_out->numel() >= ((M - 1) * ldc + N + 7) / 8,
+                  "gemm: relu_mask_out must be uint8 [M * ldc / 8]");
+      p.relu_mask_out = relu_mask_out->data_ptr<uint8_t>();
+    }
+  } else if (colscale || relu_mask_out) {
     TORCH_CHECK(tile == kTileStream && colscale.has_value() && resid.has_value() && b_mode == OP_KC && !stats && !bnr_x &&
                     !bnr_premask && rsub_h == 0 && alpha == 1.0,
                 "gemm: colscale / relu_mask_out run on the streaming kernel's forward form with a residual, without "
@@ -369,7 +414,9 @@
         py::arg("split_stride") = 0, py::arg("zcount") = 1, py::arg("za") = 0, py::arg("zb") = 0, py::arg("zc") = 0,
         py::arg("zbias") = 0, py::arg("cls_tap0") = std::vector<int64_t>{}, py::arg("cls_nt") = std::vector<int64_t>{},
         py::arg("cls_coff") = std::vector<int64_t>{}, py::arg("bnr_premask") = false,
-        py::arg("colscale") = py::none(), py::arg("relu_mask_out") = py::none());
+        py::arg("colscale") = py::none(), py::arg("relu_mask_out") = py::none(), py::arg("a2") = py::none(),
+        py::arg("b2") = py::none(), py::arg("lda2") = 0, py::arg("ldb2") = 0, py::arg("colscale2") = py::none(),
+        py::arg("bias2") = py::none());
   m.def("conv3x3_wgrad", &conv3x3_wgrad, "3x3 stride-1 weight gradient (halo kernel): gw += dW", py::arg("dy"),
         py::arg("x"), py::arg("gw"), py::arg("ws"), py::arg("splits"), py::arg("tpb"), py::arg("pp") = false);
   m.def("conv3x3_wgrad_plan", &conv3x3_wgrad_plan_py,
diff --git a/distributeddeeplearningspark_amd/csrc/include/ddl_gemm.h b/distributeddeeplearningspark_amd/csrc/include/ddl_gemm.h
--- a/distributeddeeplearningspark_amd/csrc/include/ddl_gemm.h
+++ b/distributeddeeplearningspark_amd/csrc/include/ddl_gemm.h
@@ -81,6 +81,10 @@
   long cls_coff[kMaxZCls];
   const float* colscale;
   uint8_t* relu_mask_out;
+  const void* a2; long lda2;
+  const void* b2; long ldb2;
+  const float* colscale2;
+  const float* bias2;
 };
 
 enum Activation : int { ACT_NONE = 0, ACT_RELU = 1, ACT_GELU = 2, ACT_GELU_BWD = 3 };
diff --git a/distributeddeeplearningspark_amd/csrc/include/ddl_ops.h b/distributeddeeplearningspark_amd/csrc/include/ddl_ops.h
--- a/distributeddeeplearningspark_amd/csrc/include/ddl_ops.h
+++ b/distributeddeeplearningspark_amd/csrc/include/ddl_ops.h
@@ -36,6 +36,8 @@
                  int rows, float* sums, float* s, int Co, int Ci, hipStream_t st);
 int bn_fold_coef(const void* w, long ldw, const float* P, const float* S, const float* s, const float* coef, void* WA,
                  void* WAt, void* Gm, float* kv, float* dW, long lddw, int Co, int Ci, hipStream_t st);
+int bn_fold_kv(const void* WA, const void* Gm, const float* sg, const float* s, long M, float* kv, int Co, int Ci,
+               hipStream_t st);
 int gram_colsum(const void* y2, long ld, long M, int Ci, float* S, float* s, int cus, hipStream_t st);
 int bn_fold_fwd_stats(const void* w, long ldw, const float* S, const float* s, long M, float* ws, int Co, int Ci,
                       hipStream_t st);
diff --git a/distributeddeeplearningspark_amd/csrc/kernels/bn_fold.hip b/distributeddeeplearningspark_amd/csrc/kernels/bn_fold.hip
--- a/distributeddeeplearningspark_amd/csrc/kernels/bn_fold.hip
+++ b/distributeddeeplearningspark_amd/csrc/kernels/bn_fold.hip
@@ -324,4 +324,39 @@
   return (int)hipGetLastError();
 }
 
-}
+namespace {
+
+constexpr int KVW = 16;
+__global__ __launch_bounds__(64 * KVW) void bn_fold_kv_kernel(const bf16_t* __restrict__ WA, const bf16_t* __restrict__ Gm,
+                                                               const float* __restrict__ sg, const float* __restrict__ s,
+                                                               double inv_m, float* __restrict__ kv, int Co, int Ci) {
+  __shared__ double red[KVW][64];
+  const int tx = threadIdx.x & 63, ty = threadIdx.x >> 6;
+  const int ci = blockIdx.x * 64 + tx;
+  double a = 0.0;
+  if (ci < Ci) {
+#pragma unroll 4
+    for (int co = ty; co < Co; co += KVW) a += (double)sg[co] * (double)bf2f(WA[(long)co * Ci + ci]);
+#pragma unroll 4
+    for (int cj = ty; cj < Ci; cj += KVW) a += (double)s[cj] * (double)bf2f(Gm[(long)cj * Ci + ci]);
+  }
+  red[ty][tx] = a;
+  __syncthreads();
+  if (ty == 0 && ci < Ci) {
+#pragma unroll
+    for (int j = 1; j < KVW; ++j) a += red[j][tx];
+    kv[ci] = (float)(-a * inv_m);
+  }
+}
+
+}
+
+int bn_fold_kv(const void* WA, const void* Gm, const float* sg, const float* s, long M, float* kv, int Co, int Ci,
+               hipStream_t st) {
+  if (Co <= 0 || Ci <= 0 || M <= 0) return (int)hipErrorInvalidValue;
+  hipLaunchKernelGGL(bn_fold_kv_kernel, dim3((Ci + 63) / 64), dim3(64 * KVW), 0, st, (const bf16_t*)WA, (const bf16_t*)Gm, sg,
+                     s, 1.0 / (double)M, kv, Co, Ci);
+  return (int)hipGetLastError();
+}
+
+}
diff --git a/distributeddeeplearningspark_amd/csrc/kernels/gemm_dispatch.hip b/distributeddeeplearningspark_amd/csrc/kernels/gemm_dispatch.hip
--- a/distributeddeeplearningspark_amd/csrc/kernels/gemm_dispatch.hip
+++ b/distributeddeeplearningspark_amd/csrc/kernels/gemm_dispatch.hip
@@ -15,6 +15,7 @@
   GemmParams p = p_in;
   p.group_m = 8;
   if ((p.colscale || p.relu_mask_out) && tile != kTileStream) return (int)hipErrorInvalidValue;
+  if ((p.a2 || p.b2 || p.colscale2 || p.bias2) && tile != kTileStream) return (int)hipErrorInvalidValue;
   if (p.bnr_premask && (!p.bnr_mask || !p.stats || p.bnr_scale)) return (int)hipErrorInvalidValue;
   if (p.bnr_premask && !p.bnr_x && tile != kTileStream && p.a_mode != OP_KC) return (int)hipErrorInvalidValue;
   if ((p.bnr_x || p.bnr_premask) && tile != kTileStream &&
diff --git a/distributeddeeplearningspark_amd/csrc/kernels/gemm_stream.hip b/distributeddeeplearningspark_amd/csrc/kernels/gemm_stream.hip
--- a/distributeddeeplearningspark_amd/csrc/kernels/gemm_stream.hip
+++ b/distributeddeeplearningspark_amd/csrc/kernels/gemm_stream.hip
@@ -52,9 +52,9 @@
   }
 }
 
-template <class CF>
+template <class CF, bool DUAL = false>
 __device__ __forceinline__ void stage_a(const bf16_t* __restrict__ A, long lda, int M, int m0, char* slot, int w,
-                                        int lane) {
+                                        int lane, const bf16_t* __restrict__ A2 = nullptr, long lda2 = 0) {
 #pragma unroll
   for (int i = 0; i < CF::D; ++i) {
     const int blk = i * 4 + w;
@@ -63,6 +63,9 @@
     const int c = cp ^ sw<CF::CPR>(r);
     const int gr = min(m0 + r, M - 1);
     const bf16_t* src = A + (long)gr * lda + c * 8;
+    if constexpr (DUAL) {
+      if (c >= CF::CPR / 2) src = A2 + (long)gr * lda2 + (c - CF::CPR / 2) * 8;
+    }
     const uint32_t dst = __builtin_amdgcn_readfirstlane((uint32_t) reinterpret_cast<uintptr_t>((lds_t*)(slot + blk * 1024)));
     asm volatile("s_mov_b32 m0, %1\n\tglobal_load_lds_dwordx4 %0, off" ::"v"(src), "s"(dst) : "memory", "m0");
   }
@@ -119,10 +122,11 @@
 }
 
 
-template <int WN, int K, int BMODE, bool RES, int BNR = 0, bool CSM = false>
+template <int WN, int K, int BMODE, bool RES, int BNR = 0, bool CSM = false, bool DUAL = false>
 __global__ __launch_bounds__(gst::THREADS, 2) void gemm_stream_kernel(const GemmParams p) {
   using namespace gst;
   using CF = Cfg<WN, K, CSM>;
+  static_assert(!DUAL || (CSM && !RES && BNR == 0 && BMODE == OP_KC && CF::KS % 2 == 0), "dual form");
   constexpr bool kAsmSide = true;
   __shared__ __attribute__((aligned(16))) char smem[CF::LDS];
   char* const stg = smem + CF::NBUF * CF::TILE;
@@ -131,6 +135,7 @@
   const int mt = (p.M + BM - 1) / BM;
   const int nloc = ((int)blockIdx.x < mt) ? (mt - 1 - (int)blockIdx.x) / (int)gridDim.x + 1 : 0;
   const bf16_t* __restrict__ A = reinterpret_cast<const bf16_t*>(p.a);
+  const bf16_t* __restrict__ A2 = DUAL ? reinterpret_cast<const bf16_t*>(p.a2) : nullptr;
 
   bf16x8 bfr[CF::RN][CF::KS];
   {
@@ -141,7 +146,12 @@
       for (int ks = 0; ks < CF::KS; ++ks) {
         const int n = n0 + WN * w + 16 * rn + (lane & 15);
         const int k = 32 * ks + 8 * (lane >> 4);
-        if constexpr (BMODE == OP_KC) {
+        if constexpr (DUAL) {
+          if (ks < CF::KS / 2)
+            bfr[rn][ks] = *reinterpret_cast<const bf16x8*>(B + (long)n * p.ldb + k);
+          else
+            bfr[rn][ks] = *reinterpret_cast<const bf16x8*>(reinterpret_cast<const bf16_t*>(p.b2) + (long)n * p.ldb2 + k - K / 2);
+        } else if constexpr (BMODE == OP_KC) {
           bfr[rn][ks] = *reinterpret_cast<const bf16x8*>(B + (long)n * p.ldb + k);
         } else {
           s16x8 v;
@@ -160,6 +170,15 @@
     bias_r[rn][1] = bv.y;
     bias_r[rn][2] = bv.z;
     bias_r[rn][3] = bv.w;
+    if constexpr (DUAL) {
+      if (p.bias2) {
+        const float4 b2 = *reinterpret_cast<const float4*>(p.bias2 + n0 + WN * w + 16 * rn + 4 * (lane >> 4));
+        bias_r[rn][0] += b2.x;
+        bias_r[rn][1] += b2.y;
+        bias_r[rn][2] += b2.z;
+        bias_r[rn][3] += b2.w;
+      }
+    }
   }
   float csc_r[CSM ? CF::RN : 1][4];
   if constexpr (CSM) {
@@ -172,11 +191,23 @@
       csc_r[rn][3] = cv.w;
     }
   }
+  float csc2_r[DUAL ? CF::RN : 1][4];
+  if constexpr (DUAL) {
+#pragma unroll
+    for (int rn = 0; rn < CF::RN; ++rn) {
+      const float4 cv = *reinterpret_cast<const float4*>(p.colscale2 + n0 + WN * w + 16 * rn + 4 * (lane >> 4));
+      csc2_r[rn][0] = cv.x;
+      csc2_r[rn][1] = cv.y;
+      csc2_r[rn][2] = cv.z;
+      csc2_r[rn][3] = cv.w;
+    }
+  }
   wait_vm<0>();
   auto tile_m0 = [&](int i) { return min((int)blockIdx.x + i * (int)gridDim.x, mt - 1) * BM; };
 
 #pragma unroll
-  for (int s = 0; s < CF::NBUF - 1; ++s) stage_a<CF>(A, p.lda, p.M, tile_m0(s), smem + s * CF::TILE, w, lane);
+  for (int s = 0; s < CF::NBUF - 1; ++s)
+    stage_a<CF, DUAL>(A, p.lda, p.M, tile_m0(s), smem + s * CF::TILE, w, lane, A2, p.lda2);
 
   float s1[8], s2[8];
 #pragma unroll
@@ -243,7 +274,7 @@
       }
     }
     const int ahead = i + CF::NBUF - 1;
-    stage_a<CF>(A, p.lda, p.M, tile_m0(ahead), smem + (ahead % CF::NBUF) * CF::TILE, w, lane);
+    stage_a<CF, DUAL>(A, p.lda, p.M, tile_m0(ahead), smem + (ahead % CF::NBUF) * CF::TILE, w, lane, A2, p.lda2);
     if constexpr (CSM) {
       if (p.relu_mask_out) wait_tile<CF, CF::SV>(min(i, CF::NBUF - 1));
       else wait_tile<CF>(min(i, CF::NBUF - 1));
@@ -258,6 +289,13 @@
     for (int mb = 0; mb < BM / 16; ++mb)
 #pragma unroll
       for (int rn = 0; rn < CF::RN; ++rn) acc[mb][rn] = f32x4{0.f, 0.f, 0.f, 0.f};
+    f32x4 acc2[DUAL ? BM / 16 : 1][DUAL ? CF::RN : 1];
+    if constexpr (DUAL) {
+#pragma unroll
+      for (int mb = 0; mb < BM / 16; ++mb)
+#pragma unroll
+        for (int rn = 0; rn < CF::RN; ++rn) acc2[mb][rn] = f32x4{0.f, 0.f, 0.f, 0.f};
+    }
 #pragma unroll
     for (int ks = 0; ks < CF::KS; ++ks)
 #pragma unroll
@@ -266,7 +304,15 @@
         const int c = 4 * ks + (lane >> 4);
         const bf16x8 a = *reinterpret_cast<const bf16x8*>(abuf + r * (K * 2) + ((c ^ sw<CF::CPR>(r)) << 4));
 #pragma unroll
-        for (int rn = 0; rn < CF::RN; ++rn) acc[mb][rn] = mfma16x16x32(bfr[rn][ks], a, acc[mb][rn]);
+        for (int rn = 0; rn < CF::RN; ++rn) {
+          if constexpr (DUAL) {
+            if (ks >= CF::KS / 2) {
+              acc2[mb][rn] = mfma16x16x32(bfr[rn][ks], a, acc2[mb][rn]);
+              continue;
+            }
+          }
+          acc[mb][rn] = mfma16x16x32(bfr[rn][ks], a, acc[mb][rn]);
+        }
       }
 
     constexpr int kBnrLoads = BNR == 1 ? 2 * CF::S : (BNR != 0 ? CF::S : 0);
@@ -290,7 +336,8 @@
         float v[4];
 #pragma unroll
         for (int e = 0; e < 4; ++e) {
-          if constexpr (CSM) v[e] = fmaf(acc[mb][rn][e], csc_r[rn][e], bias_r[rn][e]);
+          if constexpr (DUAL) v[e] = fmaf(acc[mb][rn][e], csc_r[rn][e], fmaf(acc2[mb][rn][e], csc2_r[rn][e], bias_r[rn][e]));
+          else if constexpr (CSM) v[e] = fmaf(acc[mb][rn][e], csc_r[rn][e], bias_r[rn][e]);
           else v[e] = fmaf(acc[mb][rn][e], p.alpha, bias_r[rn][e]);
         }
         if constexpr (RES) {
@@ -531,7 +578,27 @@
   return 0;
 }
 
+static int launch_dual(const GemmParams& p, int epi, hipStream_t s) {
+  using CF = gst::Cfg<32, 128, true>;
+  auto al16 = [](const void* q) { return (uintptr_t)q % 16 == 0; };
+  const bool ok = p.a && p.a2 && p.b && p.b2 && p.colscale && p.colscale2 && p.K == 64 && p.N > 0 && p.N % CF::NB == 0 &&
+                  epi == EPI_BF16 && p.a_mode == OP_KC && p.b_mode == OP_KC && !p.resid && !p.resid_mask && !p.stats &&
+                  !p.bnr_x && !p.bnr_premask && !p.bnr_mask && !p.rsub_h && p.alpha == 1.f && p.beta == 0.f &&
+                  !p.om.enabled && !p.aux && !p.drop_thresh && (p.relu == ACT_NONE || p.relu == ACT_RELU) &&
+                  p.k_split >= p.K && !p.split_stride && p.zcount <= 1 && !p.zcls && p.lda % 8 == 0 && p.lda2 % 8 == 0 &&
+                  p.ldb % 8 == 0 && p.ldb2 % 8 == 0 && p.ldc % 8 == 0 && p.lda >= 64 && p.lda2 >= 64 && p.ldb >= 64 &&
+                  p.ldb2 >= 64 && p.ldc >= p.N && al16(p.a) && al16(p.a2) && al16(p.b) && al16(p.b2) && al16(p.c) &&
+                  al16(p.colscale) && al16(p.colscale2) && al16(p.bias) && al16(p.bias2);
+  if (!ok) return (int)hipErrorInvalidValue;
+  const int panels = p.N / CF::NB;
+  const int mt = (p.M + gst::BM - 1) / gst::BM;
+  const int gx = std::max(1, std::min(mt, 2 * num_cus() / std::max(1, panels)));
+  hipLaunchKernelGGL((gemm_stream_kernel<32, 128, OP_KC, false, 0, true, true>), dim3(gx, panels), dim3(gst::THREADS), 0, s, p);
+  return (int)hipGetLastError();
+}
+
 int launch_gemm_stream(const GemmParams& p, int epi, hipStream_t s) {
+  if (p.a2 || p.b2 || p.colscale2 || p.bias2) return launch_dual(p, epi, s);
   int nb = gemm_stream_panel(p.N, p.K);
   if (p.resid && p.K == 128 && nb == 256) nb = 128;
   if ((p.bnr_x || p.bnr_premask) && nb > (p.K >= 256 ? 64 : 128)) nb = p.K >= 256 ? 64 : 128;
diff --git a/distributeddeeplearningspark_amd/csrc/ops_bindings.cpp b/distributeddeeplearningspark_amd/csrc/ops_bindings.cpp
--- a/distributeddeeplearningspark_amd/csrc/ops_bindings.cpp
+++ b/distributeddeeplearningspark_amd/csrc/ops_bindings.cpp
@@ -184,6 +184,19 @@
   HIP_OK(bn_fold_coef(w.data_ptr(), w.stride(0), P.data_ptr<float>(), S.data_ptr<float>(), s.data_ptr<float>(),
                       coef.data_ptr<float>(), WA.data_ptr(), WAt.data_ptr(), Gm.data_ptr(), kv.data_ptr<float>(),
                       dW.data_ptr<float>(), dW.stride(0), (int)Co, (int)Ci, cur_stream()));
+}
+
+void bn_fold_kv_(const at::Tensor& WA, const at::Tensor& Gm, const at::Tensor& sg, const at::Tensor& s, int64_t M,
+                 const at::Tensor& kv) {
+  GPU(WA); BF16(WA); BF16(Gm); F32(sg); F32(s); F32(kv);
+  CK(WA.dim() == 2 && WA.is_contiguous() && Gm.is_contiguous() && sg.is_contiguous() && s.is_contiguous() &&
+         kv.is_contiguous() && Gm.is_cuda() && sg.is_cuda() && s.is_cuda() && kv.is_cuda(),
+     "bn_fold_kv: contiguous GPU tensors, WA [Co, Ci]");
+  const int64_t Co = WA.size(0), Ci = WA.size(1);
+  CK(Gm.numel() == Ci * Ci && sg.numel() >= Co && s.numel() == Ci && kv.numel() == Ci && M > 0, "bn_fold_kv: shapes");
+  at::DeviceGuard g(WA.device());
+  HIP_OK(bn_fold_kv(WA.data_ptr(), Gm.data_ptr(), sg.data_ptr<float>(), s.data_ptr<float>(), M, kv.data_ptr<float>(),
+                    (int)Co, (int)Ci, cur_stream()));
 }
 
 void bn_bwd_dx_(const at::Tensor& dy, const at::Tensor& x, c10::optional<at::Tensor> y,
@@ -750,6 +763,7 @@
   m.def("bn_bwd_finalize", &bn_bwd_finalize_);
   m.def("bn_fold_sums", &bn_fold_sums_);
   m.def("bn_fold_coef", &bn_fold_coef_);
+  m.def("bn_fold_kv", &bn_fold_kv_);
   m.def("gram_colsum", &gram_colsum_);
   m.def("bn_fold_fwd_stats", &bn_fold_fwd_stats_);
   m.def("bn_bwd_dx", &bn_bwd_dx_);
diff --git a/distributeddeeplearningspark_amd/ops/fused_blocks.py b/distributeddeeplearningspark_amd/ops/fused_blocks.py
--- a/distributeddeeplearningspark_amd/ops/fused_blocks.py
+++ b/distributeddeeplearningspark_amd/ops/fused_blocks.py
@@ -132,17 +132,24 @@
     def forward(ctx, x, anchor, block):
         ctx.prev = _producer_of(x) if _FUSE_BNR else None
         x = x.contiguous()
-        s_down = convbn_forward(block.down, x, relu=False, apply=False) if block.down is not None else None
-        sc = s_down.yc if s_down is not None else x
-        s1 = convbn_forward(block.c1, x, relu=True)
-        s2 = convbn_forward(block.c2, s1.y, relu=True)
-        g3 = _fold_fwd_geometry(block.c3, s2.y) if s_down is None else None
-        if g3 is not None:
-            s3 = _convbn3_fold_forward(block.c3, s2.y, sc, g3)
+        gdn = _fold_down_geometry(block, x) if block.down is not None else None
+        if gdn is not None:
+            s1 = convbn_forward(block.c1, x, relu=True)
+            s2 = convbn_forward(block.c2, s1.y, relu=True)
+            s_down, s3 = _fold_down_forward(block, x, s2.y, *gdn)
+            s3.fold = True
         else:
-            s3 = convbn_forward(block.c3, s2.y, resid=sc, relu=True,
-                                res_affine=None if s_down is None else (s_down.scale, s_down.shift))
-        s3.fold = s_down is None and s3.mode == 3 and _fold_gate(s3.g)
+            s_down = convbn_forward(block.down, x, relu=False, apply=False) if block.down is not None else None
+            sc = s_down.yc if s_down is not None else x
+            s1 = convbn_forward(block.c1, x, relu=True)
+            s2 = convbn_forward(block.c2, s1.y, relu=True)
+            g3 = _fold_fwd_geometry(block.c3, s2.y) if s_down is None else None
+            if g3 is not None:
+                s3 = _convbn3_fold_forward(block.c3, s2.y, sc, g3)
+            else:
+                s3 = convbn_forward(block.c3, s2.y, resid=sc, relu=True,
+                                    res_affine=None if s_down is None else (s_down.scale, s_down.shift))
+            s3.fold = s_down is None and s3.mode == 3 and _fold_gate(s3.g)
         ctx.block, ctx.states = block, (s_down, s1, s2, s3)
         ctx.save_for_backward(x)
         ctx.needs_dx = ctx.needs_input_grad[0]
@@ -161,21 +168,31 @@
         pre3 = s3.pre_reduced
         fold = (_FOLD_BN3 and s3.fold and not _det.enabled() and pre3 is not None and pre3[2]
                 and _same_tensor(pre3[1], dout) and b.c3.bn.gamma is not None)
-        if fold:
+        fold_dn = fold and s_down is not None and s_down.gram is not None
+        fold = fold and s_down is None
+        ws_g = None
+        if fold_dn:
+            s3.pre_reduced = None
+            ws_g = pre3[0]
+            bnr2 = _bnr_mode2(s2, dout.device)
+            d2 = _fold_unit_backward(b.c3, s3, s2.y, dout, ws_g, bnr2)
+        elif fold:
             s3.pre_reduced = None
             bnr2 = _bnr_mode2(s2, dout.device)
             d2 = _fold_bn3_backward(b.c3, s3, s2, dout, pre3[0], bnr2)
             dsc = dout
-        elif s3.yc is None:
-            _recompute_yc(b.c3, s3, s2)
-            d3c, dsc = bn_backward(b.c3, s3, dout, want_dres=not masked_sc)
-        elif fuse_down:
-            Cd = s_down.yc.shape[-1]
-            ws_d = partials_workspace(s_down.yc.numel() // Cd, Cd, dout.device)
-            d3c, dsc = bn_backward(b.c3, s3, dout, False, red2=(s_down.yc, s_down.mean, ws_d))
         else:
-            d3c, dsc = bn_backward(b.c3, s3, dout, want_dres=not masked_sc)
-        if not fold:
+            if s3.yc is None:
+                _recompute_yc(b.c3, s3, s2)
+                if s_down is not None and s_down.yc is None:
+                    _recompute_yc(b.down, s_down, x)
+            if fuse_down:
+                Cd = s_down.yc.shape[-1]
+                ws_d = partials_workspace(s_down.yc.numel() // Cd, Cd, dout.device)
+                d3c, dsc = bn_backward(b.c3, s3, dout, False, red2=(s_down.yc, s_down.mean, ws_d))
+            else:
+                d3c, dsc = bn_backward(b.c3, s3, dout, want_dres=not masked_sc)
+        if not (fold or fold_dn):
             bnr2 = _bnr_mode2(s2, dout.device)
             d2 = conv_backward(b.c3, s3, d3c, s2.y, True, bnr=bnr2)
         _take_reduced(s2, bnr2, d2)
@@ -185,7 +202,9 @@
         _take_reduced(s1, bnr1, d1)
         d1c, _ = bn_backward(b.c1, s1, d1, False)
         rsub = None
-        if s_down is not None:
+        if fold_dn:
+            dsc = _fold_unit_backward(b.down, s_down, x, dout, ws_g, None, need_dx=ctx.needs_dx, exact_colsum=True)
+        elif s_down is not None:
             if fuse_down:
                 ddc, _ = bn_backward(b.down, s_down, dout, False, dy_mask=s3.mask, reduced=ws_d)
             else:
@@ -269,41 +288,97 @@
 
 
 def _convbn3_fold_forward(unit, x2, resid, g):
-    conv, bn = unit.conv, unit.bn
     M, Co, Ci = g.M, g.Co, g.Ci
     dev = x2.device
     x2m = x2.view(M, Ci)
+    st = _fold_fwd_stats(unit, x2m, g)
+    st.mask = torch.empty(-(-M * Co // 32) * 4, dtype=torch.uint8, device=dev)
+    y = torch.empty((g.N, g.H, g.W, Co), dtype=torch.bfloat16, device=dev)
+    G.linear_fwd(x2m, unit.conv.kernel.data.view(Co, Ci), bias=st.shift, relu=True, out=y.view(M, Co),
+                 resid=resid.view(M, Co), colscale=st.scale, relu_mask_out=st.mask)
+    st.y, st.mode = y, 3
+    return st
+
+
+def _recompute_yc(unit, s3, s2):
+    geo = s3.g
+    xin = s2.y if isinstance(s2, _ConvBNState) else s2
+    w = unit.conv.kernel.data.view(geo.Co, geo.Ci)
+    yc = torch.empty((geo.N, geo.H, geo.W, geo.Co), dtype=torch.bfloat16, device=xin.device)
+    G.linear_fwd(xin.view(geo.M, geo.Ci), w, out=yc.view(geo.M, geo.Co))
+    s3.yc = yc
+
+
+_FOLD_DOWN = True
+_FOLD_DOWN_MIN_ELEMS = 1 << 27
+
+
+def _pointwise_geometry(conv, xshape):
+    N, H, W, Ci = xshape
+    kh, kw = conv.kernel_size
+    if (kh, kw) != (1, 1):
+        return None
+    p = conv.padding if isinstance(conv.padding, tuple) else (0, 0)
+    g = CV.geometry(N, H, W, Ci, conv.filters, kh, kw, conv.strides, p, conv.dilation_rate)
+    return g if g.is_pointwise else None
+
+
+def _fold_down_geometry(block, x):
+    if not (_FOLD_BN3 and _FOLD_BN3_FWD and _FOLD_DOWN) or _det.enabled() or x.device.type != "cuda":
+        return None
+    if block.c3.bn.gamma is None or block.down.bn.gamma is None or x.dtype != torch.bfloat16:
+        return None
+    N, H, W, _ = x.shape
+    if any(tuple(u.conv.strides) != (1, 1) for u in (block.c1, block.c2)):
+        return None
+    gd = _pointwise_geometry(block.down.conv, x.shape)
+    g3 = _pointwise_geometry(block.c3.conv, (N, H, W, block.c2.conv.filters))
+    if gd is None or g3 is None or gd.Co != g3.Co or gd.Co % 128:
+        return None
+    if not G.stream_dual_ok(g3.Co, g3.Ci, gd.Ci) or g3.M * g3.Co < _FOLD_DOWN_MIN_ELEMS:
+        return None
+    return g3, gd
+
+
+def _fold_fwd_stats(unit, xm, g):
+    conv, bn = unit.conv, unit.bn
+    M, Co, Ci = g.M, g.Co, g.Ci
+    dev = xm.device
     ps = new_stats_workspace(-(-(Ci * Ci + Ci) // 64), dev).view(-1)
     S, s = ps[: Ci * Ci].view(Ci, Ci), ps[Ci * Ci : Ci * Ci + Ci]
-    C().gram_colsum(x2m, S, s)
+    C().gram_colsum(xm, S, s)
     stats = new_stats_workspace(Co, dev)
-    w = conv.kernel.data.view(Co, Ci)
-    C().bn_fold_fwd_stats(w, S, s, M, stats)
+    C().bn_fold_fwd_stats(conv.kernel.data.view(Co, Ci), S, s, M, stats)
     gamma = None if bn.gamma is None else bn.gamma.master
     beta = None if bn.beta is None else bn.beta.master
     rm, rv = bn._states["moving_mean"], bn._states["moving_variance"]
-    scale, shift, mean, invstd = torch.empty(4, Co, dtype=torch.float32, device=dev).unbind(0)
-    C().bn_finalize(stats, M, Co, gamma, beta, bn.epsilon, 1.0 - bn.momentum, rm, rv, mean, invstd, scale, shift)
     st = _ConvBNState()
-    st.g, st.yc = g, None
-    st.mask = torch.empty(-(-M * Co // 32) * 4, dtype=torch.uint8, device=dev)
-    y = torch.empty((g.N, g.H, g.W, Co), dtype=torch.bfloat16, device=dev)
-    G.linear_fwd(x2m, w, bias=shift, relu=True, out=y.view(M, Co), resid=resid.view(M, Co), colscale=scale,
-                 relu_mask_out=st.mask)
-    st.y, st.mean, st.invstd, st.scale, st.shift, st.mode = y, mean, invstd, scale, shift, 3
+    st.g, st.yc, st.y, st.mask = g, None, None, None
+    st.scale, st.shift, st.mean, st.invstd = torch.empty(4, Co, dtype=torch.float32, device=dev).unbind(0)
+    C().bn_finalize(stats, M, Co, gamma, beta, bn.epsilon, 1.0 - bn.momentum, rm, rv, st.mean, st.invstd, st.scale,
+                    st.shift)
     st.gram = (S, s, pool_epoch(dev))
     return st
 
 
-def _recompute_yc(unit, s3, s2):
-    geo = s3.g
-    w = unit.conv.kernel.data.view(geo.Co, geo.Ci)
-    yc = torch.empty((geo.N, geo.H, geo.W, geo.Co), dtype=torch.bfloat16, device=s2.y.device)
-    G.linear_fwd(s2.y.view(geo.M, geo.Ci), w, out=yc.view(geo.M, geo.Co))
-    s3.yc = yc
-
-
-def fold_conv_bn_backward(w, gw, g2, y2, ws_g, mean, invstd, gamma, dgamma, dbeta, bnr2=None, out=None, gram=None):
+def _fold_down_forward(block, x, y2, g3, gd):
+    M, Co = g3.M, g3.Co
+    if tuple(y2.shape) != (g3.N, g3.H, g3.W, g3.Ci):
+        raise RuntimeError("folding projection block: conv2's output does not match conv3's geometry")
+    y2 = y2.contiguous()
+    s3 = _fold_fwd_stats(block.c3, y2.view(M, g3.Ci), g3)
+    sd = _fold_fwd_stats(block.down, x.view(M, gd.Ci), gd)
+    s3.mask = torch.empty(-(-M * Co // 32) * 4, dtype=torch.uint8, device=x.device)
+    y = torch.empty((g3.N, g3.H, g3.W, Co), dtype=torch.bfloat16, device=x.device)
+    G.linear_dual_fwd(y2.view(M, g3.Ci), block.c3.conv.kernel.data.view(Co, g3.Ci), s3.scale,
+                      x.view(M, gd.Ci), block.down.conv.kernel.data.view(Co, gd.Ci), sd.scale,
+                      shift1=s3.shift, shift2=sd.shift, relu=True, out=y.view(M, Co), relu_mask_out=s3.mask)
+    s3.y, s3.mode, sd.mode = y, 3, 0
+    return sd, s3
+
+
+def fold_conv_bn_backward(w, gw, g2, y2, ws_g, mean, invstd, gamma, dgamma, dbeta, bnr2=None, out=None, gram=None,
+                          need_dx=True, exact_colsum=False):
     M, Co = g2.shape
     Ci = y2.shape[1]
     dev = g2.device
@@ -327,6 +402,10 @@
     b16 = torch.empty(2 * Co * Ci + Ci * Ci, dtype=torch.bfloat16, device=dev)
     WA, WAt, Gm = b16[: Co * Ci].view(Co, Ci), b16[Co * Ci : 2 * Co * Ci].view(Ci, Co), b16[2 * Co * Ci :].view(Ci, Ci)
     C().bn_fold_coef(w, P, S, s, coef, WA, WAt, Gm, kv, gw)
+    if not need_dx:
+        return None, sums.view(2, Co)
+    if exact_colsum:
+        C().bn_fold_kv(WA, Gm, sums[:Co], s, M, kv)
     r = G.linear_fwd(y2, Gm, bias=kv)
     if out is None:
         out = torch.empty((M, Ci), dtype=torch.bfloat16, device=dev)
@@ -335,21 +414,27 @@
 
 
 def _fold_bn3_backward(unit, s3, s2, g, ws_g, bnr2):
+    return _fold_unit_backward(unit, s3, s2.y, g, ws_g, bnr2)
+
+
+def _fold_unit_backward(unit, st, xin, g, ws_g, bnr2, need_dx=True, exact_colsum=False):
     conv, bn = unit.conv, unit.bn
-    geo = s3.g
+    geo = st.g
     M, Co, Ci = geo.M, geo.Co, geo.Ci
-    d2 = torch.empty((geo.N, geo.H, geo.W, Ci), dtype=torch.bfloat16, device=g.device)
+    dx = torch.empty((geo.N, geo.H, geo.W, Ci), dtype=torch.bfloat16, device=g.device) if need_dx else None
     gram = None
-    if s3.gram is not None and s3.gram[2] == pool_epoch(g.device):
-        gram = s3.gram[:2]
-    fold_conv_bn_backward(conv.kernel.data.view(Co, Ci), conv.kernel.grad.view(Co, Ci), g.view(M, Co), s2.y.view(M, Ci),
-                          ws_g, s3.mean, s3.invstd, bn.gamma.master, bn.gamma.grad,
-                          None if bn.beta is None else bn.beta.grad, bnr2=bnr2, out=d2.view(M, Ci), gram=gram)
+    if st.gram is not None and st.gram[2] == pool_epoch(g.device):
+        gram = st.gram[:2]
+    fold_conv_bn_backward(conv.kernel.data.view(Co, Ci), conv.kernel.grad.view(Co, Ci), g.view(M, Co), xin.view(M, Ci),
+                          ws_g, st.mean, st.invstd, bn.gamma.master, bn.gamma.grad,
+                          None if bn.beta is None else bn.beta.grad, bnr2=bnr2,
+                          out=None if dx is None else dx.view(M, Ci), gram=gram, need_dx=need_dx,
+                          exact_colsum=exact_colsum)
     if bn.grad_hook is not None:
         bn.grad_hook()
     if conv.grad_hook is not None:
         conv.grad_hook()
-    return d2
+    return dx
 
 
 def _same_tensor(a, b) -> bool:
diff --git a/distributeddeeplearningspark_amd/ops/gemm.py b/distributeddeeplearningspark_amd/ops/gemm.py
--- a/distributeddeeplearningspark_amd/ops/gemm.py
+++ b/distributeddeeplearningspark_amd/ops/gemm.py
@@ -204,6 +204,24 @@
     return gemm(x2, w, out, M, N, K, KC, KC, x2.stride(0), w.stride(0), out.stride(0), EPI_BF16, bias=bias, relu=act,
                 resid=resid, ldr=(resid.stride(0) if resid is not None else 0), stats=stats, aux=aux, drop_p=drop_p,
                 drop_seed=drop_seed)
+
+
+def stream_dual_ok(N: int, K1: int, K2: int) -> bool:
+    return K1 == 64 and K2 == 64 and N > 0 and N % 128 == 0
+
+
+def linear_dual_fwd(x1, w1, scale1, x2, w2, scale2, shift1=None, shift2=None, relu=True, out=None, relu_mask_out=None):
+    M, K1 = x1.shape
+    N = w1.shape[0]
+    K2 = x2.shape[1]
+    if not stream_dual_ok(N, K1, K2) or x2.shape[0] != M or w2.shape != (N, K2) or w1.shape[1] != K1:
+        raise ValueError("linear_dual_fwd: two [M, 64] x [N, 64]^T products with N % 128 == 0")
+    if out is None:
+        out = torch.empty((M, N), dtype=torch.bfloat16, device=x1.device)
+    C().gemm(x1, w1, out, M, N, K1, KC, KC, x1.stride(0), w1.stride(0), out.stride(0), EPI_BF16, TILE_STREAM, K1, 1.0,
+             0.0, shift1, None, 0, ACT_RELU if relu else ACT_NONE, colscale=scale1, relu_mask_out=relu_mask_out, a2=x2,
+             b2=w2, lda2=x2.stride(0), ldb2=w2.stride(0), colscale2=scale2, bias2=shift2)
+    return out
 
 
 _SPLITK_WS = {}
```

Result: faster. 13660 images/sec, median of 6 (+3.1%).
